# Orkis-Research/Quaternion-Convolutional-Neural-Networks-for-End-to-End-Automatic-Speech-Recognition

Hardware: AMD Instinct MI355X
Metric: quaternion-conv samples/sec (fwd+bwd+Adam of the full TIMIT QCNN, per-GPU batch 256) (higher is better)
Workload: dtype bf16; 1 GPU; cfg3_qcnn_relu_dropout_b256_bf16; per_gpu_batch=256, global_batch=256, filters=32, padding=same, activation=relu, loss=ctc, parallelism=dp1, optimizer=adam(5e-4) + l2 term folded into the update, launch=eager

## Files before the change

### include/qk.h

```cpp
#ifndef QK_H_
#define QK_H_

#include <stddef.h>
#include <stdint.h>

#ifdef __cplusplus
extern "C" {
#endif

#define QK_VERSION 103

typedef enum {
    QK_OK = 0,
    QK_ERR_INVALID_ARG = -1,
    QK_ERR_UNSUPPORTED = -2,
    QK_ERR_WORKSPACE = -3,
    QK_ERR_LAUNCH = -4
} qk_status_t;

typedef enum { QK_F32 = 0, QK_BF16 = 1, QK_F16 = 2 } qk_dtype_t;
typedef enum { QK_CH_LAST = 0, QK_CH_FIRST = 1 } qk_layout_t;
typedef enum { QK_ACT_LINEAR = 0, QK_ACT_RELU = 1 } qk_act_t;
typedef enum { QK_OP_FWD = 0, QK_OP_BWD_DATA = 1, QK_OP_BWD_WEIGHT = 2, QK_OP_BWD = 3 } qk_op_t;

typedef struct {
    int32_t rank;
    int32_t batch;
    int32_t in_spatial[3];
    int32_t out_spatial[3];
    int32_t cq;
    int32_t fq;
    int32_t kernel[3];
    int32_t stride[3];
    int32_t dilation[3];
    int32_t pad_lo[3];
    int32_t layout;
    int32_t dtype;
    int32_t activation;
    int32_t has_bias;
    int32_t conj;
    int32_t ws_has_kernel;
    int32_t kernel_order;
} qk_conv_desc_t;
#define QK_KERNEL_TAPS_MAJOR 0
#define QK_KERNEL_CHANNEL_MAJOR 1

typedef struct {
    int32_t rows;
    int32_t in_q;
    int32_t q_units;
    int32_t dtype;
    int32_t activation;
    int32_t has_bias;
    int32_t ws_has_kernel;
} qk_dense_desc_t;

int qk_version(void);
const char *qk_last_error(void);

#define QK_DBG_NO_MFMA16 1u
#define QK_DBG_NO_BAND16 2u
#define QK_DBG_NO_BAND32 4u
#define QK_DBG_WGRAD16_ONE_TAP 8u
#define QK_DBG_NO_WGRAD_BAND 32u
#define QK_DBG_NO_POINT16 64u
#define QK_DBG_CTC_TWO_SWEEPS 128u
#define QK_DBG_DETERMINISTIC 0x10000u
#define QK_DBG_WGRAD_BAND_V1 0x20000u
#define QK_DBG_NO_SMALL16 0x40000u
#define QK_DBG_NO_CONV_CHAIN 0x100000u
#define QK_DBG_NO_FUSED_PRELU 0x200000u
#define QK_DBG_NO_FUSED_DROPOUT 0x400000u
#define QK_DBG_NO_FUSED_CTC 0x800000u
#define QK_DBG_NO_FUSED_FIRST 0x1000000u
#define QK_DBG_NO_DENSE_IN_CHAIN 0x2000000u
#define QK_DBG_NO_FUSED_SOFTMAX 0x4000000u
#define QK_DBG_BAND16_8WAVES 16u
unsigned qk_set_debug_flags(unsigned flags);
void qk_set_debug_buffer(void *device_buffer, size_t bytes);
unsigned qk_get_debug_flags(void);

typedef enum { QK_PATH_NONE = 0, QK_PATH_MFMA16 = 1, QK_PATH_MFMA16_BAND = 2, QK_PATH_FP32_MFMA = 3,
               QK_PATH_MFMA16_POINT = 4, QK_PATH_MFMA16_SMALL = 5  } qk_path_t;
int qk_last_path(void);

typedef struct {
    int32_t op;
    int32_t dtype;
    int32_t path;
    int64_t rows;
    int32_t n, k;
    float ms;
} qk_prof_rec_t;
int qk_prof_enable(int on);
int qk_prof_count(void);
int qk_prof_get(int index, qk_prof_rec_t *out);

size_t qk_conv_workspace_bytes(const qk_conv_desc_t *desc, int op );
size_t qk_dense_workspace_bytes(const qk_dense_desc_t *desc, int op );

int qk_conv_fwd(const qk_conv_desc_t *desc, const void *x, const float *w, const float *bias,
                void *y, void *workspace, size_t workspace_bytes, void *stream);

int qk_conv_bwd_data(const qk_conv_desc_t *desc, const void *dy, const void *y, const float *w,
                     void *dx, void *workspace, size_t workspace_bytes, void *stream);

int qk_conv_bwd_weight(const qk_conv_desc_t *desc, const void *x, const void *dy, const void *y,
                       float *dw, float *dbias, void *workspace, size_t workspace_bytes,
                       void *stream);

int qk_conv_bwd_weight_acc(const qk_conv_desc_t *desc, const void *x, const void *dy, const void *y,
                           float *dw, float *dbias, void *workspace, size_t workspace_bytes,
                           void *stream);
int qk_dense_bwd_weight_acc(const qk_dense_desc_t *desc, const void *x, const void *dy, const void *y,
                            float *dw, float *dbias, void *workspace, size_t workspace_bytes,
                            void *stream);

int qk_conv_bwd(const qk_conv_desc_t *desc, const void *x, const void *dy, const void *y, const float *w,
                void *dx, float *dw, float *dbias, void *workspace, size_t workspace_bytes, void *stream);

#define QK_BWD_MASK_DX 1
#define QK_BWD_DY_PREMASKED 2
#define QK_BWD_ACCUMULATE 4
int qk_conv_bwd_chain(const qk_conv_desc_t *desc, const void *x, const void *dy, const void *y, const float *w,
                      void *dx, float *dw, float *dbias, int32_t flags, void *workspace, size_t workspace_bytes,
                      void *stream);
int qk_dense_bwd_chain(const qk_dense_desc_t *desc, const void *x, const void *dy, const void *y, const float *w,
                       void *dx, float *dw, float *dbias, int32_t flags, void *workspace, size_t workspace_bytes,
                       void *stream);

typedef struct {
    int32_t alpha_axis;
    int32_t alpha_len;
    const float *alpha;
    float drop_rate;
    uint32_t drop_seed;
    const uint32_t *drop_seed_dev;
} qk_postop_t;

int qk_conv_fwd_post(const qk_conv_desc_t *desc, const qk_postop_t *post, const void *x, const float *w,
                     const float *bias, void *pre, void *y, void *workspace, size_t workspace_bytes, void *stream);

int qk_conv_bwd_post(const qk_conv_desc_t *desc, const void *x, const void *dy, const float *w, void *dx, float *dw,
                     float *dbias, const qk_postop_t *post_x, const void *x_pre, float *dalpha_x, int32_t flags,
                     void *workspace, size_t workspace_bytes, void *stream);

int qk_postop_fwd(const qk_conv_desc_t *t, const qk_postop_t *post, const void *pre, void *y, void *stream);
int qk_postop_bwd(const qk_conv_desc_t *t, const qk_postop_t *post, const void *pre, const void *dy, void *dpre,
                  float *dalpha, void *stream);

size_t qk_conv_relu_pool_aux_bytes(const qk_conv_desc_t *desc, int32_t pool);
int qk_conv_relu_pool_fwd(const qk_conv_desc_t *desc, int32_t pool, const void *x, const float *w, const float *bias,
                          void *pooled, void *aux, void *stream);
int qk_conv_relu_pool_bwd(const qk_conv_desc_t *desc, int32_t pool, const void *x, const void *dpooled, const void *aux,
                          float *dw, float *dbias, int32_t flags, void *stream);

int qk_conv_prelu_pool_fwd(const qk_conv_desc_t *desc, int32_t pool, const qk_postop_t *post, const void *x, const float *w,
                           const float *bias, void *pooled, void *pre_pooled, void *aux, void *stream);
int qk_conv_prelu_pool_bwd(const qk_conv_desc_t *desc, int32_t pool, const qk_postop_t *post, const void *x, const void *dpooled,
                           const void *pre_pooled, const void *aux, float *dw, float *dbias, float *dalpha, int32_t flags,
                           void *stream);

int qk_conv_fold_taps(const qk_conv_desc_t *desc, const void *x, void *xcol, int32_t cq2, void *stream);

int qk_dense_fwd(const qk_dense_desc_t *desc, const void *x, const float *w, const float *bias,
                 void *y, void *workspace, size_t workspace_bytes, void *stream);
int qk_dense_bwd_data(const qk_dense_desc_t *desc, const void *dy, const void *y, const float *w,
                      void *dx, void *workspace, size_t workspace_bytes, void *stream);
int qk_dense_bwd_weight(const qk_dense_desc_t *desc, const void *x, const void *dy, const void *y,
                        float *dw, float *dbias, void *workspace, size_t workspace_bytes,
                        void *stream);

int qk_dense_bwd(const qk_dense_desc_t *desc, const void *x, const void *dy, const void *y, const float *w,
                 void *dx, float *dw, float *dbias, void *workspace, size_t workspace_bytes, void *stream);

typedef struct {
    int32_t batch, in_h, in_w, channels;
    int32_t win_h, win_w;
    int32_t out_h, out_w;
    int32_t dtype;
} qk_pool_desc_t;
int qk_maxpool2d_fwd(const qk_pool_desc_t *desc, const void *x, void *y, void *stream);
int qk_maxpool2d_bwd(const qk_pool_desc_t *desc, const void *x, const void *dy, void *dx, void *stream);

int qk_adam_step(float *param, const float *grad, float *m, float *v, size_t n, float lr,
                 float beta1, float beta2, float eps, int32_t step, float grad_scale,
                 void *stream);

int qk_adam_step_zero_grad(float *param, float *grad, float *m, float *v, size_t n, float lr,
                           float beta1, float beta2, float eps, int32_t step, float grad_scale,
                           void *stream);

size_t qk_ctc_workspace_bytes(int32_t batch, int32_t frames, int32_t max_label_len);
int qk_ctc_batch_cost(int32_t dtype, int32_t batch, int32_t frames, int32_t classes, const void *y_pred, const int32_t *labels,
                      int32_t max_label_len, const int32_t *input_length, const int32_t *label_length, float *cost, void *dy_pred,
                      void *workspace, size_t workspace_bytes, void *stream);

int qk_ctc_greedy_decode(int32_t dtype, int32_t batch, int32_t frames, int32_t classes, const void *y_pred, const int32_t *input_length,
                         int32_t *decoded, int32_t *decoded_len, float *log_prob, void *stream);
size_t qk_ctc_beam_workspace_bytes(int32_t batch, int32_t frames, int32_t beam_width);
int qk_ctc_beam_search_decode(int32_t dtype, int32_t batch, int32_t frames, int32_t classes, const void *y_pred, const int32_t *input_length,
                              int32_t beam_width, int32_t top_paths, int32_t merge_repeated, int32_t *decoded, int32_t *decoded_len,
                              float *log_prob, void *workspace, size_t workspace_bytes, void *stream);
int qk_ctc_beam_search_decode_lm(int32_t dtype, int32_t batch, int32_t frames, int32_t classes, const void *y_pred,
                                 const int32_t *input_length, int32_t beam_width, int32_t top_paths, int32_t merge_repeated,
                                 int32_t lm_order, const float *lm_table, float lm_weight, float insertion_bonus, int32_t lm_eos,
                                 int32_t *decoded, int32_t *decoded_len, float *log_prob, float *score,
                                 void *workspace, size_t workspace_bytes, void *stream);
int qk_edit_distance(int32_t batch, const int32_t *hyp, int32_t hyp_stride, const int32_t *hyp_len, const int32_t *ref, int32_t ref_stride,
                     const int32_t *ref_len, const int32_t *class_map, int32_t classes, int32_t *distance, int32_t *ref_len_out, void *stream);

#define QK_FBANK_MAX_FILT 128
enum { QK_WAVE_F32 = 0, QK_WAVE_I16 = 1 };
enum { QK_WINDOW_RECT = 0, QK_WINDOW_HAMMING = 1 };
enum { QK_FBANK_NORM_NONE = 0, QK_FBANK_NORM_UTTERANCE = 1 };
int32_t qk_fbank_num_frames(int64_t samples, int32_t frame_len, int32_t frame_step);
size_t qk_fbank_workspace_bytes(int32_t batch, int32_t frames, int32_t rows, int32_t normalize);
int qk_fbank_quaternion(int32_t wave_dtype, int32_t batch, int64_t max_samples, const void *wave, const int32_t *lengths, int32_t frames,
                        int32_t frame_len, int32_t frame_step, int32_t nfft, float preemph, int32_t window, int32_t nfilt,
                        const int32_t *mel_bins, int32_t append_energy, int32_t delta_n, int32_t normalize, int32_t out_dtype, void *out,
                        int32_t *frame_lengths, void *workspace, size_t workspace_bytes, void *stream);

#define QK_SPECAUG_MAX_MASKS 8
#define QK_SPECAUG_PLAN_WORDS 36
typedef struct qk_specaug_t {
    int32_t time_warp;
    int32_t freq_masks;
    int32_t freq_width;
    int32_t time_masks;
    int32_t time_width;
    float time_ratio;
    float fill;
    uint32_t seed;
} qk_specaug_t;
int qk_spec_augment(int32_t in_dtype, int32_t out_dtype, int32_t batch, int32_t planes, int32_t rows, int32_t frames,
                    const void *x, const int32_t *lengths, const qk_specaug_t *policy, const uint32_t *counter_dev ,
                    void *out, int32_t *plan , void *stream);

#define QK_SPEED_MAX_SPEEDS 8
#define QK_SPEED_MAX_DEN    32
#define QK_SPEED_MAX_TAPS   64
#define QK_SPEED_PLAN_WORDS 4
typedef struct qk_speed_perturb_t {
    int32_t n_speeds;
    int32_t num[QK_SPEED_MAX_SPEEDS];
    int32_t den[QK_SPEED_MAX_SPEEDS];
    int32_t half_width[QK_SPEED_MAX_SPEEDS];
    int32_t table_offset[QK_SPEED_MAX_SPEEDS];
    float gain_lo, gain_hi;
    uint32_t seed;
} qk_speed_perturb_t;
int64_t qk_speed_perturb_out_samples(int64_t max_samples, const qk_speed_perturb_t *policy);
int qk_speed_perturb(int32_t wave_dtype, int32_t batch, int64_t max_samples, const void *wave, const int32_t *lengths,
                     const qk_speed_perturb_t *policy, const float *tables , const uint32_t *counter_dev ,
                     int64_t out_samples, float *out, int32_t *out_lengths, int32_t *plan , void *stream);

int qk_softmax_rows_fwd(int32_t dtype, int64_t rows, int32_t cols, const float *logits, const float *bias, void *y, void *stream);
int qk_softmax_rows_bwd(int32_t dtype, int64_t rows, int32_t cols, const void *y, const void *dy, void *dlogits, float *dbias, void *stream);
int qk_dense_softmax_supported(int32_t dtype, int64_t rows, int32_t in_dim, int32_t units);
int qk_dense_softmax_fwd(int32_t dtype, int64_t rows, int32_t in_dim, int32_t units, const void *x, const float *kernel, const float *bias,
                         void *y, void *stream);
size_t qk_dense_softmax_bwd_workspace_bytes(int32_t dtype, int64_t rows, int32_t in_dim, int32_t units);
int qk_dense_softmax_bwd(int32_t dtype, int64_t rows, int32_t in_dim, int32_t units, const void *x, const float *kernel, const void *y,
                         const void *dy, void *dx, float *dkernel, float *dbias, const float *dy_scale_dev, float dy_scale,
                         void *workspace, size_t workspace_bytes, void *stream);
int qk_weighted_sum(int32_t dtype, int64_t n, const void *a, const float *w, float *out, void *stream);

int qk_conv_prep_kernels(int32_t n, const qk_conv_desc_t *const *descs, const int32_t *ops, const float *const *w,
                         void *const *workspaces, void *stream);

int qk_adam_step_l2(float *param, float *grad, float *m, float *v, const float *decay, size_t n, float lr,
                    float beta1, float beta2, float eps, int32_t step, float grad_scale, int32_t zero_grad,
                    void *stream);

int qk_adam_step_dev(float *param, float *grad, float *m, float *v, const float *decay, size_t n, float lr,
                     float beta1, float beta2, float eps, int32_t *step_dev, float grad_scale, int32_t zero_grad,
                     void *stream);

typedef struct qk_grad_guard_config_t {
    float clipnorm;
    float clipvalue;
    int32_t dynamic;
    float growth_factor;
    float backoff_factor;
    int32_t growth_interval;
    float min_scale;
    float max_scale;
} qk_grad_guard_config_t;

typedef struct qk_grad_guard_state_t {
    float scale;
    int32_t good_steps;
    int32_t skipped_steps;
    int32_t last_skipped;
    float last_norm;
    float last_coef;
    float last_unscale;
    int32_t nonfinite_count;
} qk_grad_guard_state_t;

size_t qk_grad_guard_workspace_bytes(size_t n);

int qk_grad_guard_reduce(const float *grad, const float *param, const float *decay, size_t n, float grad_scale,
                         const qk_grad_guard_config_t *config, qk_grad_guard_state_t *state, void *workspace,
                         size_t workspace_bytes, void *stream);

int qk_adam_step_guarded(float *param, float *grad, float *m, float *v, const float *decay, size_t n, float lr,
                         float beta1, float beta2, float eps, int32_t *step_dev, int32_t zero_grad,
                         const qk_grad_guard_config_t *config, const qk_grad_guard_state_t *state, void *stream);

#ifdef __cplusplus
}
#endif
#endif
```

### quaternion-convolutional-neural-networks-for-end-to-end-automatic-speech-recognition_amd/_lib.py

```python
import ctypes
import os

_HERE = os.path.dirname(os.path.realpath(__file__))
LIB_PATH = os.environ.get('QK_LIB') or os.path.join(_HERE, 'libqk_hip.so')

QK_F32, QK_BF16, QK_F16 = 0, 1, 2
QK_CH_LAST, QK_CH_FIRST = 0, 1
QK_ACT_LINEAR, QK_ACT_RELU = 0, 1
QK_OP_FWD, QK_OP_BWD_DATA, QK_OP_BWD_WEIGHT, QK_OP_BWD = 0, 1, 2, 3
QK_KERNEL_TAPS_MAJOR, QK_KERNEL_CHANNEL_MAJOR = 0, 1
QK_BWD_MASK_DX, QK_BWD_DY_PREMASKED, QK_BWD_ACCUMULATE = 1, 2, 4
QK_DBG_NO_MFMA16, QK_DBG_NO_BAND16, QK_DBG_NO_BAND32, QK_DBG_WGRAD16_ONE_TAP, QK_DBG_BAND16_8WAVES = 1, 2, 4, 8, 16
QK_DBG_NO_WGRAD_BAND = 32
QK_DBG_NO_POINT16 = 64
QK_DBG_CTC_TWO_SWEEPS = 128
QK_DBG_DETERMINISTIC = 0x10000
QK_DBG_WGRAD_BAND_V1 = 0x20000
QK_DBG_NO_SMALL16 = 0x40000
QK_DBG_NO_CONV_CHAIN, QK_DBG_NO_FUSED_PRELU, QK_DBG_NO_FUSED_DROPOUT, QK_DBG_NO_FUSED_CTC = 0x100000, 0x200000, 0x400000, 0x800000
QK_DBG_NO_FUSED_FIRST, QK_DBG_NO_DENSE_IN_CHAIN, QK_DBG_NO_FUSED_SOFTMAX = 0x1000000, 0x2000000, 0x4000000
QK_WAVE_F32, QK_WAVE_I16 = 0, 1
QK_WINDOW_RECT, QK_WINDOW_HAMMING = 0, 1
QK_FBANK_NORM_NONE, QK_FBANK_NORM_UTTERANCE = 0, 1
QK_FBANK_MAX_FILT = 128
QK_SPECAUG_MAX_MASKS, QK_SPECAUG_PLAN_WORDS = 8, 36
QK_SPEED_MAX_SPEEDS, QK_SPEED_MAX_DEN, QK_SPEED_MAX_TAPS, QK_SPEED_PLAN_WORDS = 8, 32, 64, 4
QK_ERR_INVALID_ARG, QK_ERR_UNSUPPORTED, QK_ERR_WORKSPACE, QK_ERR_LAUNCH = -1, -2, -3, -4
QK_PATH_NAMES = {0: 'none', 1: 'mfma16', 2: 'mfma16_band', 3: 'fp32_mfma', 4: 'mfma16_point', 5: 'mfma16_small'}

I32 = ctypes.c_int32


class ConvDesc(ctypes.Structure):
    _fields_ = [('rank', I32), ('batch', I32), ('in_spatial', I32 * 3), ('out_spatial', I32 * 3),
                ('cq', I32), ('fq', I32), ('kernel', I32 * 3), ('stride', I32 * 3),
                ('dilation', I32 * 3), ('pad_lo', I32 * 3), ('layout', I32), ('dtype', I32),
                ('activation', I32), ('has_bias', I32), ('conj', I32), ('ws_has_kernel', I32), ('kernel_order', I32)]


class DenseDesc(ctypes.Structure):
    _fields_ = [('rows', I32), ('in_q', I32), ('q_units', I32), ('dtype', I32),
                ('activation', I32), ('has_bias', I32), ('ws_has_kernel', I32)]


_VP, _FP, _SZ = ctypes.c_void_p, ctypes.c_void_p, ctypes.c_size_t
_CD, _DD = ctypes.POINTER(ConvDesc), ctypes.POINTER(DenseDesc)
class PoolDesc(ctypes.Structure):
    _fields_ = [('batch', ctypes.c_int32), ('in_h', ctypes.c_int32), ('in_w', ctypes.c_int32),
                ('channels', ctypes.c_int32), ('win_h', ctypes.c_int32), ('win_w', ctypes.c_int32),
                ('out_h', ctypes.c_int32), ('out_w', ctypes.c_int32), ('dtype', ctypes.c_int32)]


_PD = ctypes.POINTER(PoolDesc)


class PostOp(ctypes.Structure):
    _fields_ = [('alpha_axis', ctypes.c_int32), ('alpha_len', ctypes.c_int32), ('alpha', ctypes.c_void_p),
                ('drop_rate', ctypes.c_float), ('drop_seed', ctypes.c_uint32), ('drop_seed_dev', ctypes.c_void_p)]


_PO = ctypes.POINTER(PostOp)

class ProfRec(ctypes.Structure):
    _fields_ = [('op', I32), ('dtype', I32), ('path', I32), ('rows', ctypes.c_int64), ('n', I32), ('k', I32),
                ('ms', ctypes.c_float)]


class GradGuardConfig(ctypes.Structure):
    _fields_ = [('clipnorm', ctypes.c_float), ('clipvalue', ctypes.c_float), ('dynamic', I32),
                ('growth_factor', ctypes.c_float), ('backoff_factor', ctypes.c_float), ('growth_interval', I32),
                ('min_scale', ctypes.c_float), ('max_scale', ctypes.c_float)]


class SpecAugPolicy(ctypes.Structure):
    _fields_ = [('time_warp', I32), ('freq_masks', I32), ('freq_width', I32), ('time_masks', I32), ('time_width', I32),
                ('time_ratio', ctypes.c_float), ('fill', ctypes.c_float), ('seed', ctypes.c_uint32)]


class SpeedPerturbPolicy(ctypes.Structure):
    _fields_ = [('n_speeds', I32), ('num', I32 * 8), ('den', I32 * 8), ('half_width', I32 * 8), ('table_offset', I32 * 8),
                ('gain_lo', ctypes.c_float), ('gain_hi', ctypes.c_float), ('seed', ctypes.c_uint32)]


GRAD_GUARD_STATE = (('scale', True), ('good_steps', False), ('skipped_steps', False), ('last_skipped', False),
                    ('last_norm', True), ('last_coef', True), ('last_unscale', True), ('nonfinite_count', False))
_GC = ctypes.POINTER(GradGuardConfig)

SYMBOLS = {
    'qk_version': (ctypes.c_int, []),
    'qk_prof_enable': (ctypes.c_int, [ctypes.c_int]),
    'qk_prof_count': (ctypes.c_int, []),
    'qk_prof_get': (ctypes.c_int, [ctypes.c_int, ctypes.POINTER(ProfRec)]),
    'qk_last_error': (ctypes.c_char_p, []),
    'qk_set_debug_flags': (ctypes.c_uint, [ctypes.c_uint]),
    'qk_get_debug_flags': (ctypes.c_uint, []),
    'qk_set_debug_buffer': (None, [_VP, _SZ]),
    'qk_last_path': (ctypes.c_int, []),
    'qk_conv_workspace_bytes': (_SZ, [_CD, ctypes.c_int]),
    'qk_dense_workspace_bytes': (_SZ, [_DD, ctypes.c_int]),
    'qk_conv_fwd': (ctypes.c_int, [_CD, _VP, _FP, _FP, _VP, _VP, _SZ, _VP]),
    'qk_conv_bwd_data': (ctypes.c_int, [_CD, _VP, _VP, _FP, _VP, _VP, _SZ, _VP]),
    'qk_conv_fwd_post': (ctypes.c_int, [_CD, _PO, _VP, _FP, _FP, _VP, _VP, _VP, _SZ, _VP]),
    'qk_conv_bwd_post': (ctypes.c_int, [_CD, _VP, _VP, _FP, _VP, _FP, _FP, _PO, _VP, _FP, I32, _VP, _SZ, _VP]),
    'qk_postop_fwd': (ctypes.c_int, [_CD, _PO, _VP, _VP, _VP]),
    'qk_postop_bwd': (ctypes.c_int, [_CD, _PO, _VP, _VP, _VP, _FP, _VP]),
    'qk_conv_bwd_weight': (ctypes.c_int, [_CD, _VP, _VP, _VP, _FP, _FP, _VP, _SZ, _VP]),
    'qk_conv_bwd_chain': (ctypes.c_int, [_CD, _VP, _VP, _VP, _FP, _VP, _FP, _FP, I32, _VP, _SZ, _VP]),
    'qk_dense_bwd_chain': (ctypes.c_int, [_DD, _VP, _VP, _VP, _FP, _VP, _FP, _FP, I32, _VP, _SZ, _VP]),
    'qk_conv_bwd_weight_acc': (ctypes.c_int, [_CD, _VP, _VP, _VP, _FP, _FP, _VP, _SZ, _VP]),
    'qk_dense_bwd_weight_acc': (ctypes.c_int, [_DD, _VP, _VP, _VP, _FP, _FP, _VP, _SZ, _VP]),
    'qk_conv_bwd': (ctypes.c_int, [_CD, _VP, _VP, _VP, _FP, _VP, _FP, _FP, _VP, _SZ, _VP]),
    'qk_dense_bwd': (ctypes.c_int, [_DD, _VP, _VP, _VP, _FP, _VP, _FP, _FP, _VP, _SZ, _VP]),
    'qk_conv_fold_taps': (ctypes.c_int, [_CD, _VP, _VP, I32, _VP]),
    'qk_conv_relu_pool_aux_bytes': (_SZ, [_CD, I32]),
    'qk_conv_relu_pool_fwd': (ctypes.c_int, [_CD, I32, _VP, _FP, _FP, _VP, _VP, _VP]),
    'qk_conv_relu_pool_bwd': (ctypes.c_int, [_CD, I32, _VP, _VP, _VP, _FP, _FP, I32, _VP]),
    'qk_conv_prelu_pool_fwd': (ctypes.c_int, [_CD, I32, _PO, _VP, _FP, _FP, _VP, _VP, _VP, _VP]),
    'qk_conv_prelu_pool_bwd': (ctypes.c_int, [_CD, I32, _PO, _VP, _VP, _VP, _VP, _FP, _FP, _FP, I32, _VP]),
    'qk_dense_fwd': (ctypes.c_int, [_DD, _VP, _FP, _FP, _VP, _VP, _SZ, _VP]),
    'qk_dense_bwd_data': (ctypes.c_int, [_DD, _VP, _VP, _FP, _VP, _VP, _SZ, _VP]),
    'qk_dense_bwd_weight': (ctypes.c_int, [_DD, _VP, _VP, _VP, _FP, _FP, _VP, _SZ, _VP]),
    'qk_adam_step_zero_grad': (ctypes.c_int, [_FP, _FP, _FP, _FP, _SZ, ctypes.c_float, ctypes.c_float,
                                              ctypes.c_float, ctypes.c_float, I32, ctypes.c_float, _VP]),
    'qk_ctc_workspace_bytes': (_SZ, [I32, I32, I32]),
    'qk_ctc_batch_cost': (ctypes.c_int, [I32, I32, I32, I32, _VP, _VP, I32, _VP, _VP, _FP, _VP, _VP, _SZ, _VP]),
    'qk_conv_prep_kernels': (ctypes.c_int, [I32, ctypes.POINTER(_CD), ctypes.POINTER(I32), ctypes.POINTER(ctypes.c_void_p),
                                            ctypes.POINTER(ctypes.c_void_p), _VP]),
    'qk_adam_step_l2': (ctypes.c_int, [_FP, _FP, _FP, _FP, _FP, _SZ, ctypes.c_float, ctypes.c_float,
                                       ctypes.c_float, ctypes.c_float, I32, ctypes.c_float, I32, _VP]),
    'qk_adam_step_dev': (ctypes.c_int, [_FP, _FP, _FP, _FP, _FP, _SZ, ctypes.c_float, ctypes.c_float,
                                        ctypes.c_float, ctypes.c_float, _VP, ctypes.c_float, I32, _VP]),
    'qk_ctc_greedy_decode': (ctypes.c_int, [I32, I32, I32, I32, _VP, _VP, _VP, _VP, _FP, _VP]),
    'qk_ctc_beam_workspace_bytes': (_SZ, [I32, I32, I32]),
    'qk_ctc_beam_search_decode': (ctypes.c_int, [I32, I32, I32, I32, _VP, _VP, I32, I32, I32, _VP, _VP, _FP, _VP, _SZ, _VP]),
    'qk_ctc_beam_search_decode_lm': (ctypes.c_int, [I32, I32, I32, I32, _VP, _VP, I32, I32, I32, I32, _FP, ctypes.c_float,
                                                    ctypes.c_float, I32, _VP, _VP, _FP, _FP, _VP, _SZ, _VP]),
    'qk_edit_distance': (ctypes.c_int, [I32, _VP, I32, _VP, _VP, I32, _VP, _VP, I32, _VP, _VP, _VP]),
    'qk_fbank_num_frames': (I32, [ctypes.c_int64, I32, I32]),
    'qk_fbank_workspace_bytes': (_SZ, [I32, I32, I32, I32]),
    'qk_fbank_quaternion': (ctypes.c_int, [I32, I32, ctypes.c_int64, _VP, _VP, I32, I32, I32, I32, ctypes.c_float, I32, I32,
                                           ctypes.POINTER(I32), I32, I32, I32, I32, _VP, _VP, _VP, _SZ, _VP]),
    'qk_spec_augment': (ctypes.c_int, [I32, I32, I32, I32, I32, I32, _VP, _VP, ctypes.POINTER(SpecAugPolicy), _VP, _VP, _VP, _VP]),
    'qk_speed_perturb_out_samples': (ctypes.c_int64, [ctypes.c_int64, ctypes.POINTER(SpeedPerturbPolicy)]),
    'qk_speed_perturb': (ctypes.c_int, [I32, I32, ctypes.c_int64, _VP, _VP, ctypes.POINTER(SpeedPerturbPolicy), _VP, _VP, ctypes.c_int64,
                                        _VP, _VP, _VP, _VP]),
    'qk_softmax_rows_fwd': (ctypes.c_int, [I32, ctypes.c_int64, I32, _VP, _VP, _VP, _VP]),
    'qk_softmax_rows_bwd': (ctypes.c_int, [I32, ctypes.c_int64, I32, _VP, _VP, _VP, _VP, _VP]),
    'qk_dense_softmax_supported': (ctypes.c_int, [I32, ctypes.c_int64, I32, I32]),
    'qk_dense_softmax_fwd': (ctypes.c_int, [I32, ctypes.c_int64, I32, I32, _VP, _VP, _VP, _VP, _VP]),
    'qk_dense_softmax_bwd_workspace_bytes': (ctypes.c_size_t, [I32, ctypes.c_int64, I32, I32]),
    'qk_dense_softmax_bwd': (ctypes.c_int, [I32, ctypes.c_int64, I32, I32, _VP, _VP, _VP, _VP, _VP, _VP, _VP, _VP, ctypes.c_float, _VP, _SZ, _VP]),
    'qk_weighted_sum': (ctypes.c_int, [I32, ctypes.c_int64, _VP, _VP, _VP, _VP]),
    'qk_maxpool2d_fwd': (ctypes.c_int, [_PD, _VP, _VP, _VP]),
    'qk_maxpool2d_bwd': (ctypes.c_int, [_PD, _VP, _VP, _VP, _VP]),
    'qk_adam_step': (ctypes.c_int, [_FP, _FP, _FP, _FP, _SZ, ctypes.c_float, ctypes.c_float,
                                    ctypes.c_float, ctypes.c_float, I32, ctypes.c_float, _VP]),
    'qk_grad_guard_workspace_bytes': (_SZ, [_SZ]),
    'qk_grad_guard_reduce': (ctypes.c_int, [_FP, _FP, _FP, _SZ, ctypes.c_float, _GC, _VP, _VP, _SZ, _VP]),
    'qk_adam_step_guarded': (ctypes.c_int, [_FP, _FP, _FP, _FP, _FP, _SZ, ctypes.c_float, ctypes.c_float, ctypes.c_float,
                                            ctypes.c_float, _VP, I32, _GC, _VP, _VP]),
}

_lib = None


def lib():
    global _lib
    if _lib is None:
        if not os.path.exists(LIB_PATH):
            raise RuntimeError(
                'libqk_hip.so is not built (%s). Run `python -c "import __graft_entry__ as g; '
                'g.build()"` -- the quaternion layers have no CPU or eager fallback.' % LIB_PATH)
        handle = ctypes.CDLL(LIB_PATH)
        for name, (res, args) in SYMBOLS.items():
            fn = getattr(handle, name)
            fn.restype, fn.argtypes = res, args
        _lib = handle
    return _lib


def check(rc, what):
    if rc != 0:
        msg = lib().qk_last_error()
        raise RuntimeError('%s failed (status %d): %s' % (what, rc, msg.decode() if msg else ''))


def dbg(bit):
    return bool(lib().qk_get_debug_flags() & bit)


class debug_flags(object):

    def __init__(self, bits, ablate=0):
        self.bits = int(bits) | (int(ablate) << 8)

    def __enter__(self):
        self.prev = lib().qk_get_debug_flags()
        lib().qk_set_debug_flags(self.prev | self.bits)
        return self

    def __exit__(self, *exc):
        lib().qk_set_debug_flags(self.prev)
        return False


class profile(object):

    OPS = {QK_OP_FWD: 'fwd', QK_OP_BWD_DATA: 'bwd_data', QK_OP_BWD_WEIGHT: 'bwd_weight'}

    def __enter__(self):
        lib().qk_prof_enable(1)
        return self

    def __exit__(self, *exc):
        lib().qk_prof_enable(0)
        return False

    def records(self):
        out = []
        rec = ProfRec()
        for i in range(lib().qk_prof_count()):
            check(lib().qk_prof_get(i, ctypes.byref(rec)), 'qk_prof_get')
            out.append(dict(op=self.OPS.get(rec.op, str(rec.op)), dtype=rec.dtype, path=QK_PATH_NAMES.get(rec.path, 'none'),
                            rows=int(rec.rows), n=int(rec.n), k=int(rec.k), ms=float(rec.ms)))
        return out


def last_path():
    return QK_PATH_NAMES.get(lib().qk_last_path(), 'none')
```

### quaternion-convolutional-neural-networks-for-end-to-end-automatic-speech-recognition_amd/csrc/qk_api.hip

```cpp
#include <limits.h>
#include <math.h>
#include <stdarg.h>
#include <stdio.h>
#include <string.h>

#include "qk_common.h"

#include <atomic>
#include <mutex>
#include <vector>

namespace qk {

static thread_local char g_err[512] = "";
static thread_local int g_path = QK_PATH_NONE;
void note_path(int p) { g_path = p; }

namespace {
unsigned env_flags()
{
    unsigned f = 0;
    if (getenv("QK_NO_MFMA16")) f |= kDbgNoMfma16;
    if (getenv("QK_NO_BAND16")) f |= kDbgNoBand16;
    if (getenv("QK_NO_BAND32")) f |= kDbgNoBand32;
    if (getenv("QK_WGRAD16_ONE_TAP")) f |= kDbgWgradOneTap;
    if (getenv("QK_BAND16_8WAVES")) f |= kDbgBand8Waves;
    if (getenv("QK_NO_WGRAD_BAND")) f |= kDbgNoWgradBand;
    if (getenv("QK_NO_POINT16")) f |= kDbgNoPoint16;
    if (getenv("QK_CTC_TWO_SWEEPS")) f |= kDbgCtcTwoSweeps;
    if (getenv("QK_DETERMINISTIC")) f |= kDbgDeterministic;
    if (getenv("QK_WGRAD_BAND_V1")) f |= kDbgWgradBandV1;
    if (getenv("QK_NO_SMALL16")) f |= kDbgNoSmall16;
    if (getenv("QK_NO_CONV_CHAIN")) f |= QK_DBG_NO_CONV_CHAIN;
    if (getenv("QK_NO_FUSED_PRELU")) f |= QK_DBG_NO_FUSED_PRELU;
    if (getenv("QK_NO_FUSED_DROPOUT")) f |= QK_DBG_NO_FUSED_DROPOUT;
    if (getenv("QK_NO_FUSED_CTC")) f |= QK_DBG_NO_FUSED_CTC;
    if (getenv("QK_NO_FUSED_FIRST")) f |= QK_DBG_NO_FUSED_FIRST;
    if (getenv("QK_NO_DENSE_IN_CHAIN")) f |= QK_DBG_NO_DENSE_IN_CHAIN;
    if (getenv("QK_NO_FUSED_SOFTMAX")) f |= QK_DBG_NO_FUSED_SOFTMAX;
    if (const char *ab = getenv("QK_ABLATE")) f |= ((unsigned)atoi(ab) << kDbgAblateShift) & kDbgAblateMask;
    return f;
}
std::atomic<unsigned> &dbg_word()
{
    static std::atomic<unsigned> w{env_flags()};
    return w;
}
struct ForceCfg { bool set; int policy, bq; };
const ForceCfg &force_cfg()
{
    static const ForceCfg fc = [] {
        ForceCfg c = {false, -1, -1};
        if (const char *f = getenv("QK_FORCE_CFG")) c.set = sscanf(f, "%d,%d", &c.policy, &c.bq) == 2;
        return c;
    }();
    return fc;
}
}

unsigned debug_flags() { return dbg_word().load(std::memory_order_relaxed); }
static std::atomic<unsigned long long *> g_dbg_buf{nullptr};
static std::atomic<size_t> g_dbg_bytes{0};
unsigned long long *debug_buffer(size_t *bytes) { if (bytes) *bytes = g_dbg_bytes.load(); return g_dbg_buf.load(); }

namespace {
struct ProfRec { int op, dtype, path; long long rows; int n, k; hipEvent_t e0, e1; };
struct Prof { std::mutex mu; std::atomic<int> on{0}; std::vector<ProfRec> recs; };
Prof &prof() { static Prof p; return p; }
}
static thread_local int g_prof_nest = 0;
struct ProfScope {
    bool live = false;
    ProfRec r;
    hipStream_t stream;
    ProfScope(int op, const qk_conv_desc_t *d, hipStream_t st) : stream(st)
    {
        if (g_prof_nest++ > 0) return;
        if (!prof().on.load(std::memory_order_relaxed) || !d) return;
        r.op = op; r.dtype = d->dtype; r.path = QK_PATH_NONE;
        r.rows = (long long)d->batch * d->out_spatial[0] * d->out_spatial[1] * d->out_spatial[2];
        r.n = 4 * d->fq;
        r.k = 4 * d->cq * d->kernel[0] * d->kernel[1] * d->kernel[2];
        if (hipEventCreate(&r.e0) != hipSuccess) return;
        if (hipEventCreate(&r.e1) != hipSuccess) { (void)hipEventDestroy(r.e0); return; }
        live = hipEventRecord(r.e0, stream) == hipSuccess;
    }
    ~ProfScope()
    {
        --g_prof_nest;
        if (!live) return;
        (void)hipEventRecord(r.e1, stream);
        r.path = g_path;
        std::lock_guard<std::mutex> lk(prof().mu);
        prof().recs.push_back(r);
    }
};
bool debug_force_cfg(int *policy, int *bq)
{
    const ForceCfg &c = force_cfg();
    if (c.set) { *policy = c.policy; *bq = c.bq; }
    return c.set;
}
int device_cu_count()
{
    int dev = 0, n = 0;
    if (hipGetDevice(&dev) != hipSuccess || hipDeviceGetAttribute(&n, hipDeviceAttributeMultiprocessorCount, dev) != hipSuccess || n <= 0)
        return 256;
    return n;
}

void set_error(const char *fmt, ...)
{
    va_list ap;
    va_start(ap, fmt);
    vsnprintf(g_err, sizeof(g_err), fmt, ap);
    va_end(ap);
}

#define QK_DECL(sfx)                                                                              \
    int launch_hgemm_##sfx(const void *, const void *, const float *, const float *, void *,      \
                           const GemmGeom &, bool, hipStream_t);                                  \
    int launch_wgrad_##sfx(const void *, const void *, const void *, float *, float *,            \
                           const WgradGeom &, bool, hipStream_t);
QK_DECL(f32)
QK_DECL(bf16)
QK_DECL(f16)
#undef QK_DECL

int try_hgemm_16(int dtype, const void *in, const void *mask, const float *w_f32, const float *bias,
                 void *out, const GemmGeom &g, bool w_is_transposed, void *ws, size_t ws_bytes,
                 hipStream_t stream);

int try_wgrad_band_16(int dtype, const void *x, const void *dy, const void *ymask, float *dw, float *dbias,
                      const WgradGeom &g, hipStream_t stream);
int try_wgrad_16(int dtype, const void *x, const void *dy, const void *ymask, float *dw, float *dbias,
                 const WgradGeom &g, hipStream_t stream);

int launch_hgemm(int dtype, const void *in, const void *mask, const float *wk, const float *bias,
                 void *out, const GemmGeom &g, bool vec_ok, hipStream_t stream)
{
    switch (dtype) {
    case QK_F32: return launch_hgemm_f32(in, mask, wk, bias, out, g, vec_ok, stream);
    case QK_BF16: return launch_hgemm_bf16(in, mask, wk, bias, out, g, vec_ok, stream);
    case QK_F16: return launch_hgemm_f16(in, mask, wk, bias, out, g, vec_ok, stream);
    }
    return QK_ERR_INVALID_ARG;
}

int launch_wgrad(int dtype, const void *x, const void *dy, const void *ymask, float *dw,
                 float *dbias, WgradGeom g, bool vec_ok, hipStream_t stream)
{
    switch (dtype) {
    case QK_F32: return launch_wgrad_f32(x, dy, ymask, dw, dbias, g, vec_ok, stream);
    case QK_BF16: return launch_wgrad_bf16(x, dy, ymask, dw, dbias, g, vec_ok, stream);
    case QK_F16: return launch_wgrad_f16(x, dy, ymask, dw, dbias, g, vec_ok, stream);
    }
    return QK_ERR_INVALID_ARG;
}

namespace {

size_t elem_bytes(int dtype) { return dtype == QK_F32 ? 4 : 2; }

bool aligned(const void *p, size_t a) { return (reinterpret_cast<uintptr_t>(p) % a) == 0; }

bool vec_aligned(const void *p, int dtype) { return aligned(p, 4 * elem_bytes(dtype)); }

int validate(const qk_conv_desc_t *d, bool allow_rank0)
{
    if (!d) { set_error("descriptor is NULL"); return QK_ERR_INVALID_ARG; }
    if (d->rank < (allow_rank0 ? 0 : 1) || d->rank > 3) {
        set_error("rank %d not in [1,3]", d->rank); return QK_ERR_INVALID_ARG;
    }
    if (d->batch <= 0 || d->cq <= 0 || d->fq <= 0) {
        set_error("batch/cq/fq must be positive (got %d/%d/%d)", d->batch, d->cq, d->fq);
        return QK_ERR_INVALID_ARG;
    }
    long long si = 1, so = 1, taps = 1;
    for (int i = 0; i < 3; ++i) {
        if (d->in_spatial[i] <= 0 || d->out_spatial[i] <= 0 || d->kernel[i] <= 0 ||
            d->stride[i] <= 0 || d->dilation[i] <= 0 || d->pad_lo[i] < 0) {
            set_error("axis %d: extents/kernel/stride/dilation must be > 0 and pad_lo >= 0", i);
            return QK_ERR_INVALID_ARG;
        }
        if (i >= d->rank && (d->in_spatial[i] != 1 || d->out_spatial[i] != 1 || d->kernel[i] != 1 ||
                             d->stride[i] != 1 || d->dilation[i] != 1 || d->pad_lo[i] != 0)) {
            set_error("axis %d is beyond rank %d and must be the identity (1,1,1,1,1,0)", i, d->rank);
            return QK_ERR_INVALID_ARG;
        }
        si *= d->in_spatial[i]; so *= d->out_spatial[i]; taps *= d->kernel[i];
    }
    if (si * d->batch * 4LL * d->cq > INT_MAX || so * d->batch * 4LL * d->fq > INT_MAX ||
// ... 966 lines not shown
    g.span = (g.tile - 1) * frame_step + frame_len;
    const bool norm = normalize == QK_FBANK_NORM_UTTERANCE;
    const size_t need = fbank_workspace_bytes(batch, frames, g.F, norm);
    if (!workspace || workspace_bytes < need || !aligned(workspace, 16)) { set_error("fbank_quaternion needs %zu workspace bytes, got %zu", need, workspace_bytes); return QK_ERR_WORKSPACE; }
    return check_launch(launch_fbank(wave_dtype, wave, lengths, g, delta_n, norm, out_dtype, out, frame_lengths, workspace,
                                     (hipStream_t)stream), "qk_fbank_quaternion");
}

int qk_spec_augment(int32_t in_dtype, int32_t out_dtype, int32_t batch, int32_t planes, int32_t rows, int32_t frames,
                    const void *x, const int32_t *lengths, const qk_specaug_t *policy, const uint32_t *counter_dev,
                    void *out, int32_t *plan, void *stream)
{
    if (batch < 1 || planes < 1 || rows < 1 || frames < 1 || in_dtype < QK_F32 || in_dtype > QK_F16 || out_dtype < QK_F32 || out_dtype > QK_F16) {
        set_error("spec_augment: bad arguments (batch %d, planes %d, rows %d, frames %d, dtypes %d / %d)", batch, planes, rows, frames, in_dtype, out_dtype);
        return QK_ERR_INVALID_ARG;
    }
    if (!x || !lengths || !policy || !out) { set_error("spec_augment: NULL argument"); return QK_ERR_INVALID_ARG; }
    const qk_specaug_t &p = *policy;
    if (p.freq_masks < 0 || p.freq_masks > QK_SPECAUG_MAX_MASKS || p.time_masks < 0 || p.time_masks > QK_SPECAUG_MAX_MASKS) {
        set_error("spec_augment: freq_masks %d / time_masks %d outside 0 .. %d", p.freq_masks, p.time_masks, QK_SPECAUG_MAX_MASKS);
        return QK_ERR_INVALID_ARG;
    }
    if (p.time_warp < 0 || p.freq_width < 0 || p.time_width < 0) {
        set_error("spec_augment: time_warp %d, freq_width %d and time_width %d must be >= 0", p.time_warp, p.freq_width, p.time_width);
        return QK_ERR_INVALID_ARG;
    }
    if (!isfinite(p.time_ratio) || p.time_ratio < 0.f || p.time_ratio > 1.f || !isfinite(p.fill)) {
        set_error("spec_augment: time_ratio %g must lie in [0, 1] and fill %g be finite", (double)p.time_ratio, (double)p.fill);
        return QK_ERR_INVALID_ARG;
    }
    const long long count = (long long)batch * planes * rows * frames;
    if (count > INT_MAX) { set_error("spec_augment: tensor with >= 2^31 elements"); return QK_ERR_UNSUPPORTED; }
    const size_t in_bytes = (size_t)count * elem_bytes(in_dtype), out_bytes = (size_t)count * elem_bytes(out_dtype);
    if (!aligned(x, elem_bytes(in_dtype)) || !aligned(out, elem_bytes(out_dtype)) || (plan && !aligned(plan, 4))) {
        set_error("spec_augment: x, out and plan must be aligned to their element size"); return QK_ERR_INVALID_ARG;
    }
    const uintptr_t xa = reinterpret_cast<uintptr_t>(x), oa = reinterpret_cast<uintptr_t>(out);
    if (xa < oa + out_bytes && oa < xa + in_bytes) { set_error("spec_augment: out overlaps x (the warp reads neighbouring frames)"); return QK_ERR_INVALID_ARG; }
    return check_launch(launch_spec_augment(in_dtype, out_dtype, batch, planes, rows, frames, x, lengths, p, counter_dev, out, plan,
                                            (hipStream_t)stream), "qk_spec_augment");
}

static int speed_policy_check(const qk_speed_perturb_t *policy)
{
    if (!policy) { set_error("speed_perturb: policy is NULL"); return QK_ERR_INVALID_ARG; }
    const qk_speed_perturb_t &p = *policy;
    if (p.n_speeds < 1 || p.n_speeds > QK_SPEED_MAX_SPEEDS) {
        set_error("speed_perturb: n_speeds %d outside 1 .. %d", p.n_speeds, QK_SPEED_MAX_SPEEDS); return QK_ERR_INVALID_ARG;
    }
    if (!isfinite(p.gain_lo) || !isfinite(p.gain_hi) || p.gain_lo < 0.f || p.gain_lo > p.gain_hi) {
        set_error("speed_perturb: gains %g, %g must be finite with 0 <= gain_lo <= gain_hi", (double)p.gain_lo, (double)p.gain_hi);
        return QK_ERR_INVALID_ARG;
    }
    for (int i = 0; i < p.n_speeds; ++i) {
        const int num = p.num[i], den = p.den[i], kw = p.half_width[i];
        if (num < 1 || num > QK_SPEED_MAX_DEN || den < 1 || den > QK_SPEED_MAX_DEN || 2 * num < den || num > 2 * den) {
            set_error("speed_perturb: speed %d = %d / %d (both in 1 .. %d, ratio in [1/2, 2])", i, num, den, QK_SPEED_MAX_DEN);
            return QK_ERR_INVALID_ARG;
        }
        if (kw < 0 || (num == den) != (kw == 0)) {
            set_error("speed_perturb: speed %d = %d / %d with half_width %d (0 exactly when num == den)", i, num, den, kw);
            return QK_ERR_INVALID_ARG;
        }
        if (num != den && p.table_offset[i] < 0) { set_error("speed_perturb: table_offset[%d] = %d", i, p.table_offset[i]); return QK_ERR_INVALID_ARG; }
    }
    for (int i = 0; i < p.n_speeds; ++i)
        if (2 * (long long)p.half_width[i] + 2 > QK_SPEED_MAX_TAPS) {
            set_error("speed_perturb: speed %d has %lld taps, more than %d", i, 2 * (long long)p.half_width[i] + 2, QK_SPEED_MAX_TAPS);
            return QK_ERR_UNSUPPORTED;
        }
    return 0;
}

int64_t qk_speed_perturb_out_samples(int64_t max_samples, const qk_speed_perturb_t *policy)
{
    if (max_samples < 1) { set_error("speed_perturb_out_samples: max_samples %lld < 1", (long long)max_samples); return -1; }
    const int rc = speed_policy_check(policy);
    if (rc != 0 && rc != QK_ERR_UNSUPPORTED) return -1;
    if (max_samples > INT64_MAX / QK_SPEED_MAX_DEN) { set_error("speed_perturb_out_samples: max_samples too large"); return -1; }
    int64_t most = 0;
    for (int i = 0; i < policy->n_speeds; ++i) {
        const int64_t len = (max_samples * policy->den[i] + policy->num[i] - 1) / policy->num[i];
        if (len > most) most = len;
    }
    return most;
}

int qk_speed_perturb(int32_t wave_dtype, int32_t batch, int64_t max_samples, const void *wave, const int32_t *lengths,
                     const qk_speed_perturb_t *policy, const float *tables, const uint32_t *counter_dev, int64_t out_samples, float *out,
                     int32_t *out_lengths, int32_t *plan, void *stream)
{
    if (batch < 1 || max_samples < 1 || (wave_dtype != QK_WAVE_F32 && wave_dtype != QK_WAVE_I16)) {
        set_error("speed_perturb: bad arguments (batch %d, max_samples %lld, wave_dtype %d)", batch, (long long)max_samples, wave_dtype);
        return QK_ERR_INVALID_ARG;
    }
    if (!wave || !lengths || !out || !out_lengths) { set_error("speed_perturb: NULL argument"); return QK_ERR_INVALID_ARG; }
    const int rc = speed_policy_check(policy);
    if (rc == QK_ERR_INVALID_ARG) return rc;
    bool filters = false;
    for (int i = 0; i < policy->n_speeds; ++i) filters |= policy->num[i] != policy->den[i];
    if (filters && !tables) { set_error("speed_perturb: tables is NULL, but a speed has num != den"); return QK_ERR_INVALID_ARG; }
    const int64_t limit = (int64_t)1 << 26;
    if (max_samples < limit && out_samples < qk_speed_perturb_out_samples(max_samples, policy)) {
        set_error("speed_perturb: out_samples %lld below the %lld that max_samples %lld needs", (long long)out_samples,
                  (long long)qk_speed_perturb_out_samples(max_samples, policy), (long long)max_samples);
        return QK_ERR_INVALID_ARG;
    }
    const size_t wave_elem = wave_dtype == QK_WAVE_I16 ? 2 : 4;
    if (!aligned(wave, wave_elem) || !aligned(out, 4) || !aligned(lengths, 4) || !aligned(out_lengths, 4) || (plan && !aligned(plan, 4)) ||
        (tables && !aligned(tables, 4)) || (counter_dev && !aligned(counter_dev, 4))) {
        set_error("speed_perturb: pointers must be aligned to their element size"); return QK_ERR_INVALID_ARG;
    }
    if (rc != 0) return rc;
    if (max_samples >= limit || out_samples >= limit) {
        set_error("speed_perturb: max_samples %lld / out_samples %lld must be below 2^26", (long long)max_samples, (long long)out_samples);
        return QK_ERR_UNSUPPORTED;
    }
    const uintptr_t wa = reinterpret_cast<uintptr_t>(wave), oa = reinterpret_cast<uintptr_t>(out);
    const size_t wave_bytes = (size_t)batch * (size_t)max_samples * wave_elem, out_bytes = (size_t)batch * (size_t)out_samples * 4;
    if (wa < oa + out_bytes && oa < wa + wave_bytes) { set_error("speed_perturb: out overlaps wave"); return QK_ERR_INVALID_ARG; }
    return check_launch(launch_speed_perturb(wave_dtype, batch, (int)max_samples, wave, lengths, *policy, tables, counter_dev, (int)out_samples,
                                             out, out_lengths, plan, (hipStream_t)stream), "qk_speed_perturb");
}

int qk_softmax_rows_fwd(int32_t dtype, int64_t rows, int32_t cols, const float *logits, const float *bias, void *y, void *stream)
{
    if (!logits || !y || rows < 0 || cols < 1 || cols > 64 || dtype < QK_F32 || dtype > QK_F16) { set_error("qk_softmax_rows_fwd: bad argument (1 <= cols <= 64)"); return QK_ERR_INVALID_ARG; }
    if (rows == 0) return QK_OK;
    return check_launch(launch_softmax_rows(dtype, false, logits, bias, y, nullptr, rows, cols, (hipStream_t)stream), "qk_softmax_rows_fwd");
}

int qk_softmax_rows_bwd(int32_t dtype, int64_t rows, int32_t cols, const void *y, const void *dy, void *dlogits, float *dbias, void *stream)
{
    if (!y || !dy || !dlogits || rows < 0 || cols < 1 || cols > 64 || dtype < QK_F32 || dtype > QK_F16) { set_error("qk_softmax_rows_bwd: bad argument (1 <= cols <= 64)"); return QK_ERR_INVALID_ARG; }
    if (rows == 0) return QK_OK;
    return check_launch(launch_softmax_rows(dtype, true, y, dy, dlogits, dbias, rows, cols, (hipStream_t)stream), "qk_softmax_rows_bwd");
}

int qk_dense_softmax_supported(int32_t dtype, int64_t rows, int32_t in_dim, int32_t units)
{
    return dense_softmax_supported(dtype, rows, in_dim, units) ? 1 : 0;
}

int qk_dense_softmax_fwd(int32_t dtype, int64_t rows, int32_t in_dim, int32_t units, const void *x, const float *kernel, const float *bias,
                         void *y, void *stream)
{
    if (!x || !kernel || !y || rows < 0) { set_error("qk_dense_softmax_fwd: NULL buffer or negative row count"); return QK_ERR_INVALID_ARG; }
    if (!dense_softmax_supported(dtype, rows, in_dim, units)) { set_error("qk_dense_softmax_fwd: in_dim %d / units %d / dtype %d outside the kernel (in_dim 64, 128, 256; even units <= 64; 16-bit)", in_dim, units, dtype); return QK_ERR_UNSUPPORTED; }
    if (!aligned(x, 16) || !aligned(y, 4) || !aligned(kernel, 4)) { set_error("qk_dense_softmax_fwd: x must be 16-byte aligned, y 4-byte"); return QK_ERR_INVALID_ARG; }
    if (rows == 0) return QK_OK;
    return check_launch(launch_dense_softmax_fwd(dtype, rows, in_dim, units, x, kernel, bias, y, (hipStream_t)stream), "qk_dense_softmax_fwd");
}

size_t qk_dense_softmax_bwd_workspace_bytes(int32_t dtype, int64_t rows, int32_t in_dim, int32_t units)
{
    return dense_softmax_bwd_workspace_bytes(dtype, rows, in_dim, units);
}

int qk_dense_softmax_bwd(int32_t dtype, int64_t rows, int32_t in_dim, int32_t units, const void *x, const float *kernel, const void *y,
                         const void *dy, void *dx, float *dkernel, float *dbias, const float *dy_scale_dev, float dy_scale,
                         void *workspace, size_t workspace_bytes, void *stream)
{
    if (!x || !kernel || !y || !dy || !dx || rows < 0) { set_error("qk_dense_softmax_bwd: NULL buffer or negative row count"); return QK_ERR_INVALID_ARG; }
    if (!dense_softmax_supported(dtype, rows, in_dim, units)) { set_error("qk_dense_softmax_bwd: in_dim %d / units %d / dtype %d outside the kernel (in_dim 64, 128, 256; even units <= 64; 16-bit)", in_dim, units, dtype); return QK_ERR_UNSUPPORTED; }
    if (!aligned(x, 16) || !aligned(dx, 16) || !aligned(y, 4) || !aligned(dy, 4)) { set_error("qk_dense_softmax_bwd: x / dx must be 16-byte aligned, y / dy 4-byte"); return QK_ERR_INVALID_ARG; }
    if (rows == 0) return QK_OK;
    if (dkernel || dbias) {
        const size_t need = dense_softmax_bwd_workspace_bytes(dtype, rows, in_dim, units);
        if (!workspace || workspace_bytes < need || !aligned(workspace, 16)) { set_error("qk_dense_softmax_bwd needs %zu workspace bytes (16-byte aligned), got %zu", need, workspace_bytes); return QK_ERR_WORKSPACE; }
    }
    return check_launch(launch_dense_softmax_bwd(dtype, rows, in_dim, units, x, kernel, y, dy, dx, dkernel, dbias, dy_scale_dev, dy_scale, static_cast<float *>(workspace), (hipStream_t)stream), "qk_dense_softmax_bwd");
}

int qk_weighted_sum(int32_t dtype, int64_t n, const void *a, const float *w, float *out, void *stream)
{
    if (!a || !w || !out || n < 0 || dtype < QK_F32 || dtype > QK_F16) { set_error("qk_weighted_sum: bad argument"); return QK_ERR_INVALID_ARG; }
    if (n == 0) return QK_OK;
    return check_launch(launch_weighted_sum(dtype, a, w, out, n, (hipStream_t)stream), "qk_weighted_sum");
}

int qk_conv_prep_kernels(int32_t n, const qk_conv_desc_t *const *descs, const int32_t *ops, const float *const *w,
                         void *const *workspaces, void *stream)
{
    if (n < 0 || (n > 0 && (!descs || !ops || !w || !workspaces))) { set_error("qk_conv_prep_kernels: NULL argument"); return QK_ERR_INVALID_ARG; }
    for (int dt = QK_BF16; dt <= QK_F16; ++dt) {
        PrepJobs jobs;
        int m = 0;
        for (int i = 0; i <= n; ++i) {
            if (i < n) {
                const qk_conv_desc_t *d = descs[i];
                if (!d || !w[i] || !workspaces[i]) { set_error("qk_conv_prep_kernels: job %d has a NULL member", i); return QK_ERR_INVALID_ARG; }
                if (d->dtype != dt) continue;
                if (ops[i] != QK_OP_FWD && ops[i] != QK_OP_BWD_DATA && ops[i] != QK_OP_BWD) { set_error("qk_conv_prep_kernels: job %d: bad op %d", i, ops[i]); return QK_ERR_INVALID_ARG; }
                if (!aligned(workspaces[i], 16)) { set_error("qk_conv_prep_kernels: job %d: workspace not 16-byte aligned", i); return QK_ERR_INVALID_ARG; }
                if (d->cq % 16 || d->fq % 16) continue;
                const bool bwd = ops[i] != QK_OP_FWD;
                PrepJob &j = jobs.j[m++];
                j.w = w[i]; j.wq = workspaces[i]; j.taps = taps_of(d); j.cq = d->cq; j.fq = d->fq;
                j.transposed = bwd ? 1 : 0;
                j.small = 0; j.kin = 0; j.n_ot = 0;
                j.ch_major = d->kernel_order == QK_KERNEL_CHANNEL_MAJOR;
                j.neg_ijk = bwd ? (d->conj ? 1 : 0) : (d->conj ? 0 : 1);
                {
                    GemmGeom sg, sbg;
                    Small16 sm;
                    prep_geom(d, bwd, &sg);
                    if (d->layout == QK_CH_LAST && !j.ch_major && small16_shape(sg, &sbg, &sm)) {
                        PrepJob &k = jobs.j[m++];
                        k = j;
                        k.wq = static_cast<char *>(workspaces[i]) + (size_t)j.taps * pad32(d->cq) * 4 * pad32(d->fq) * 2 + 256;
                        k.small = 1; k.kin = sm.kin; k.n_ot = sm.n_ot;
                    }
                }
            }
            if (m >= 31 || (i == n && m > 0)) {
                if (int rc = launch_prep_w16_batch(dt, jobs, m, (hipStream_t)stream)) return check_launch(rc, "qk_conv_prep_kernels");
                m = 0;
            }
        }
    }
    for (int i = 0; i < n; ++i)
        if (descs[i]->dtype != QK_BF16 && descs[i]->dtype != QK_F16) { set_error("qk_conv_prep_kernels: job %d is not a 16-bit descriptor", i); return QK_ERR_INVALID_ARG; }
    return QK_OK;
}

int qk_adam_step(float *param, const float *grad, float *m, float *v, size_t n, float lr, float beta1,
                 float beta2, float eps, int32_t step, float grad_scale, void *stream)
{
    if (!param || !grad || !m || !v) { set_error("adam: NULL buffer"); return QK_ERR_INVALID_ARG; }
    if (step < 1) { set_error("adam: step must be >= 1"); return QK_ERR_INVALID_ARG; }
    return check_launch(launch_adam(param, const_cast<float *>(grad), m, v, nullptr, n, lr, beta1, beta2, eps, step, grad_scale, false, (hipStream_t)stream), "qk_adam_step");
}

int qk_adam_step_zero_grad(float *param, float *grad, float *m, float *v, size_t n, float lr, float beta1,
                           float beta2, float eps, int32_t step, float grad_scale, void *stream)
{
    if (!param || !grad || !m || !v) { set_error("adam: NULL buffer"); return QK_ERR_INVALID_ARG; }
    if (step < 1) { set_error("adam: step must be >= 1"); return QK_ERR_INVALID_ARG; }
    return check_launch(launch_adam(param, grad, m, v, nullptr, n, lr, beta1, beta2, eps, step, grad_scale, true, (hipStream_t)stream), "qk_adam_step_zero_grad");
}

int qk_adam_step_l2(float *param, float *grad, float *m, float *v, const float *decay, size_t n, float lr, float beta1,
                    float beta2, float eps, int32_t step, float grad_scale, int32_t zero_grad, void *stream)
{
    if (!param || !grad || !m || !v) { set_error("adam: NULL buffer"); return QK_ERR_INVALID_ARG; }
    if (step < 1) { set_error("adam: step must be >= 1"); return QK_ERR_INVALID_ARG; }
    return check_launch(launch_adam(param, grad, m, v, decay, n, lr, beta1, beta2, eps, step, grad_scale, zero_grad != 0, (hipStream_t)stream), "qk_adam_step_l2");
}

int qk_adam_step_dev(float *param, float *grad, float *m, float *v, const float *decay, size_t n, float lr, float beta1,
                     float beta2, float eps, int32_t *step_dev, float grad_scale, int32_t zero_grad, void *stream)
{
    if (!param || !grad || !m || !v || !step_dev) { set_error("adam: NULL buffer"); return QK_ERR_INVALID_ARG; }
    return check_launch(launch_adam(param, grad, m, v, decay, n, lr, beta1, beta2, eps, 1, grad_scale, zero_grad != 0, (hipStream_t)stream, step_dev), "qk_adam_step_dev");
}

static bool guard_config_ok(const qk_grad_guard_config_t *c, const char *what)
{
    if (!c) { set_error("%s: NULL config", what); return false; }
    if (!(c->clipnorm >= 0.f) || !(c->clipvalue >= 0.f)) { set_error("%s: clipnorm / clipvalue must be >= 0", what); return false; }
    if (c->dynamic && !(c->backoff_factor > 0.f && c->backoff_factor < 1.f && c->growth_factor > 1.f && c->growth_interval >= 1
                        && c->min_scale > 0.f && c->min_scale <= c->max_scale)) {
        set_error("%s: dynamic scaling needs 0 < backoff_factor < 1 < growth_factor, growth_interval >= 1, 0 < min_scale <= max_scale", what);
        return false;
    }
    return true;
}

size_t qk_grad_guard_workspace_bytes(size_t n) { return grad_guard_workspace_bytes(n); }

int qk_grad_guard_reduce(const float *grad, const float *param, const float *decay, size_t n, float grad_scale,
                         const qk_grad_guard_config_t *config, qk_grad_guard_state_t *state, void *workspace,
                         size_t workspace_bytes, void *stream)
{
    if (!grad || !state || !workspace) { set_error("qk_grad_guard_reduce: NULL grad, state or workspace"); return QK_ERR_INVALID_ARG; }
    if (n == 0) { set_error("qk_grad_guard_reduce: n must be > 0"); return QK_ERR_INVALID_ARG; }
    if ((param == nullptr) != (decay == nullptr)) { set_error("qk_grad_guard_reduce: param and decay go together"); return QK_ERR_INVALID_ARG; }
    if (!guard_config_ok(config, "qk_grad_guard_reduce")) return QK_ERR_INVALID_ARG;
    if (!aligned(grad, 4) || !aligned(state, 4) || (param && (!aligned(param, 4) || !aligned(decay, 4))) || !aligned(workspace, 16)) {
        set_error("qk_grad_guard_reduce: buffers need 4-byte alignment, the workspace 16-byte alignment");
        return QK_ERR_INVALID_ARG;
    }
    if (workspace_bytes < grad_guard_workspace_bytes(n)) {
        set_error("qk_grad_guard_reduce: workspace of %zu bytes, %zu needed", workspace_bytes, grad_guard_workspace_bytes(n));
        return QK_ERR_INVALID_ARG;
    }
    return check_launch(launch_grad_guard_reduce(grad, param, decay, n, grad_scale, *config, state, workspace, (hipStream_t)stream),
                        "qk_grad_guard_reduce");
}

int qk_adam_step_guarded(float *param, float *grad, float *m, float *v, const float *decay, size_t n, float lr, float beta1,
                         float beta2, float eps, int32_t *step_dev, int32_t zero_grad, const qk_grad_guard_config_t *config,
                         const qk_grad_guard_state_t *state, void *stream)
{
    if (!param || !grad || !m || !v || !step_dev || !state) { set_error("qk_adam_step_guarded: NULL buffer, step counter or state"); return QK_ERR_INVALID_ARG; }
    if (n == 0) { set_error("qk_adam_step_guarded: n must be > 0"); return QK_ERR_INVALID_ARG; }
    if (!guard_config_ok(config, "qk_adam_step_guarded")) return QK_ERR_INVALID_ARG;
    return check_launch(launch_adam_guarded(param, grad, m, v, decay, n, lr, beta1, beta2, eps, step_dev, zero_grad != 0, config->clipvalue,
                                            state, (hipStream_t)stream), "qk_adam_step_guarded");
}

}
```

### quaternion-convolutional-neural-networks-for-end-to-end-automatic-speech-recognition_amd/csrc/qk_common.h

```cpp
#pragma once

#include <hip/hip_runtime.h>
#include <stdint.h>
#include <stdio.h>
#include <stdlib.h>

#include "../../include/qk.h"

namespace qk {

constexpr unsigned kSignConv = 0x5390u;
constexpr unsigned kSignConj = 0x284Eu;

struct PostOp {
    int kind;
    int alpha_sel;
    int alpha_len;
    const float *alpha;
    float drop_scale;
    unsigned drop_thr;
    unsigned drop_seed;
    const unsigned *seed_dev;
};

// ... 131 lines not shown
    *mul = (unsigned)(((1ull << (31 + s)) + d - 1) / d);
    *sh = s;
}
__host__ __device__ __forceinline__ int fast_div(int n, unsigned mul, unsigned sh)
{
    return (int)(((unsigned long long)(unsigned)n * mul) >> (31 + sh));
}

struct bf16 { uint16_t x; };
typedef _Float16 f16;

__device__ __forceinline__ float to_f32(float v) { return v; }
__device__ __forceinline__ float to_f32(bf16 v) { return __uint_as_float(((uint32_t)v.x) << 16); }
__device__ __forceinline__ float to_f32(f16 v) { return (float)v; }

template <typename T> __device__ __forceinline__ T from_f32(float v);
template <> __device__ __forceinline__ float from_f32<float>(float v) { return v; }
template <> __device__ __forceinline__ bf16 from_f32<bf16>(float v)
{
    uint32_t u = __float_as_uint(v);
    bf16 r;
    if ((u & 0x7fffffffu) > 0x7f800000u) { r.x = (uint16_t)((u >> 16) | 0x40u); return r; }
    u += 0x7fffu + ((u >> 16) & 1u);
    r.x = (uint16_t)(u >> 16);
    return r;
}
template <> __device__ __forceinline__ f16 from_f32<f16>(float v) { return (f16)v; }

__device__ __forceinline__ void load4(const float *p, float (&o)[4])
{
    const float4 v = *reinterpret_cast<const float4 *>(p);
    o[0] = v.x; o[1] = v.y; o[2] = v.z; o[3] = v.w;
}
__device__ __forceinline__ void load4(const bf16 *p, float (&o)[4])
{
    const uint2 v = *reinterpret_cast<const uint2 *>(p);
    o[0] = __uint_as_float(v.x << 16); o[1] = __uint_as_float(v.x & 0xffff0000u);
    o[2] = __uint_as_float(v.y << 16); o[3] = __uint_as_float(v.y & 0xffff0000u);
}
__device__ __forceinline__ void load4(const f16 *p, float (&o)[4])
{
    typedef f16 h4 __attribute__((ext_vector_type(4)));
    const h4 v = *reinterpret_cast<const h4 *>(p);
    o[0] = (float)v[0]; o[1] = (float)v[1]; o[2] = (float)v[2]; o[3] = (float)v[3];
}

template <typename T>
__device__ __forceinline__ void prep_small16_write(const float *w, T *wq, long long idx, int Cq, int F, int transposed, int neg_ijk,
                                                   int kin, int q32, int fb_n)
{
    const int kso = q32 ? kin : (kin + 1) / 2;
    long long r = idx;
    const int e = (int)(r % 8); r /= 8;
    const int lane = (int)(r % 64); r /= 64;
    const int fb = (int)(r % fb_n); r /= fb_n;
    const int p = (int)(r % 4); r /= 4;
    const int kk = (int)r;
    const int k = (lane >> 4) * 8 + e;
    const int ot = kk / kso, ki = kk - ot * kso;
    const int tap_in = q32 ? ki : 2 * ki + (k >> 4);
    const int q = q32 ? k : (k & 15);
    const int j = fb * 16 + (lane & 15);
    float v = 0.f;
    if (tap_in < kin) {
        const int tap = ot * kin + tap_in;
        const int c = transposed ? j : q, f = transposed ? q : j;
        v = w[((long long)(tap * Cq + c) * 4 + p) * F + f];
        if (neg_ijk && p) v = -v;
    }
    wq[idx] = from_f32<T>(v);
}

typedef float floatx16 __attribute__((ext_vector_type(16)));
typedef float floatx4 __attribute__((ext_vector_type(4)));

__device__ __forceinline__ int mfma32_row(int r, int lane) { return (r & 3) + 8 * (r >> 2) + 4 * (lane >> 5); }

int launch_hgemm(int dtype, const void *in, const void *mask, const float *wk, const float *bias,
                 void *out, const GemmGeom &g, bool vec_ok, hipStream_t stream);
int launch_wgrad(int dtype, const void *x, const void *dy, const void *ymask, float *dw,
                 float *dbias, WgradGeom g, bool vec_ok, hipStream_t stream);
int launch_fold_taps(int dtype, const void *x, void *xcol, const GemmGeom &g, int cq2, hipStream_t stream);
int launch_mask_gt0(int dtype, void *data, const void *mask, size_t n, hipStream_t stream);
struct PrepJob { const float *w; void *wq; int taps, cq, fq, transposed, neg_ijk;
                 int small, kin, n_ot, ch_major; };
struct PrepJobs { PrepJob j[32]; };
int launch_prep_w16_batch(int dtype, const PrepJobs &jobs, int n, hipStream_t stream);
struct Small16 { int q32, fb, kin, kso, n_ot, nkk; unsigned w_bytes; };
inline bool small16_shape(const GemmGeom &g_in, GemmGeom *bg, Small16 *s)
{
    if (!((g_in.Q == 16 || g_in.Q == 32) && g_in.J == 16)) return false;
    GemmGeom g = g_in;
    g.Qp = pad32(g.Q); g.Jp = pad32(g.J);
    if (!band_geom(g, 2, bg)) return false;
    s->q32 = g.Q == 32; s->fb = g.J / 16; s->kin = bg->ks[2]; s->n_ot = bg->ks[0] * bg->ks[1];
    s->kso = s->q32 ? s->kin : (s->kin + 1) / 2;
    s->nkk = s->n_ot * s->kso;
    s->w_bytes = (unsigned)(s->nkk * 4 * s->fb * 1024);
    return s->n_ot <= 3;
}
inline size_t small16_region_bytes(const Small16 &s) { return ((size_t)s.w_bytes + 255) / 256 * 256 + 256; }
int launch_prep_small16(int dtype, const float *w, void *wq, int Cq, int F, int transposed, int neg_ijk, const Small16 &s, hipStream_t stream);
int launch_hconv16_small(int dtype, const void *in, const void *wq, const float *bias, void *out, const GemmGeom &bg, const Small16 &s, hipStream_t stream);

size_t ctc_workspace_bytes(int B, int T, int Lmax);
int launch_ctc(int dtype, int B, int T, int C, const void *pred, const int *labels, int Lmax, const int *in_len, const int *lab_len,
               float *cost, void *dpred, float *ws, hipStream_t stream);
size_t ctc_beam_workspace_bytes(int B, int T, int W);
int launch_ctc_greedy(int dtype, int B, int T, int C, const void *pred, const int *in_len, int *decoded, int *dlen, float *logp,
                      hipStream_t stream);
int launch_ctc_beam(int dtype, int B, int T, int C, const void *pred, const int *in_len, int W, int top, int merge, int *decoded,
                    int *dlen, float *logp, int *hist, hipStream_t stream);
int ctc_beam_lm_supported(int C, int W, int order);
int launch_ctc_beam_lm(int dtype, int B, int T, int C, const void *pred, const int *in_len, int W, int top, int merge, int order,
                       const float *table, float alpha, float beta, int eos, int *decoded, int *dlen, float *logp, float *score, int *hist,
                       hipStream_t stream);
int launch_edit_distance(int B, const int *hyp, int hs, const int *hl, const int *ref, int rs, const int *rl, const int *cmap,
                         int classes, int *out, int *rlen_out, hipStream_t stream);
struct FbankGeom {
    int B, n_max, T;
    int L, S, nfft;
    int nfilt, F;
    int tile, span;
    int window;
    float preemph;
    int bins[QK_FBANK_MAX_FILT + 2];
};
int fbank_tile(int L, int S);
size_t fbank_workspace_bytes(int B, int T, int F, bool norm);
int launch_fbank(int wave_dtype, const void *wave, const int *lengths, const FbankGeom &g, int N, bool norm, int out_dtype, void *out,
                 int *frame_lengths, void *ws, hipStream_t stream);
int launch_spec_augment(int in_dtype, int out_dtype, int B, int P, int R, int T, const void *x, const int *lengths,
                        const qk_specaug_t &pol, const unsigned *counter, void *out, int *plan, hipStream_t stream);
int launch_speed_perturb(int wave_dtype, int B, int n_max, const void *wave, const int *lengths, const qk_speed_perturb_t &pol,
                         const float *tables, const unsigned *counter, int n_out, float *out, int *out_lengths, int *plan,
                         hipStream_t stream);
int launch_relayout16(const void *src, void *dst, int n, int A, int B, hipStream_t stream);
struct PoolGeom { int batch, ih, iw, C, wh, ww, oh, ow; };
int launch_maxpool(int dtype, bool backward, const void *x, const void *dy, void *out, const PoolGeom &g, hipStream_t stream);
size_t conv1_pool_argbits_bytes(int N, int H, int W, int F);
int launch_conv1_pool(int dtype, bool backward, const void *x, const float *w, const float *bias, const void *io, void *argbits,
                      float *dw, float *dbias, int N, int H, int W, int F, int has_bias, hipStream_t stream,
                      const float *alpha = nullptr, int alpha_len = 0, const void *pre = nullptr, float *dalpha = nullptr,
                      int x_planes = 0);
int launch_postop(int dtype, bool backward, const void *pre, const void *dy, void *out, float *dalpha, const PostOp &p,
                  long long rows, int channels, int key_div, int key_mod, hipStream_t stream);
int launch_softmax_rows(int dtype, bool backward, const void *a, const void *b, void *out, float *dbias, long long rows, int cols,
                        hipStream_t stream);
int launch_weighted_sum(int dtype, const void *a, const float *w, float *out, long long n, hipStream_t stream);
bool dense_softmax_supported(int dtype, long long rows, int K, int U);
int launch_dense_softmax_fwd(int dtype, long long rows, int K, int U, const void *x, const float *w, const float *bias, void *y, hipStream_t stream);
size_t dense_softmax_bwd_workspace_bytes(int dtype, long long rows, int K, int U);
int launch_dense_softmax_bwd(int dtype, long long rows, int K, int U, const void *x, const float *w, const void *y, const void *dy, void *dx,
                             float *dw, float *dbias, const float *dy_scale_dev, float dy_scale, float *ws, hipStream_t stream);
int launch_adam(float *p, float *g, float *m, float *v, const float *decay, size_t n, float lr, float b1,
                float b2, float eps, int step, float gscale, bool zero_grad, hipStream_t stream, int *step_dev = nullptr);
size_t grad_guard_workspace_bytes(size_t n);
int launch_grad_guard_reduce(const float *grad, const float *param, const float *decay, size_t n, float grad_scale,
                             const qk_grad_guard_config_t &cfg, qk_grad_guard_state_t *state, void *ws, hipStream_t stream);
int launch_adam_guarded(float *p, float *g, float *m, float *v, const float *decay, size_t n, float lr, float b1, float b2, float eps,
                        int *step_dev, bool zero_grad, float clipvalue, const qk_grad_guard_state_t *state, hipStream_t stream);

void set_error(const char *fmt, ...);
void note_path(int qk_path);

enum : unsigned {
    kDbgNoMfma16 = QK_DBG_NO_MFMA16, kDbgNoBand16 = QK_DBG_NO_BAND16, kDbgNoBand32 = QK_DBG_NO_BAND32,
    kDbgWgradOneTap = QK_DBG_WGRAD16_ONE_TAP, kDbgBand8Waves = QK_DBG_BAND16_8WAVES, kDbgNoWgradBand = QK_DBG_NO_WGRAD_BAND,
    kDbgNoPoint16 = QK_DBG_NO_POINT16, kDbgCtcTwoSweeps = QK_DBG_CTC_TWO_SWEEPS, kDbgDeterministic = QK_DBG_DETERMINISTIC, kDbgWgradBandV1 = QK_DBG_WGRAD_BAND_V1, kDbgNoSmall16 = QK_DBG_NO_SMALL16, kDbgAblateShift = 8, kDbgAblateMask = 0xffu << 8
};
unsigned debug_flags();
unsigned long long *debug_buffer(size_t *bytes);
inline int debug_ablate() { return (int)((debug_flags() & kDbgAblateMask) >> kDbgAblateShift); }
bool debug_force_cfg(int *policy, int *bq);
int device_cu_count();

}
```

### quaternion-convolutional-neural-networks-for-end-to-end-automatic-speech-recognition_amd/csrc/qk_out_layer.hip

```cpp
#include "qk_common.h"

namespace qk {
namespace {

typedef __bf16 o_bf16x8 __attribute__((ext_vector_type(8)));
typedef _Float16 o_f16x8 __attribute__((ext_vector_type(8)));
typedef short o_v4s __attribute__((ext_vector_type(4)));
typedef short o_v8s __attribute__((ext_vector_type(8)));
typedef __attribute__((address_space(3))) o_v4s o_lds_v4s;

__device__ __forceinline__ floatx4 mfma_o(bf16, const uint4 &a, const uint4 &b, const floatx4 &c)
{
    return __builtin_amdgcn_mfma_f32_16x16x32_bf16(__builtin_bit_cast(o_bf16x8, a), __builtin_bit_cast(o_bf16x8, b), c, 0, 0, 0);
}
__device__ __forceinline__ floatx4 mfma_o(f16, const uint4 &a, const uint4 &b, const floatx4 &c)
{
    return __builtin_amdgcn_mfma_f32_16x16x32_f16(__builtin_bit_cast(o_f16x8, a), __builtin_bit_cast(o_f16x8, b), c, 0, 0, 0);
}
__device__ __forceinline__ unsigned pack2o(bf16, float a, float b) { return (unsigned)from_f32<bf16>(a).x | ((unsigned)from_f32<bf16>(b).x << 16); }
__device__ __forceinline__ unsigned pack2o(f16, float a, float b)
{
    const f16 x = (f16)a, y = (f16)b;
    return (unsigned)__builtin_bit_cast(unsigned short, x) | ((unsigned)__builtin_bit_cast(unsigned short, y) << 16);
}
__device__ __forceinline__ float lo16(bf16, unsigned v) { return __uint_as_float(v << 16); }
__device__ __forceinline__ float hi16(bf16, unsigned v) { return __uint_as_float(v & 0xffff0000u); }
__device__ __forceinline__ float lo16(f16, unsigned v) { return (float)__builtin_bit_cast(f16, (unsigned short)(v & 0xffffu)); }
__device__ __forceinline__ float hi16(f16, unsigned v) { return (float)__builtin_bit_cast(f16, (unsigned short)(v >> 16)); }

typedef unsigned int o_u32x4 __attribute__((ext_vector_type(4)));
__device__ __forceinline__ __amdgpu_buffer_rsrc_t rsrc_o(const void *p, unsigned long long bytes)
{
    return __builtin_amdgcn_make_buffer_rsrc(const_cast<void *>(p), 0, (int)(bytes > 0xffffffffull ? 0xffffffffu : (unsigned)bytes), 0x00020000);
}
__device__ __forceinline__ uint4 ld16_o(__amdgpu_buffer_rsrc_t r, unsigned voff)
{
    const o_u32x4 v = __builtin_amdgcn_raw_buffer_load_b128(r, (int)voff, 0, 0);
    return make_uint4(v.x, v.y, v.z, v.w);
}
constexpr unsigned kOob = 0xF0000000u;

template <typename T, int KS>
__global__ void __launch_bounds__(256) __attribute__((amdgpu_waves_per_eu(2, 2)))
k_dense_softmax_fwd(const T *__restrict__ x, const float *__restrict__ w, const float *__restrict__ bias, T *__restrict__ y,
                    const long long rows, const int U)
{
    constexpr int K = KS * 32;
    constexpr int WP = K + 8;
    __shared__ __attribute__((aligned(16))) T wt[64 * WP];
    const int tid = threadIdx.x, lane = tid & 63, wave = tid >> 6;
    const int l16 = lane & 15, g = lane >> 4;
    const __amdgpu_buffer_rsrc_t rx = rsrc_o(x, (unsigned long long)rows * K * sizeof(T));
    const long long n_tiles = (rows + 15) / 16;
    const long long stride = (long long)gridDim.x * 4;
    long long tile = (long long)blockIdx.x * 4 + wave;
    uint4 xf[KS], xn[KS];
    auto fetch = [&](long long tl, uint4 (&dst)[KS]) {
        const long long row = tl * 16 + l16;
        const unsigned off = (tl < n_tiles && row < rows) ? (unsigned)((row * K + 8 * g) * (long long)sizeof(T)) : kOob;
#pragma unroll
        for (int s = 0; s < KS; ++s) dst[s] = ld16_o(rx, off == kOob ? kOob : off + 64u * s);
    };
    fetch(tile, xf);
    {
        const int c = tid & 63, kq = tid >> 6;
        constexpr int KPT = K / 4;
        const float *wc = w + c;
#pragma unroll
        for (int k0 = 0; k0 < KPT; k0 += 16) {
            float v[16];
#pragma unroll
            for (int q = 0; q < 16; ++q) v[q] = c < U ? wc[(long long)(kq * KPT + k0 + q) * U] : 0.f;
#pragma unroll
            for (int q = 0; q < 16; q += 2) *reinterpret_cast<unsigned *>(wt + c * WP + kq * KPT + k0 + q) = pack2o(T(), v[q], v[q + 1]);
        }
    }
    __syncthreads();
    uint4 wf[4][KS];
#pragma unroll
    for (int t = 0; t < 4; ++t)
#pragma unroll
        for (int s = 0; s < KS; ++s) wf[t][s] = *reinterpret_cast<const uint4 *>(wt + (16 * t + l16) * WP + 32 * s + 8 * g);
    float b0[4][4];
#pragma unroll
    for (int t = 0; t < 4; ++t)
#pragma unroll
        for (int r = 0; r < 4; ++r) {
            const int c = 16 * t + 4 * g + r;
            b0[t][r] = c < U ? (bias ? bias[c] : 0.f) : -1e30f;
        }
    for (; tile < n_tiles; tile += stride) {
        fetch(tile + stride, xn);
        floatx4 acc[4];
#pragma unroll
        for (int t = 0; t < 4; ++t)
#pragma unroll
            for (int r = 0; r < 4; ++r) acc[t][r] = b0[t][r];
#pragma unroll
        for (int s = 0; s < KS; ++s)
#pragma unroll
            for (int t = 0; t < 4; ++t) acc[t] = mfma_o(T(), wf[t][s], xf[s], acc[t]);
        float m = -1e30f;
#pragma unroll
        for (int t = 0; t < 4; ++t)
#pragma unroll
            for (int r = 0; r < 4; ++r) m = fmaxf(m, acc[t][r]);
        m = fmaxf(m, __shfl_xor(m, 16));
        m = fmaxf(m, __shfl_xor(m, 32));
        float sum = 0.f;
#pragma unroll
        for (int t = 0; t < 4; ++t)
#pragma unroll
            for (int r = 0; r < 4; ++r) { acc[t][r] = __expf(acc[t][r] - m); sum += acc[t][r]; }
        sum += __shfl_xor(sum, 16);
        sum += __shfl_xor(sum, 32);
        const float inv = 1.f / sum;
        const long long row = tile * 16 + l16;
        if (row < rows) {
            T *yr = y + row * U;
#pragma unroll
            for (int t = 0; t < 4; ++t) {
                const int c = 16 * t + 4 * g;
                if ((U & 1) == 0) {
                    if (c + 1 < U) *reinterpret_cast<unsigned *>(yr + c) = pack2o(T(), acc[t][0] * inv, acc[t][1] * inv);
                    if (c + 3 < U) *reinterpret_cast<unsigned *>(yr + c + 2) = pack2o(T(), acc[t][2] * inv, acc[t][3] * inv);
                } else {
#pragma unroll
                    for (int r = 0; r < 4; ++r)
                        if (c + r < U) yr[c + r] = from_f32<T>(acc[t][r] * inv);
                }
            }
        }
#pragma unroll
        for (int s = 0; s < KS; ++s) xf[s] = xn[s];
    }
}

template <typename T, int NW>
__global__ void __launch_bounds__(NW * 64)
k_dense_softmax_bwd(const T *__restrict__ x, const float *__restrict__ w, const T *__restrict__ y, const T *__restrict__ dy,
                    T *__restrict__ dx, float *__restrict__ part, const long long rows, const int U,
                    const float *__restrict__ dy_scale_dev, const float dy_scale)
{
    constexpr int K = NW * 64, NTHR = NW * 64;
    constexpr int XP = K * 2 + 32;
    constexpr int DP = 160;
    static_assert(((XP / 4) % 16) == 8, "x tile pitch: 8 dwords (mod 16) keeps 8 consecutive rows on 8 different 8-bank groups");
    constexpr int RPT = (32 * 8) / NTHR;
    constexpr int XU = (32 * K * 2 / 16) / NTHR;
    __shared__ __attribute__((aligned(16))) char xs[32 * XP];
    __shared__ __attribute__((aligned(16))) char ds[32 * DP];
    __shared__ float dbs[NTHR / 8][64];
    const int tid = threadIdx.x, lane = tid & 63, wave = __builtin_amdgcn_readfirstlane(tid >> 6);
    const int l16 = lane & 15, g = lane >> 4;

    uint4 wf[2][2][2];
#pragma unroll
    for (int u = 0; u < 2; ++u)
#pragma unroll
        for (int e = 0; e < 2; ++e)
#pragma unroll
            for (int s = 0; s < 2; ++s) {
                const int col = 64 * wave + 32 * u + 8 * (l16 >> 2) + 4 * e + (l16 & 3);
                const float *wr = w + (long long)col * U + 32 * s + 8 * g;
                float v[8];
#pragma unroll
                for (int q = 0; q < 8; ++q) v[q] = (32 * s + 8 * g + q < U) ? wr[q] : 0.f;
                wf[u][e][s] = make_uint4(pack2o(T(), v[0], v[1]), pack2o(T(), v[2], v[3]), pack2o(T(), v[4], v[5]), pack2o(T(), v[6], v[7]));
            }
    floatx4 gw[4][4];
#pragma unroll
    for (int t = 0; t < 4; ++t)
#pragma unroll
        for (int u = 0; u < 4; ++u)
#pragma unroll
            for (int r = 0; r < 4; ++r) gw[t][u][r] = 0.f;
    float dbp[8];
#pragma unroll
    for (int q = 0; q < 8; ++q) dbp[q] = 0.f;

    const __amdgpu_buffer_rsrc_t rx = rsrc_o(x, (unsigned long long)rows * K * sizeof(T));
    const float sc = (dy_scale_dev ? *dy_scale_dev : 1.f) * dy_scale;
    const int l8 = tid & 7;
    const int np = (U + 1) / 2;
    const long long n_blocks = (rows + 31) / 32;
    uint4 xr[XU];
    unsigned yv[RPT][4], gv[RPT][4];
    auto fetch = [&](long long blk) {
#pragma unroll
        for (int k = 0; k < XU; ++k) {
            const int unit = tid + k * NTHR;
            const long long row = blk * 32 + unit / (K / 8);
            xr[k] = ld16_o(rx, (blk < n_blocks && row < rows) ? (unsigned)(row * K * 2 + (unit % (K / 8)) * 16) : kOob);
        }
#pragma unroll
        for (int rr = 0; rr < RPT; ++rr) {
            const long long row = blk * 32 + (tid >> 3) + rr * (NTHR / 8);
            const bool ok = blk < n_blocks && row < rows;
#pragma unroll
            for (int q = 0; q < 4; ++q) {
                const int p = l8 + 8 * q;
                const bool okp = ok && p < np;
                yv[rr][q] = okp ? *reinterpret_cast<const unsigned *>(y + row * U + 2 * p) : 0u;
                gv[rr][q] = okp ? *reinterpret_cast<const unsigned *>(dy + row * U + 2 * p) : 0u;
            }
        }
    };
    long long blk = blockIdx.x;
    if (blk < n_blocks) fetch(blk);
    for (; blk < n_blocks; blk += gridDim.x) {
#pragma unroll
        for (int rr = 0; rr < RPT; ++rr) {
            float dot = 0.f;
#pragma unroll
            for (int q = 0; q < 4; ++q)
                dot += lo16(T(), yv[rr][q]) * lo16(T(), gv[rr][q]) + hi16(T(), yv[rr][q]) * hi16(T(), gv[rr][q]);
            dot += __shfl_xor(dot, 1);
            dot += __shfl_xor(dot, 2);
            dot += __shfl_xor(dot, 4);
            const int lrow = (tid >> 3) + rr * (NTHR / 8);
#pragma unroll
            for (int q = 0; q < 4; ++q) {
                const int p = l8 + 8 * q;
                const unsigned d2 = pack2o(T(), sc * lo16(T(), yv[rr][q]) * (lo16(T(), gv[rr][q]) - dot), sc * hi16(T(), yv[rr][q]) * (hi16(T(), gv[rr][q]) - dot));
                *reinterpret_cast<unsigned *>(ds + lrow * DP + 4 * p) = p < np ? d2 : 0u;
                dbp[2 * q] += lo16(T(), d2);
                dbp[2 * q + 1] += hi16(T(), d2);
            }
        }
#pragma unroll
        for (int k = 0; k < XU; ++k) {
            const int unit = tid + k * NTHR;
            *reinterpret_cast<uint4 *>(xs + (unit / (K / 8)) * XP + (unit % (K / 8)) * 16) = xr[k];
        }
        __syncthreads();
        fetch(blk + gridDim.x);
        {
            floatx4 acc[2][2][2];
#pragma unroll
            for (int rt = 0; rt < 2; ++rt) {
                uint4 dl[2];
#pragma unroll
                for (int s = 0; s < 2; ++s) dl[s] = *reinterpret_cast<const uint4 *>(ds + (16 * rt + l16) * DP + 64 * s + 16 * g);
#pragma unroll
                for (int u = 0; u < 2; ++u)
#pragma unroll
                    for (int e = 0; e < 2; ++e) {
                        floatx4 a = {0.f, 0.f, 0.f, 0.f};
                        a = mfma_o(T(), wf[u][e][0], dl[0], a);
                        a = mfma_o(T(), wf[u][e][1], dl[1], a);
                        acc[rt][u][e] = a;
                    }
            }
#pragma unroll
            for (int rt = 0; rt < 2; ++rt) {
                const long long row = blk * 32 + 16 * rt + l16;
                if (row < rows) {
#pragma unroll
                    for (int u = 0; u < 2; ++u) {
                        const floatx4 a0 = acc[rt][u][0], a1 = acc[rt][u][1];
                        const uint4 v = make_uint4(pack2o(T(), a0[0], a0[1]), pack2o(T(), a0[2], a0[3]), pack2o(T(), a1[0], a1[1]), pack2o(T(), a1[2], a1[3]));
                        *reinterpret_cast<uint4 *>(dx + row * K + 64 * wave + 32 * u + 8 * g) = v;
                    }
                }
            }
        }
        {
            const int tr_row = 4 * g + (l16 >> 2), tr_col = 4 * (l16 & 3);
            uint4 af[4], bf[4];
#pragma unroll
            for (int t = 0; t < 4; ++t) {
                const char *p = ds + tr_row * DP + (16 * t + tr_col) * 2;
                const o_v4s lo = __builtin_amdgcn_ds_read_tr16_b64_v4i16((o_lds_v4s *)(p));
                const o_v4s hi = __builtin_amdgcn_ds_read_tr16_b64_v4i16((o_lds_v4s *)(p + 16 * DP));
                af[t] = __builtin_bit_cast(uint4, __builtin_shufflevector(lo, hi, 0, 1, 2, 3, 4, 5, 6, 7));
            }
#pragma unroll
            for (int u = 0; u < 4; ++u) {
                const char *p = xs + tr_row * XP + (64 * wave + 16 * u + tr_col) * 2;
                const o_v4s lo = __builtin_amdgcn_ds_read_tr16_b64_v4i16((o_lds_v4s *)(p));
                const o_v4s hi = __builtin_amdgcn_ds_read_tr16_b64_v4i16((o_lds_v4s *)(p + 16 * XP));
                bf[u] = __builtin_bit_cast(uint4, __builtin_shufflevector(lo, hi, 0, 1, 2, 3, 4, 5, 6, 7));
            }
#pragma unroll
            for (int t = 0; t < 4; ++t)
#pragma unroll
                for (int u = 0; u < 4; ++u) gw[t][u] = mfma_o(T(), af[t], bf[u], gw[t][u]);
        }
        __syncthreads();
    }
    if (part) {
        float *slab = part + (long long)blockIdx.x * (NW * 16 * 256 + 64);
#pragma unroll
        for (int t = 0; t < 4; ++t)
#pragma unroll
            for (int u = 0; u < 4; ++u)
                *reinterpret_cast<floatx4 *>(slab + ((wave * 16 + t * 4 + u) * 64 + lane) * 4) = gw[t][u];
#pragma unroll
        for (int q = 0; q < 4; ++q) {
            const int p = l8 + 8 * q;
            dbs[tid >> 3][2 * p] = dbp[2 * q];
            dbs[tid >> 3][2 * p + 1] = dbp[2 * q + 1];
        }
        __syncthreads();
        if (tid < 64) {
            float sum = 0.f;
            for (int r = 0; r < NTHR / 8; ++r) sum += dbs[r][tid];
            slab[NW * 16 * 256 + tid] = sum;
        }
    }
}

template <int NW>
__global__ void __launch_bounds__(1024)
k_dense_softmax_reduce(const float *__restrict__ part, const int n_slabs, float *__restrict__ dw, float *__restrict__ dbias, const int U)
{
    __shared__ floatx4 red[64][16];
    constexpr int SLAB = NW * 16 * 256 + 64;
    const int q = threadIdx.x & 15, grp = threadIdx.x >> 4;
    floatx4 sum = {0.f, 0.f, 0.f, 0.f};
    if ((int)blockIdx.x == NW * 64) {
        for (int sl = grp; sl < n_slabs; sl += 64) sum += *reinterpret_cast<const floatx4 *>(part + (long long)sl * SLAB + NW * 16 * 256 + 4 * q);
    } else {
        const float *p = part + ((long long)blockIdx.x * 16 + q) * 4;
#pragma unroll 8
        for (int sl = grp; sl < n_slabs; sl += 64) sum += *reinterpret_cast<const floatx4 *>(p + (long long)sl * SLAB);
    }
    red[grp][q] = sum;
    __syncthreads();
    if (grp < 8) {
        floatx4 v = red[grp][q];
#pragma unroll
        for (int k = 1; k < 8; ++k) v += red[grp + 8 * k][q];
        red[grp][q] = v;
    }
    __syncthreads();
    if (grp != 0) return;
    floatx4 v = red[0][q];
#pragma unroll
    for (int k = 1; k < 8; ++k) v += red[k][q];
    if ((int)blockIdx.x == NW * 64) {
        if (dbias)
#pragma unroll
            for (int r = 0; r < 4; ++r)
                if (4 * q + r < U) dbias[4 * q + r] += v[r];
        return;
    }
    if (!dw) return;
    const int f = blockIdx.x * 16 + q;
    const int reg = f >> 6, lane = f & 63;
    const int wave = reg >> 4, t = (reg >> 2) & 3, u = reg & 3, l16 = lane & 15, g = lane >> 4;
    const int xc = 64 * wave + 16 * u + l16;
#pragma unroll
    for (int r = 0; r < 4; ++r) {
        const int c = 16 * t + 4 * g + r;
        if (c < U) dw[(long long)xc * U + c] += v[r];
    }
}

}

bool dense_softmax_supported(int dtype, long long rows, int K, int U)
{
    return (dtype == QK_BF16 || dtype == QK_F16) && rows >= 0 && (K == 64 || K == 128 || K == 256) && U >= 2 && U <= 64 && (U % 2) == 0 &&
           rows * (long long)K * 2 < 0xF0000000ll;
}

int launch_dense_softmax_fwd(int dtype, long long rows, int K, int U, const void *x, const float *w, const float *bias, void *y, hipStream_t stream)
{
    if (!dense_softmax_supported(dtype, rows, K, U)) return QK_ERR_UNSUPPORTED;
    const long long n_tiles = (rows + 15) / 16;
    long long blocks = (long long)device_cu_count() * 2;
    if (blocks > (n_tiles + 3) / 4) blocks = (n_tiles + 3) / 4;
    if (blocks < 1) blocks = 1;
#define QK_GO(TT, KS) hipLaunchKernelGGL((k_dense_softmax_fwd<TT, KS>), dim3((unsigned)blocks), dim3(256), 0, stream, (const TT *)x, w, bias, (TT *)y, rows, U)
    if (dtype == QK_BF16) { if (K == 256) QK_GO(bf16, 8); else if (K == 128) QK_GO(bf16, 4); else QK_GO(bf16, 2); }
    else { if (K == 256) QK_GO(f16, 8); else if (K == 128) QK_GO(f16, 4); else QK_GO(f16, 2); }
#undef QK_GO
    return hipGetLastError() == hipSuccess ? 0 : QK_ERR_LAUNCH;
}

static int dense_softmax_bwd_grid(long long rows, int K)
{
    const long long n_blocks = (rows + 31) / 32;
    long long blocks = (long long)device_cu_count() * (K == 256 ? 1 : K == 128 ? 2 : 4);
    if (blocks > n_blocks) blocks = n_blocks;
    return (int)(blocks < 1 ? 1 : blocks);
}

size_t dense_softmax_bwd_workspace_bytes(int dtype, long long rows, int K, int U)
{
    if (!dense_softmax_supported(dtype, rows, K, U)) return 0;
    return (size_t)dense_softmax_bwd_grid(rows, K) * ((size_t)(K / 64) * 16 * 256 + 64) * sizeof(float);
}

int launch_dense_softmax_bwd(int dtype, long long rows, int K, int U, const void *x, const float *w, const void *y, const void *dy, void *dx,
                             float *dw, float *dbias, const float *dy_scale_dev, float dy_scale, float *ws, hipStream_t stream)
{
    if (!dense_softmax_supported(dtype, rows, K, U)) return QK_ERR_UNSUPPORTED;
    const int blocks = dense_softmax_bwd_grid(rows, K);
    float *part = (dw || dbias) ? ws : nullptr;
#define QK_GO(TT, NW) do { hipLaunchKernelGGL((k_dense_softmax_bwd<TT, NW>), dim3((unsigned)blocks), dim3(NW * 64), 0, stream, (const TT *)x, w, (const TT *)y, (const TT *)dy, (TT *)dx, part, rows, U, dy_scale_dev, dy_scale); \
        if (part) hipLaunchKernelGGL((k_dense_softmax_reduce<NW>), dim3(NW * 64 + 1), dim3(1024), 0, stream, part, blocks, dw, dbias, U); } while (0)
    if (dtype == QK_BF16) { if (K == 256) QK_GO(bf16, 4); else if (K == 128) QK_GO(bf16, 2); else QK_GO(bf16, 1); }
    else { if (K == 256) QK_GO(f16, 4); else if (K == 128) QK_GO(f16, 2); else QK_GO(f16, 1); }
#undef QK_GO
    return hipGetLastError() == hipSuccess ? 0 : QK_ERR_LAUNCH;
}

}
```

### quaternion-convolutional-neural-networks-for-end-to-end-automatic-speech-recognition_amd/functional.py

```python
import ctypes
import math

import numpy as np
import torch

from . import _lib as L
from ._shape import conv_output_length, normalize_tuple, tf_pads

_DTYPES = {torch.float32: L.QK_F32, torch.bfloat16: L.QK_BF16, torch.float16: L.QK_F16}
_PREP_CACHE_ON = not __import__('os').environ.get('QK_NO_PREP_CACHE')
_PREP_PARAMS = __import__('weakref').WeakValueDictionary()
_CAST_PARAMS = __import__('weakref').WeakValueDictionary()
_PREP_WARNED = False


def invalidate_cached_kernels(params=None):
    if params is None:
        params = list(_PREP_PARAMS.values()) + list(_CAST_PARAMS.values())
    n = 0
    for p in params:
        hit = False
        for key in ('_qk_prep', '_qk_cast16', '_qk_cast'):
            if p.__dict__.pop(key, None) is not None:
                hit = True
# ... 91 lines not shown
        self._ws_bytes = {}

    def _prep_job(self, op):
        d = self.desc
        if isinstance(d, L.DenseDesc):
            c = L.ConvDesc()
            c.rank, c.batch, c.cq, c.fq, c.dtype, c.conj, c.layout = 0, d.rows, d.in_q, d.q_units, d.dtype, 1, L.QK_CH_LAST
            for i in range(3):
                c.in_spatial[i] = c.out_spatial[i] = c.kernel[i] = c.stride[i] = c.dilation[i] = 1
        else:
            c = L.ConvDesc.from_buffer_copy(d)
        return c, (L.QK_OP_FWD if op == L.QK_OP_FWD else L.QK_OP_BWD_DATA)

    def _kernel_only_bytes(self, op):
        d = self.desc
        if d.dtype == L.QK_F32 or getattr(d, 'layout', L.QK_CH_LAST) != L.QK_CH_LAST:
            return 0
        cq, fq = (d.in_q, d.q_units) if isinstance(d, L.DenseDesc) else (d.cq, d.fq)
        if cq % 16 or fq % 16:
            return 0
        kop = L.QK_OP_FWD if op == L.QK_OP_FWD else L.QK_OP_BWD_DATA
        n = self._ws_bytes.get(('k', kop))
        if n is None:
            n = self._ws_bytes[('k', kop)] = int(getattr(L.lib(), self.ws_fn)(ctypes.byref(self.desc), kop))
        return n

    def _prep_key(self, op):
        d = self.desc
        key = ('f' if op == L.QK_OP_FWD else 't', int(d.conj) if hasattr(d, 'conj') else 1, int(d.dtype))
        if getattr(d, 'kernel_order', L.QK_KERNEL_TAPS_MAJOR) != L.QK_KERNEL_TAPS_MAJOR:
            key += (int(d.kernel_order), tuple(d.kernel), int(d.cq), int(d.fq))
        return key

    def _ws(self, op, like, wparam=None):
        n = self._ws_bytes.get(op)
        if n is None:
            n = self._ws_bytes[op] = int(getattr(L.lib(), self.ws_fn)(ctypes.byref(self.desc), op))
        self.desc.ws_has_kernel = 0
        if n == 0:
            return None, 0
        if (wparam is not None and not self.static_buffers and n == self._kernel_only_bytes(op) and wparam.is_leaf
                and wparam.requires_grad and _PREP_CACHE_ON):
            key = self._prep_key(op)
            cache = wparam.__dict__.setdefault('_qk_prep', {})
            base = getattr(wparam, '_qk_flat_base', None)
            ver = (wparam._version, -1 if base is None else base._version)
            hit = cache.get(key)
            if hit is not None and hit[0] == ver and hit[1] == wparam.data_ptr() and hit[2].numel() == n \
                    and hit[2].device == like.device:
                self.desc.ws_has_kernel = 1
                return hit[2], n
            buf = torch.empty(n, dtype=torch.uint8, device=like.device)
            cache[key] = [ver, wparam.data_ptr(), buf, self._prep_job(op)]
            _PREP_PARAMS[id(wparam)] = wparam
            return buf, n
        if self.static_buffers:
            buf = self._ws_cache.get(op)
            if buf is None:
                buf = self._ws_cache[op] = torch.empty(n, dtype=torch.uint8, device=like.device)
            return buf, n
        return torch.empty(n, dtype=torch.uint8, device=like.device), n

    def fwd(self, x, w, bias, out=None, wparam=None):
        y = out if out is not None else torch.empty(self.y_shape, dtype=x.dtype, device=x.device)
        ws, n = self._ws(L.QK_OP_FWD, x, wparam)
        with _on_device(x.device):
            rc = getattr(L.lib(), self.names[0])(ctypes.byref(self.desc), _ptr(x), _ptr(w), _ptr(bias),
                                                 _ptr(y), _ptr(ws), n, _stream(x))
        L.check(rc, self.names[0])
        return y

    def bwd_data(self, dy, y, w, out=None, wparam=None):
        dx = out if out is not None else torch.empty(self.x_shape, dtype=dy.dtype, device=dy.device)
        ws, n = self._ws(L.QK_OP_BWD_DATA, dy, wparam)
        with _on_device(dy.device):
            rc = getattr(L.lib(), self.names[1])(ctypes.byref(self.desc), _ptr(dy), _ptr(y), _ptr(w),
                                                 _ptr(dx), _ptr(ws), n, _stream(dy))
        L.check(rc, self.names[1])
        return dx

    def bwd_weight(self, x, dy, y, has_bias, out=None, masked_dy_out=None, accumulate=False):
        if out is not None:
            dw, db = out
        else:
            dw = torch.empty(self.w_shape, dtype=torch.float32, device=x.device)
            db = torch.empty((self.w_shape[-1],), dtype=torch.float32, device=x.device) if has_bias else None
        ws, n = self._ws(L.QK_OP_BWD_WEIGHT, x)
        if masked_dy_out is not None:
            ws, n = masked_dy_out, masked_dy_out.numel() * masked_dy_out.element_size()
        with _on_device(x.device):
            name = self.names[2] + ('_acc' if accumulate else '')
            if accumulate and out is None:
                raise ValueError('accumulate=True needs the buffers to add into (out=)')
            rc = getattr(L.lib(), name)(ctypes.byref(self.desc), _ptr(x), _ptr(dy), _ptr(y),
                                        _ptr(dw), _ptr(db), _ptr(ws), n, _stream(x))
        L.check(rc, name)
        return dw, db


    def fwd_post(self, x, w, bias, post, wparam=None):
        pre = torch.empty(self.y_shape, dtype=x.dtype, device=x.device) if post.alpha is not None else None
        y = torch.empty(self.y_shape, dtype=x.dtype, device=x.device)
        ws, n = self._ws(L.QK_OP_FWD, x, wparam)
        with _on_device(x.device):
            rc = L.lib().qk_conv_fwd_post(ctypes.byref(self.desc), ctypes.byref(post.struct), _ptr(x), _ptr(w), _ptr(bias),
                                          _ptr(pre), _ptr(y), _ptr(ws), n, _stream(x))
        L.check(rc, 'qk_conv_fwd_post')
        return pre, y

    def bwd_post(self, x, dy, w, has_bias, post_x, x_pre, dalpha_x, direct=None, wparam=None):
        dx = torch.empty(self.x_shape, dtype=dy.dtype, device=dy.device)
        if direct is not None:
            dw, db = direct
        else:
            dw = torch.empty(self.w_shape, dtype=torch.float32, device=x.device)
            db = torch.empty((self.w_shape[-1],), dtype=torch.float32, device=x.device) if has_bias else None
        ws, n = self._ws(L.QK_OP_BWD, x, wparam)
        with _on_device(x.device):
            rc = L.lib().qk_conv_bwd_post(ctypes.byref(self.desc), _ptr(x), _ptr(dy), _ptr(w), _ptr(dx), _ptr(dw), _ptr(db),
                                          ctypes.byref(post_x.struct), _ptr(x_pre), _ptr(dalpha_x),
                                          L.QK_BWD_ACCUMULATE if direct is not None else 0, _ptr(ws), n, _stream(x))
        L.check(rc, 'qk_conv_bwd_post')
        return (dx, None, None) if direct is not None else (dx, dw, db)

    def bwd(self, x, dy, y, w, has_bias, out=None, flags=0, wparam=None):
        if out is not None:
            dx, dw, db = out
        else:
            dx = torch.empty(self.x_shape, dtype=dy.dtype, device=dy.device)
            dw = torch.empty(self.w_shape, dtype=torch.float32, device=x.device)
            db = torch.empty((self.w_shape[-1],), dtype=torch.float32, device=x.device) if has_bias else None
        ws, n = self._ws(L.QK_OP_BWD, x, wparam)
        name = self.names[1].replace('_bwd_data', '_bwd')
        with _on_device(x.device):
            if flags:
                name += '_chain'
                rc = getattr(L.lib(), name)(ctypes.byref(self.desc), _ptr(x), _ptr(dy), _ptr(y), _ptr(w), _ptr(dx),
                                            _ptr(dw), _ptr(db), int(flags), _ptr(ws), n, _stream(x))
            else:
                rc = getattr(L.lib(), name)(ctypes.byref(self.desc), _ptr(x), _ptr(dy), _ptr(y), _ptr(w), _ptr(dx),
                                            _ptr(dw), _ptr(db), _ptr(ws), n, _stream(x))
        L.check(rc, name)
        return dx, dw, db


class PostOp(object):

    def __init__(self, alpha, alpha_axis=-1, rate=0.0, seed=0, seed_dev=None):
        if alpha is not None and (alpha.dtype != torch.float32 or not alpha.is_cuda):
            raise TypeError('PReLU slopes must be float32 device tensors')
        if seed_dev is not None and (seed_dev.dtype != torch.int32 or not seed_dev.is_cuda or seed_dev.numel() != 1):
            raise TypeError('seed_dev must be a one-element int32 device tensor (the training step counter of adam_step)')
        self.seed_dev = seed_dev
        if not 0.0 <= float(rate) < 1.0:
            raise ValueError('dropout rate must be in [0, 1), got %r' % (rate,))
        self.alpha, self.alpha_axis, self.rate, self.seed = alpha, int(alpha_axis), float(rate), int(seed) & 0xffffffff
        self.applied_rate = min(255, int(self.rate * 256.0 + 0.5)) / 256.0
        self.flat = alpha.detach().reshape(-1).contiguous() if alpha is not None else None
        self.struct = L.PostOp(self.alpha_axis if alpha is not None else -1, self.flat.numel() if alpha is not None else 0,
                               self.flat.data_ptr() if alpha is not None else None, self.rate, self.seed,
                               seed_dev.data_ptr() if seed_dev is not None else None)


def _tensor_desc(t):
    d = L.ConvDesc()
    d.rank, d.batch, d.fq, d.dtype = t.dim() - 2, t.shape[0], t.shape[-1] // 4, _DTYPES[t.dtype]
    for i in range(3):
        d.out_spatial[i] = t.shape[1 + i] if i < t.dim() - 2 else 1
    return d


def postop_fwd(pre, post):
    y = torch.empty_like(pre)
    d = _tensor_desc(pre)
    with _on_device(pre.device):
        rc = L.lib().qk_postop_fwd(ctypes.byref(d), ctypes.byref(post.struct), _ptr(pre), _ptr(y), _stream(pre))
    L.check(rc, 'qk_postop_fwd')
    return y


def postop_bwd(pre, dy, post, dalpha):
    dpre = torch.empty_like(pre)
    d = _tensor_desc(pre)
    with _on_device(pre.device):
        rc = L.lib().qk_postop_bwd(ctypes.byref(d), ctypes.byref(post.struct), _ptr(pre), _ptr(dy), _ptr(dpre), _ptr(dalpha),
                                   _stream(pre))
    L.check(rc, 'qk_postop_bwd')
    return dpre


class _PostOpFn(torch.autograd.Function):
    @staticmethod
    def forward(ctx, pre, alpha, post):
        ctx.post = post
        y = postop_fwd(pre, post)
        ctx.save_for_backward(pre if post.alpha is not None else y)
        return y

    @staticmethod
    def backward(ctx, dy):
        pre, = ctx.saved_tensors
        post = ctx.post
        if post.alpha is None:
            return postop_bwd(pre, dy.contiguous(), post, None), None, None
        dalpha = torch.zeros(post.flat.numel(), dtype=torch.float32, device=pre.device)
        dpre = postop_bwd(pre, dy.contiguous(), post, dalpha)
        return dpre, dalpha.reshape(post.alpha.shape), None


def prelu_dropout(x, alpha, alpha_axis=-1, rate=0.0, seed=0):
    _require_device(x, 'prelu_dropout')
    xc = x.contiguous()
    if xc.shape[-1] % (4 if xc.dtype == torch.float32 else 8) or xc.dim() < 2 or xc.dim() > 5:
        raise ValueError('prelu_dropout: unsupported shape %s' % (tuple(x.shape),))
    return _PostOpFn.apply(xc, alpha, PostOp(alpha, alpha_axis, rate, seed))


def relu_dropout(x, rate=0.0, seed=0):
    return prelu_dropout(x, None, -1, rate, seed)


def _direct_grad(w, b, want_w, want_b):
    if not (want_w and getattr(w, '_qk_direct_grad', False) and w.grad is not None and w.grad.is_contiguous()
            and w.grad.dtype == torch.float32):
        return None
    if b is None:
        return w.grad, None
    if not (want_b and getattr(b, '_qk_direct_grad', False) and b.grad is not None and b.grad.is_contiguous()
            and b.grad.dtype == torch.float32):
        return None
    return w.grad, b.grad


def _grad_ready(*params):
    for p in params:
        cb = getattr(p, '_qk_grad_ready', None) if p is not None else None
        if cb is not None:
            cb(p)


class _HamiltonFn(torch.autograd.Function):
    @staticmethod
    def forward(ctx, x, w, bias, call):
        y = call.fwd(x, w, bias, wparam=w)
        ctx.call = call
        ctx.has_bias = bias is not None
        ctx.params = (w, bias)
        ctx.save_for_backward(x, w, y if call.relu else None)
        return y

    @staticmethod
    def backward(ctx, dy):
        x, w, y = ctx.saved_tensors
        call = ctx.call
        dy = dy.contiguous()
        dx = dw = db = None
        want_w = ctx.needs_input_grad[1] or (ctx.has_bias and ctx.needs_input_grad[2])
        direct = _direct_grad(ctx.params[0], ctx.params[1], ctx.needs_input_grad[1], ctx.has_bias and ctx.needs_input_grad[2])
        if ctx.needs_input_grad[0] and want_w:
            if direct is not None:
                dx = torch.empty(call.x_shape, dtype=dy.dtype, device=dy.device)
                call.bwd(x, dy, y, w, ctx.has_bias, out=(dx,) + direct, flags=L.QK_BWD_ACCUMULATE, wparam=ctx.params[0])
            else:
                dx, dw, db = call.bwd(x, dy, y, w, ctx.has_bias, wparam=ctx.params[0])
        elif ctx.needs_input_grad[0]:
            dx = call.bwd_data(dy, y, w, wparam=ctx.params[0])
        elif want_w:
            if direct is not None:
                call.bwd_weight(x, dy, y, ctx.has_bias, out=direct, accumulate=True)
            else:
                dw, db = call.bwd_weight(x, dy, y, ctx.has_bias)
        if direct is not None and want_w:
            _grad_ready(*ctx.params)
        return dx, dw, db, None


def _act_code(activation):
    if activation in (None, 'linear'):
        return L.QK_ACT_LINEAR
    if activation == 'relu':
        return L.QK_ACT_RELU
    raise ValueError('fused activation must be None/"linear"/"relu", got %r' % (activation,))


def _check_weights(w, bias, n_out):
    if w.dtype != torch.float32 or (bias is not None and bias.dtype != torch.float32):
        raise TypeError('kernel / bias must be float32 (Keras floatx); activations may be 16-bit')
    if bias is not None and tuple(bias.shape) != (n_out,):
        raise ValueError('bias must have shape (%d,), got %s' % (n_out, tuple(bias.shape)))


def conv_call(x_shape, w_shape, dtype, rank, strides=1, padding='valid', layout='channels_last',
              dilation_rate=1, activation=None, use_bias=True, conj=False, kernel_order=0):
    st = normalize_tuple(strides, rank, 'strides')
    dl = normalize_tuple(dilation_rate, rank, 'dilation_rate')
    if len(x_shape) != rank + 2 or len(w_shape) != rank + 2:
        raise ValueError('rank %d conv needs %d-D input and kernel' % (rank, rank + 2))
    if layout == 'channels_first':
        ci, sp = x_shape[1], tuple(x_shape[2:])
    else:
        ci, sp = x_shape[-1], tuple(x_shape[1:-1])
    cq, fq = w_shape[-2], w_shape[-1] // 4
    if ci != 4 * cq or w_shape[-1] != 4 * fq:
        raise ValueError('input channels %d / kernel shape %s are not quaternion-consistent'
                         % (ci, tuple(w_shape)))
    d = L.ConvDesc()
# ... 270 lines not shown

    @staticmethod
    def backward(ctx, dout):
        x, aux = ctx.saved_tensors
        dout = dout.contiguous()
        direct = _direct_grad(ctx.params[0], ctx.params[1], ctx.needs_input_grad[1], ctx.has_bias and ctx.needs_input_grad[2])
        if direct is not None:
            dw, db = direct
        else:
            dw = torch.empty(ctx.w_shape, dtype=torch.float32, device=x.device)
            db = torch.empty((ctx.w_shape[-1],), dtype=torch.float32, device=x.device) if ctx.has_bias else None
        with _on_device(x.device):
            rc = L.lib().qk_conv_relu_pool_bwd(ctypes.byref(ctx.call.desc), ctx.pool, _ptr(x), _ptr(dout), _ptr(aux), _ptr(dw), _ptr(db),
                                               L.QK_BWD_ACCUMULATE if direct is not None else 0, _stream(x))
        L.check(rc, 'qk_conv_relu_pool_bwd')
        if direct is not None:
            _grad_ready(*ctx.params)
            return None, None, None, None, None
        return None, dw, db, None, None


def _first_layer_call(x, kernel, activation, use_bias, x_layout):
    if x_layout == 'channels_first':
        n, c, h, w = x.shape
        call = conv_call((n, h, w, c), tuple(kernel.shape), x.dtype, 2, 1, 'same', 'channels_last', 1, activation, use_bias, False)
        call.desc.layout = L.QK_CH_FIRST
        return call
    return conv_call(tuple(x.shape), tuple(kernel.shape), x.dtype, 2, 1, 'same', 'channels_last', 1, activation, use_bias, False)


def conv_relu_pool_supported(x, kernel, pool, x_layout='channels_last'):
    ch_axis, h_axis = (1, 2) if x_layout == 'channels_first' else (-1, 1)
    if not (x.is_cuda and x.dtype in (torch.bfloat16, torch.float16) and x.dim() == 4 and x.shape[ch_axis] == 4 and not x.requires_grad
            and kernel.dim() == 4 and tuple(kernel.shape[:3]) == (3, 5, 1) and kernel.shape[-1] % 4 == 0 and x.shape[0] > 0):
        return False
    if tf_pads(x.shape[h_axis], pool, pool, 1, 'same')[0] != 0:
        return False
    try:
        call = _first_layer_call(x, kernel, 'relu', True, x_layout)
    except ValueError:
        return False
    return int(L.lib().qk_conv_relu_pool_aux_bytes(ctypes.byref(call.desc), pool)) > 0


def conv_relu_pool(x, kernel, bias=None, pool=3, x_layout='channels_last'):
    _require_device(x, 'conv_relu_pool')
    _check_weights(kernel, bias, kernel.shape[-1])
    xc = x.contiguous()
    call = _first_layer_call(xc, kernel, 'relu', bias is not None, x_layout)
    if not L.lib().qk_conv_relu_pool_aux_bytes(ctypes.byref(call.desc), pool):
        raise RuntimeError('conv_relu_pool: geometry outside the fused first-layer kernel')
    return _ConvReluPoolFn.apply(xc, kernel.contiguous(), bias, call, pool)


class _ConvPreluPoolFn(torch.autograd.Function):

    @staticmethod
    def forward(ctx, x, w, bias, alpha, call, pool, post):
        n, h, wd = call.desc.batch, call.desc.in_spatial[0], call.desc.in_spatial[1]
        ctx.params = (w, bias)
        out = torch.empty((n, -(-h // pool), wd, w.shape[-1]), dtype=x.dtype, device=x.device)
        nb = int(L.lib().qk_conv_relu_pool_aux_bytes(ctypes.byref(call.desc), pool))
        keep = any(ctx.needs_input_grad[1:4])
        aux = torch.empty(nb, dtype=torch.uint8, device=x.device) if keep else None
        pre = torch.empty_like(out) if keep else None
        with _on_device(x.device):
            rc = L.lib().qk_conv_prelu_pool_fwd(ctypes.byref(call.desc), pool, ctypes.byref(post.struct), _ptr(x), _ptr(w), _ptr(bias),
                                                _ptr(out), _ptr(pre), _ptr(aux), _stream(x))
        L.check(rc, 'qk_conv_prelu_pool_fwd')
        ctx.call, ctx.pool, ctx.post, ctx.has_bias = call, pool, post, bias is not None
        ctx.w_shape = tuple(w.shape)
        ctx.save_for_backward(x, aux, pre)
        return out

    @staticmethod
    def backward(ctx, dout):
        x, aux, pre = ctx.saved_tensors
        dout = dout.contiguous()
        post = ctx.post
        direct = _direct_grad(ctx.params[0], ctx.params[1], ctx.needs_input_grad[1], ctx.has_bias and ctx.needs_input_grad[2])
        if direct is not None:
            dw, db = direct
        else:
            dw = torch.empty(ctx.w_shape, dtype=torch.float32, device=x.device)
            db = torch.empty((ctx.w_shape[-1],), dtype=torch.float32, device=x.device) if ctx.has_bias else None
        da = torch.zeros(post.flat.numel(), dtype=torch.float32, device=x.device)
        with _on_device(x.device):
            rc = L.lib().qk_conv_prelu_pool_bwd(ctypes.byref(ctx.call.desc), ctx.pool, ctypes.byref(post.struct), _ptr(x), _ptr(dout),
                                                _ptr(pre), _ptr(aux), _ptr(dw), _ptr(db), _ptr(da),
                                                L.QK_BWD_ACCUMULATE if direct is not None else 0, _stream(x))
        L.check(rc, 'qk_conv_prelu_pool_bwd')
        if direct is not None:
            _grad_ready(*ctx.params)
            return None, None, None, da.reshape(post.alpha.shape), None, None, None
        return None, dw, db, da.reshape(post.alpha.shape), None, None, None


def conv_prelu_pool_supported(x, kernel, alpha, alpha_axis, pool, x_layout='channels_last'):
    n = alpha.numel()
    h = x.shape[2] if x_layout == 'channels_first' else x.shape[1]
    return (conv_relu_pool_supported(x, kernel, pool, x_layout) and alpha.is_cuda and alpha.dtype == torch.float32 and
            ((alpha_axis == -1 and n == 1) or (alpha_axis == 0 and n == h and n <= 64)))


def conv_prelu_pool(x, kernel, bias, alpha, alpha_axis=0, pool=3, x_layout='channels_last'):
    _require_device(x, 'conv_prelu_pool')
    _check_weights(kernel, bias, kernel.shape[-1])
    xc = x.contiguous()
    call = _first_layer_call(xc, kernel, None, bias is not None, x_layout)
    post = PostOp(alpha, alpha_axis, 0.0, 0)
    return _ConvPreluPoolFn.apply(xc, kernel.contiguous(), bias, alpha, call, pool, post)


chain_tap = None


class _ConvChainFn(torch.autograd.Function):

    @staticmethod
    def forward(ctx, x, calls, posts, *params):
        n = len(calls)
        ws, bs, alphas = params[:n], params[n:2 * n], params[2 * n:]
        acts, pres = [x], []
        for call, w, b, post in zip(calls, ws, bs, posts):
            if post is None:
                acts.append(call.fwd(acts[-1], w, b, wparam=w))
                pres.append(None)
            else:
                pre, y = call.fwd_post(acts[-1], w, b, post, wparam=w)
                acts.append(y)
                pres.append(pre)
        if chain_tap is not None:
            chain_tap(list(acts))
        ctx.calls, ctx.posts = calls, posts
        ctx.param_refs = (ws, bs)
        ctx.has_bias = [b is not None for b in bs]
        ctx.n_pre = [p is not None for p in pres]
        ctx.save_for_backward(*acts, *ws, *[p for p in pres if p is not None])
        return acts[-1]

    @staticmethod
    def backward(ctx, dy):
        calls, posts = ctx.calls, ctx.posts
        n = len(calls)
        saved = ctx.saved_tensors
        acts, ws = saved[:n + 1], saved[n + 1:2 * n + 1]
        it = iter(saved[2 * n + 1:])
        pres = [next(it) if has else None for has in ctx.n_pre]
        g = dy.contiguous()
        dws, dbs, das = [None] * n, [None] * n, [None] * n
        for i, post in enumerate(posts):
            if post is not None and post.alpha is not None:
                das[i] = torch.zeros(post.flat.numel(), dtype=torch.float32, device=g.device)
        if posts[n - 1] is not None:
            last = posts[n - 1]
            g = postop_bwd(pres[n - 1] if last.alpha is not None else acts[n], g, last, das[n - 1])
        for i in range(n - 1, -1, -1):
            pw, pb = ctx.param_refs[0][i], ctx.param_refs[1][i]
            direct = _direct_grad(pw, pb, ctx.needs_input_grad[3 + i], ctx.has_bias[i] and ctx.needs_input_grad[3 + n + i])
            if i > 0 and posts[i - 1] is not None:
                g, dws[i], dbs[i] = calls[i].bwd_post(acts[i], g, ws[i], ctx.has_bias[i], posts[i - 1], pres[i - 1], das[i - 1],
                                                      direct=direct, wparam=pw)
                if direct is not None:
                    _grad_ready(pw, pb)
                continue
            if i == 0 and not ctx.needs_input_grad[0]:
                if direct is not None:
                    calls[0].bwd_weight(acts[0], g, acts[1], ctx.has_bias[0], out=direct, accumulate=True)
                    _grad_ready(pw, pb)
                else:
                    dws[0], dbs[0] = calls[0].bwd_weight(acts[0], g, acts[1], ctx.has_bias[0])
                g = None
                continue
            flags = 0
            if i > 0 and calls[i - 1].relu:
                flags |= L.QK_BWD_MASK_DX
            if i < n - 1 and calls[i].relu:
                flags |= L.QK_BWD_DY_PREMASKED
            if direct is not None:
                dx = torch.empty(calls[i].x_shape, dtype=g.dtype, device=g.device)
                calls[i].bwd(acts[i], g, acts[i + 1], ws[i], ctx.has_bias[i], out=(dx,) + direct, flags=flags | L.QK_BWD_ACCUMULATE,
                             wparam=pw)
                _grad_ready(pw, pb)
                g = dx
            else:
                g, dws[i], dbs[i] = calls[i].bwd(acts[i], g, acts[i + 1], ws[i], ctx.has_bias[i], flags=flags, wparam=pw)
        das = [None if d is None else d.reshape(p.alpha.shape) for d, p in zip(das, posts)]
        dws = [None if d is None else d.reshape(w.shape) for d, w in zip(dws, ctx.param_refs[0])]
        return (g, None, None) + tuple(dws) + tuple(dbs) + tuple(das)


def quaternion_conv_chain(x, layers):
    _require_device(x, 'quaternion_conv_chain')
    xp = x.contiguous()
    calls, ws, bs, posts, alphas = [], [], [], [], []
    shape = tuple(xp.shape)
    for kernel, bias, kw in layers:
        order = 0
        if kernel.dim() == 2 and kw.get('dense_kernel_size') is not None:
            ksz = tuple(int(v) for v in kw['dense_kernel_size'])
            rank = len(ksz)
            taps = int(math.prod(ksz))
            if kernel.shape[0] % taps:
                raise ValueError('dense kernel rows %d are not a multiple of the %d taps' % (kernel.shape[0], taps))
            kw = dict(kw, conj=True, strides=1, padding='valid', dilation_rate=1)
            w_shape = ksz + (kernel.shape[0] // taps, kernel.shape[1])
            order = L.QK_KERNEL_CHANNEL_MAJOR
        elif kernel.dim() == 2:
            rank = len(shape) - 2
            kw = dict(kw, conj=True, strides=1, padding='valid', dilation_rate=1)
            w_shape = (1,) * rank + tuple(kernel.shape)
        else:
            rank = kernel.dim() - 2
            w_shape = tuple(kernel.shape)
        _check_weights(kernel, bias, kernel.shape[-1])
        po = kw.get('post')
        if po is not None and kw.get('activation') not in (None, 'linear'):
            raise ValueError('a layer with a post-op must be linear (the post-op is its activation)')
        call = conv_call(shape, w_shape, xp.dtype, rank, kw.get('strides', 1), kw.get('padding', 'valid'),
                         'channels_last', kw.get('dilation_rate', 1), kw.get('activation'), bias is not None,
                         bool(kw.get('conj', False)), order)
        calls.append(call)
        ws.append(kernel.contiguous())
        bs.append(bias)
        posts.append(None if po is None else PostOp(po['alpha'], po.get('alpha_axis', -1), po.get('rate', 0.0), po.get('seed', 0), po.get('seed_dev')))
        alphas.append(None if po is None else po['alpha'])
        shape = tuple(call.y_shape)
    return _ConvChainFn.apply(xp, tuple(calls), tuple(posts), *ws, *bs, *alphas)


def softmax_rows_fwd(logits, bias, out_dtype):
    _require_device(logits, 'softmax_rows_fwd')
    if logits.dtype != torch.float32 or logits.dim() != 2 or not logits.is_contiguous() or logits.shape[1] > 64:
        raise ValueError('softmax_rows_fwd: contiguous fp32 (rows, cols <= 64) logits')
    y = torch.empty(logits.shape, dtype=out_dtype, device=logits.device)
    with _on_device(logits.device):
        rc = L.lib().qk_softmax_rows_fwd(_DTYPES[out_dtype], logits.shape[0], logits.shape[1], _ptr(logits), _ptr(bias), _ptr(y), _stream(logits))
    L.check(rc, 'qk_softmax_rows_fwd')
    return y


def softmax_rows_bwd(y, dy, dbias=None):
    _require_device(y, 'softmax_rows_bwd')
    if dy.dtype != y.dtype or dy.shape != y.shape or dy.device != y.device or y.dim() != 2:
        raise ValueError('softmax_rows_bwd: dy must match y (2-D, same shape, dtype and device); got %s %s vs %s %s'
                         % (tuple(dy.shape), dy.dtype, tuple(y.shape), y.dtype))
    if dbias is not None and (dbias.dtype != torch.float32 or dbias.numel() != y.shape[1] or dbias.device != y.device or not dbias.is_contiguous()):
        raise ValueError('softmax_rows_bwd: dbias must be a contiguous fp32 device tensor with one entry per column')
    y, dy = y.contiguous(), dy.contiguous()
    dl = torch.empty_like(y)
    with _on_device(y.device):
        rc = L.lib().qk_softmax_rows_bwd(_DTYPES[y.dtype], y.shape[0], y.shape[1], _ptr(y), _ptr(dy), _ptr(dl), _ptr(dbias), _stream(y))
    L.check(rc, 'qk_softmax_rows_bwd')
    return dl


def dense_softmax_supported(x, units):
    return (x.is_cuda and x.dim() == 2 and x.dtype in (torch.bfloat16, torch.float16) and x.is_contiguous()
            and bool(L.lib().qk_dense_softmax_supported(_DTYPES[x.dtype], x.shape[0], x.shape[1], int(units))))


def dense_softmax_fwd(x, kernel, bias):
    _require_device(x, 'dense_softmax_fwd')
    if kernel.dtype != torch.float32 or not kernel.is_contiguous() or kernel.dim() != 2 or kernel.shape[0] != x.shape[1] or kernel.device != x.device:
        raise ValueError('dense_softmax_fwd: kernel must be a contiguous fp32 (in_dim, units) device tensor')
    if bias is not None and (bias.dtype != torch.float32 or bias.numel() != kernel.shape[1] or not bias.is_contiguous() or bias.device != x.device):
        raise ValueError('dense_softmax_fwd: bias must be a contiguous fp32 device tensor with one entry per unit')
    x = x.contiguous()
    y = torch.empty((x.shape[0], kernel.shape[1]), dtype=x.dtype, device=x.device)
    with _on_device(x.device):
        rc = L.lib().qk_dense_softmax_fwd(_DTYPES[x.dtype], x.shape[0], x.shape[1], kernel.shape[1], _ptr(x), _ptr(kernel), _ptr(bias), _ptr(y), _stream(x))
    L.check(rc, 'qk_dense_softmax_fwd')
    return y


def dense_softmax_bwd(x, kernel, y, dy, dkernel, dbias, dy_scale_dev=None, dy_scale=1.0):
    if dy_scale_dev is not None and (dy_scale_dev.dtype != torch.float32 or dy_scale_dev.numel() != 1 or dy_scale_dev.device != x.device):
        raise ValueError('dense_softmax_bwd: dy_scale_dev must be a one-element fp32 tensor on the device of x')
    _require_device(x, 'dense_softmax_bwd')
    if dy.dtype != y.dtype or dy.shape != y.shape or y.dtype != x.dtype or y.device != x.device or dy.device != x.device:
        raise ValueError('dense_softmax_bwd: y / dy must match each other and x in dtype and device')
    for name, t, n in (('dkernel', dkernel, kernel.numel()), ('dbias', dbias, kernel.shape[1])):
        if t is not None and (t.dtype != torch.float32 or t.numel() != n or not t.is_contiguous() or t.device != x.device):
            raise ValueError('dense_softmax_bwd: %s must be a contiguous fp32 device tensor of %d elements' % (name, n))
    x, y, dy = x.contiguous(), y.contiguous(), dy.contiguous()
    dx = torch.empty_like(x)
    with _on_device(x.device):
        ws, n = None, 0
        if dkernel is not None or dbias is not None:
            n = int(L.lib().qk_dense_softmax_bwd_workspace_bytes(_DTYPES[x.dtype], x.shape[0], x.shape[1], kernel.shape[1]))
            ws = torch.empty(n, dtype=torch.uint8, device=x.device)
        rc = L.lib().qk_dense_softmax_bwd(_DTYPES[x.dtype], x.shape[0], x.shape[1], kernel.shape[1], _ptr(x), _ptr(kernel), _ptr(y), _ptr(dy),
                                          _ptr(dx), _ptr(dkernel), _ptr(dbias), _ptr(dy_scale_dev), float(dy_scale), _ptr(ws), n, _stream(x))
    L.check(rc, 'qk_dense_softmax_bwd')
    return dx


class _WeightedSumFn(torch.autograd.Function):

    @staticmethod
    def forward(ctx, a, w):
        out = torch.zeros((), dtype=torch.float32, device=a.device)
        with _on_device(a.device):
            rc = L.lib().qk_weighted_sum(_DTYPES[a.dtype], a.numel(), _ptr(a), _ptr(w), _ptr(out), _stream(a))
        L.check(rc, 'qk_weighted_sum')
        cache = w.__dict__.setdefault('_qk_cast', {})
        _CAST_PARAMS[id(w)] = w
        hit = cache.get(a.dtype)
        ver = (w._version, w.data_ptr())
        if hit is None or hit[0] != ver:
            hit = cache[a.dtype] = (ver, w.to(a.dtype))
        ctx.wt = hit[1]
        ctx.a_shape = a.shape
        return out

    @staticmethod
    def backward(ctx, g):
        return (ctx.wt * g.to(ctx.wt.dtype)).reshape(ctx.a_shape), None


def weighted_sum(a, w):
    _require_device(a, 'weighted_sum')
    if w.dtype != torch.float32 or w.numel() != a.numel() or w.requires_grad:
        raise ValueError('weighted_sum: w must be a constant fp32 tensor with as many elements as a')
    return _WeightedSumFn.apply(a.contiguous(), w.contiguous())


class _CtcFn(torch.autograd.Function):

    @staticmethod
    def forward(ctx, y_pred, labels, input_length, label_length, loss_scale=1.0):
        b, t, c = y_pred.shape
        lab = labels.to(device=y_pred.device, dtype=torch.int32).contiguous()
        il = input_length.reshape(-1).to(device=y_pred.device, dtype=torch.int32).contiguous()
        ll = label_length.reshape(-1).to(device=y_pred.device, dtype=torch.int32).contiguous()
        lmax = lab.shape[1] if lab.dim() == 2 else 0
        cost = torch.empty(b, dtype=torch.float32, device=y_pred.device)
        want = ctx.needs_input_grad[0]
        dpred = torch.empty_like(y_pred) if want else None
        n = int(L.lib().qk_ctc_workspace_bytes(b, t, lmax))
        ws = torch.empty(n, dtype=torch.uint8, device=y_pred.device)
        with _on_device(y_pred.device):
            rc = L.lib().qk_ctc_batch_cost(_DTYPES[y_pred.dtype], b, t, c, _ptr(y_pred), _ptr(lab), lmax, _ptr(il), _ptr(ll), _ptr(cost),
                                           _ptr(dpred), _ptr(ws), n, _stream(y_pred))
        L.check(rc, 'qk_ctc_batch_cost')
        ctx.save_for_backward(dpred)
        ctx.loss_scale = loss_scale if isinstance(loss_scale, torch.Tensor) else float(loss_scale)
        return cost.reshape(b, 1)

    @staticmethod
    def backward(ctx, dcost):
        dpred, = ctx.saved_tensors
        if isinstance(ctx.loss_scale, torch.Tensor) or ctx.loss_scale != 1.0:
            return (dpred.float() * (dcost.reshape(-1, 1, 1).float() * ctx.loss_scale)).to(dpred.dtype), None, None, None, None
        return dpred * dcost.reshape(-1, 1, 1).to(dpred.dtype), None, None, None, None


def ctc_cost_and_grad(y_pred, labels, input_length, label_length):
    _require_device(y_pred, 'ctc_cost_and_grad')
    y_pred = y_pred.contiguous()
    b, t, c = y_pred.shape
    lab = labels.to(device=y_pred.device, dtype=torch.int32).contiguous()
    il = input_length.reshape(-1).to(device=y_pred.device, dtype=torch.int32).contiguous()
    ll = label_length.reshape(-1).to(device=y_pred.device, dtype=torch.int32).contiguous()
    lmax = lab.shape[1] if lab.dim() == 2 else 0
    cost = torch.empty(b, dtype=torch.float32, device=y_pred.device)
    dpred = torch.empty_like(y_pred)
    n = int(L.lib().qk_ctc_workspace_bytes(b, t, lmax))
    ws = torch.empty(n, dtype=torch.uint8, device=y_pred.device)
    with _on_device(y_pred.device):
        rc = L.lib().qk_ctc_batch_cost(_DTYPES[y_pred.dtype], b, t, c, _ptr(y_pred), _ptr(lab), lmax, _ptr(il), _ptr(ll), _ptr(cost),
                                       _ptr(dpred), _ptr(ws), n, _stream(y_pred))
    L.check(rc, 'qk_ctc_batch_cost')
    return cost, dpred


def ctc_shape_supported(frames, classes, max_label_len):
    return classes <= 256 and max_label_len <= 127 and (frames + 8 * max_label_len + 4 + 2 * classes + 4) * 4 <= 64 * 1024


def ctc_supported(y_pred, labels):
    return (y_pred.is_cuda and y_pred.dtype in _DTYPES and y_pred.dim() == 3 and y_pred.shape[0] > 0 and labels.dim() == 2
            and ctc_shape_supported(y_pred.shape[1], y_pred.shape[2], labels.shape[1]))


def loss_scale_arg(loss_scale, device=None):
    if isinstance(loss_scale, torch.Tensor):
        if (loss_scale.dtype != torch.float32 or loss_scale.numel() != 1 or not loss_scale.is_cuda
                or (device is not None and loss_scale.device != device)):
            raise TypeError('a tensor loss_scale must be a one-element float32 tensor on the device of the data')
        return loss_scale.detach()
    if not (loss_scale > 0 and math.isfinite(loss_scale)):
        raise ValueError('loss_scale must be a positive finite number')
    return float(loss_scale)


def ctc_batch_cost(y_pred, labels, input_length, label_length, loss_scale=1.0):
    _require_device(y_pred, 'ctc_batch_cost')
    return _CtcFn.apply(y_pred.contiguous(), labels, input_length, label_length, loss_scale_arg(loss_scale, y_pred.device))


CTC_MAX_BEAM, CTC_MAX_CLASSES, EDIT_MAX_REF = 128, 256, 1024


def _decode_args(y_pred, input_length, what):
    _require_device(y_pred, what)
    if y_pred.dim() != 3 or min(y_pred.shape) < 1:
        raise ValueError('%s: y_pred must be a non-empty (B, T, C) tensor, got shape %s' % (what, tuple(y_pred.shape)))
    b, t, c = y_pred.shape
    if c < 2 or c > CTC_MAX_CLASSES:
        raise ValueError('%s: %d classes; the decoders take 2 <= classes <= %d' % (what, c, CTC_MAX_CLASSES))
    il = input_length
    if not torch.is_tensor(il):
        il = torch.as_tensor(il)
    if il.numel() != b or (il.dim() == 2 and il.shape[1] != 1) or il.dim() > 2:
        raise ValueError('%s: input_length must have shape (B,) or (B, 1), got %s' % (what, tuple(il.shape)))
    if il.is_cuda and il.device != y_pred.device:
        raise ValueError('%s: input_length is on %s, y_pred on %s' % (what, il.device, y_pred.device))
    il = il.reshape(-1).to(device=y_pred.device, dtype=torch.int32).contiguous()
    return y_pred.contiguous(), il


def ctc_greedy_decode(y_pred, input_length):
    y, il = _decode_args(y_pred, input_length, 'ctc_greedy_decode')
    b, t, c = y.shape
    dec = torch.empty((b, t), dtype=torch.int32, device=y.device)
    dlen = torch.empty(b, dtype=torch.int32, device=y.device)
    lp = torch.empty(b, dtype=torch.float32, device=y.device)
    with _on_device(y.device):
        rc = L.lib().qk_ctc_greedy_decode(_DTYPES[y.dtype], b, t, c, _ptr(y), _ptr(il), _ptr(dec), _ptr(dlen), _ptr(lp), _stream(y))
    L.check(rc, 'qk_ctc_greedy_decode')
    return dec, dlen, lp


def ctc_beam_search_decode(y_pred, input_length, beam_width=100, top_paths=1, merge_repeated=True):
    beam_width, top_paths = int(beam_width), int(top_paths)
    if not 1 <= beam_width <= CTC_MAX_BEAM:
        raise ValueError('ctc_beam_search_decode: beam_width %d outside 1 .. %d' % (beam_width, CTC_MAX_BEAM))
    if not 1 <= top_paths <= beam_width:
        raise ValueError('ctc_beam_search_decode: top_paths %d outside 1 .. beam_width (%d)' % (top_paths, beam_width))
    y, il = _decode_args(y_pred, input_length, 'ctc_beam_search_decode')
    b, t, c = y.shape
    dec = torch.empty((top_paths, b, t), dtype=torch.int32, device=y.device)
    dlen = torch.empty((top_paths, b), dtype=torch.int32, device=y.device)
    lp = torch.empty((b, top_paths), dtype=torch.float32, device=y.device)
    n = int(L.lib().qk_ctc_beam_workspace_bytes(b, t, beam_width))
# ... 314 lines not shown
```

### quaternion-convolutional-neural-networks-for-end-to-end-automatic-speech-recognition_amd/layers.py

```python

import numpy as np
import torch
import torch.nn.functional as F

from . import _lib as L
from . import functional as Fq
from ._shape import normalize_tuple, tf_pads
from .keras_like import Layer, activations, initializers, regularizers


class Flatten(Layer):
    def call(self, inputs):
        return inputs.reshape(inputs.shape[0], -1)

    def compute_output_shape(self, input_shape):
        return (input_shape[0], int(np.prod(input_shape[1:])))


class Dropout(Layer):
    def __init__(self, rate, **kwargs):
        super(Dropout, self).__init__(**kwargs)
        self.rate = rate

    def call(self, inputs):
        return F.dropout(inputs, self.rate, self.training)


class _TallDenseFn(torch.autograd.Function):

    SPLITS = 32

    @staticmethod
    def forward(ctx, x, w, b):
        w16 = w.to(x.dtype)
        ctx.save_for_backward(x, w16)
        ctx.has_bias = b is not None
        out = x @ w16
        return out + b.to(x.dtype) if b is not None else out

    @staticmethod
    def backward(ctx, dy):
        x, w16 = ctx.saved_tensors
        dy = dy.contiguous()
        dx = dy @ w16.t() if ctx.needs_input_grad[0] else None
        dw = db = None
        if ctx.needs_input_grad[1]:
            s = _TallDenseFn.SPLITS
            dw = torch.bmm(x.view(s, -1, x.shape[1]).transpose(1, 2), dy.view(s, -1, dy.shape[1]), out_dtype=torch.float32).sum(0)
        if ctx.has_bias and ctx.needs_input_grad[2]:
            db = dy.float().sum(0)
        return dx, dw, db


def _cast_cached(w, dtype):
    base = getattr(w, '_qk_flat_base', None)
    ver = (w._version, -1 if base is None else base._version, w.data_ptr())
    hit = w.__dict__.get('_qk_cast16')
    if hit is None or hit[0] != ver or hit[1].dtype != dtype:
        hit = (ver, w.detach().to(dtype))
        w.__dict__['_qk_cast16'] = hit
        Fq._CAST_PARAMS[id(w)] = w
    return hit[1]


class _DenseSoftmaxFn(torch.autograd.Function):

    @staticmethod
    def forward(ctx, x, w, b):
        ctx.fused = Fq.dense_softmax_supported(x, w.shape[1]) and w.is_contiguous() and (b is None or b.is_contiguous())
        ctx.params = (w, b)
        if ctx.fused:
            y = Fq.dense_softmax_fwd(x, w.detach(), b.detach() if b is not None else None)
            ctx.save_for_backward(x, w, y)
            return y
        w16 = _cast_cached(w, x.dtype)
        logits = torch.mm(x, w16, out_dtype=torch.float32)
        y = Fq.softmax_rows_fwd(logits, b, x.dtype)
        ctx.save_for_backward(x, w16, y)
        return y

    @staticmethod
    def backward(ctx, dy):
        x, wk, y = ctx.saved_tensors
        w, b = ctx.params
        want_w = ctx.needs_input_grad[1]
        want_b = b is not None and ctx.needs_input_grad[2]
        if ctx.fused:
            direct = Fq._direct_grad(w, b, want_w, want_b) if want_w and (b is None or want_b) else None
            if direct is not None:
                dw, db = direct
            else:
                dw = torch.zeros(w.shape, dtype=torch.float32, device=y.device) if want_w else None
                db = torch.zeros(b.shape, dtype=torch.float32, device=y.device) if want_b else None
            dx = Fq.dense_softmax_bwd(x, wk.detach(), y, dy, dw, db)
            if direct is not None:
                Fq._grad_ready(w, b)
                dw = db = None
            return (dx if ctx.needs_input_grad[0] else None), dw, db
        w16 = wk
        direct_b = want_b and getattr(b, '_qk_direct_grad', False) and b.grad is not None and b.grad.dtype == torch.float32
        db = None
        if want_b:
            db = b.grad if direct_b else torch.zeros(b.shape, dtype=torch.float32, device=y.device)
        dl = Fq.softmax_rows_bwd(y, dy.contiguous(), db)
        dx = dl @ w16.t() if ctx.needs_input_grad[0] else None
        dw = None
        if want_w:
            s = _TallDenseFn.SPLITS
            dw = torch.bmm(x.view(s, -1, x.shape[1]).transpose(1, 2), dl.view(s, -1, dl.shape[1]), out_dtype=torch.float32).sum(0)
        if direct_b:
            Fq._grad_ready(b)
            db = None
        return dx, dw, db


class _DenseSoftmaxCtcMeanFn(torch.autograd.Function):

    @staticmethod
    def forward(ctx, x, w, b, labels, input_length, label_length, batch, loss_scale):
        y = Fq.dense_softmax_fwd(x, w.detach(), b.detach() if b is not None else None)
        cost, dpred = Fq.ctc_cost_and_grad(y.view(batch, -1, y.shape[1]), labels, input_length, label_length)
        ctx.save_for_backward(x, w, y, dpred)
        if isinstance(loss_scale, torch.Tensor):
            ctx.params, ctx.scale, ctx.scale_dev = (w, b), 1.0 / batch, loss_scale
        else:
            ctx.params, ctx.scale, ctx.scale_dev = (w, b), float(loss_scale) / batch, None
        return cost.mean()

    @staticmethod
    def backward(ctx, g):
        x, wk, y, dpred = ctx.saved_tensors
        w, b = ctx.params
        want_w, want_b = ctx.needs_input_grad[1], b is not None and ctx.needs_input_grad[2]
        direct = Fq._direct_grad(w, b, want_w, want_b) if want_w and (b is None or want_b) else None
        if direct is not None:
            dw, db = direct
        else:
            dw = torch.zeros(w.shape, dtype=torch.float32, device=y.device) if want_w else None
            db = torch.zeros(b.shape, dtype=torch.float32, device=y.device) if want_b else None
        g = g.detach().reshape(1).float()
        if ctx.scale_dev is not None:
            g = g * ctx.scale_dev.reshape(1)
        dx = Fq.dense_softmax_bwd(x, wk.detach(), y, dpred.view(y.shape), dw, db, dy_scale_dev=g, dy_scale=ctx.scale)
        if direct is not None:
            Fq._grad_ready(w, b)
            dw = db = None
        return (dx if ctx.needs_input_grad[0] else None), dw, db, None, None, None, None, None


def dense_softmax_ctc_mean(features, dense, labels, input_length, label_length, loss_scale=1.0):
    loss_scale = Fq.loss_scale_arg(loss_scale, features.device if features.is_cuda else None)
    if (not features.is_cuda or features.dim() != 3 or not dense.built or dense.kernel.dtype != torch.float32
            or activations.serialize(dense.activation) != 'softmax' or L.dbg(L.QK_DBG_NO_FUSED_SOFTMAX | L.QK_DBG_NO_FUSED_CTC)):
        return None
    b, t, k = features.shape
    x2 = features.reshape(b * t, k)
    if not (b > 0 and x2.is_contiguous() and Fq.dense_softmax_supported(x2, dense.units) and dense.kernel.is_contiguous()
            and (dense.bias is None or dense.bias.is_contiguous())):
        return None
    if not (labels.dim() == 2 and Fq.ctc_shape_supported(t, dense.units, labels.shape[1])):
        return None
    return _DenseSoftmaxCtcMeanFn.apply(x2, dense.kernel, dense.bias, labels, input_length, label_length, b, loss_scale)


class Dense(Layer):

    def __init__(self, units, activation=None, use_bias=True, kernel_initializer='glorot_uniform',
                 bias_initializer='zeros', kernel_regularizer=None, bias_regularizer=None, **kwargs):
        super(Dense, self).__init__(**kwargs)
        self.units, self.use_bias = units, use_bias
        self.activation = activations.get(activation)
        self.kernel_initializer = initializers.get(kernel_initializer)
        self.bias_initializer = initializers.get(bias_initializer)
        self.kernel_regularizer = regularizers.get(kernel_regularizer)
        self.bias_regularizer = regularizers.get(bias_regularizer)

    def build(self, input_shape):
        self.add_weight('kernel', (input_shape[-1], self.units), initializer=self.kernel_initializer,
                        regularizer=self.kernel_regularizer)
        if self.use_bias:
            self.add_weight('bias', (self.units,), initializer=self.bias_initializer,
                            regularizer=self.bias_regularizer)
        else:
            self.bias = None
        self.built = True

    def call(self, inputs):
        rows = inputs.numel() // max(inputs.shape[-1], 1)
        tall = (inputs.is_cuda and inputs.dtype in (torch.bfloat16, torch.float16) and self.kernel.dtype == torch.float32
                and rows >= 8192 and rows % _TallDenseFn.SPLITS == 0 and inputs.is_contiguous())
        if (inputs.is_cuda and inputs.dtype in (torch.bfloat16, torch.float16) and self.kernel.dtype == torch.float32 and rows > 0
                and inputs.is_contiguous() and activations.serialize(self.activation) == 'softmax' and self.units <= 64
                and not L.dbg(L.QK_DBG_NO_FUSED_SOFTMAX)):
            x2 = inputs.reshape(rows, inputs.shape[-1])
            if tall or Fq.dense_softmax_supported(x2, self.units):
                y = _DenseSoftmaxFn.apply(x2, self.kernel, self.bias)
                return y.reshape(tuple(inputs.shape[:-1]) + (self.units,))
        if tall:
            out = _TallDenseFn.apply(inputs.reshape(rows, inputs.shape[-1]), self.kernel, self.bias)
            return self.activation(out.reshape(tuple(inputs.shape[:-1]) + (self.units,)))
        out = inputs @ self.kernel.to(inputs.dtype)
        if self.bias is not None:
            out = out + self.bias.to(inputs.dtype)
        return self.activation(out)

    def compute_output_shape(self, input_shape):
        return tuple(input_shape[:-1]) + (self.units,)


def _pool_nd(x, pool, strides, padding, axes, mode):
    rank = len(axes)
    if x.dim() == 4 and rank <= 2:
        win, step = [1, 1, 1], [1, 1, 1]
        for ax, pl, st in zip(axes, pool, strides):
            win[ax - 1], step[ax - 1] = pl, st
        if win[0] == 1 and step[0] == 1:
            lo_hi = [tf_pads(x.shape[d], win[d - 1], step[d - 1], 1, padding) for d in (2, 3)]
            if all(lo == 0 for lo, _ in lo_hi):
                ceil = any(hi > 0 for _, hi in lo_hi)
                if mode == 'max':
                    xl = x.permute(0, 2, 3, 1)
                    if xl.is_contiguous() and Fq.maxpool2d_supported(xl, win[1:], step[1:]):
                        out = [-(-x.shape[d] // step[d - 1]) if ceil else (x.shape[d] - win[d - 1]) // step[d - 1] + 1
                               for d in (2, 3)]
                        return Fq.maxpool2d_channels_last(xl, win[1:], out).permute(0, 3, 1, 2)
                    return F.max_pool2d(x, tuple(win[1:]), tuple(step[1:]), ceil_mode=ceil)
                return F.avg_pool2d(x, tuple(win[1:]), tuple(step[1:]), ceil_mode=ceil, count_include_pad=False)
    perm = [0] + [i for i in range(1, x.dim()) if i not in axes] + list(axes)
    xp = x.permute(perm)
    lead = xp.shape[:x.dim() - rank]
    xp = xp.reshape((-1, 1) + tuple(xp.shape[-rank:]))
    pads = []
    for ax in reversed(range(rank)):
        lo, hi = tf_pads(xp.shape[2 + ax], pool[ax], strides[ax], 1, padding)
        pads += [lo, hi]
    fn = {1: (F.max_pool1d, F.avg_pool1d), 2: (F.max_pool2d, F.avg_pool2d), 3: (F.max_pool3d, F.avg_pool3d)}[rank]
    if mode == 'max':
        if any(pads):
            xp = F.pad(xp, pads, value=float('-inf'))
        y = fn[0](xp, pool, strides)
    else:
        k = float(np.prod(pool))
        if any(pads):
            ones = F.pad(torch.ones_like(xp), pads)
            y = fn[1](F.pad(xp, pads), pool, strides) / fn[1](ones, pool, strides)
        else:
            y = fn[1](xp, pool, strides)
        del k
    y = y.reshape(tuple(lead) + tuple(y.shape[-rank:]))
    inv = [0] * x.dim()
    for i, p in enumerate(perm):
        inv[p] = i
    return y.permute(inv)


class _Pooling(Layer):
    rank, mode = 1, 'max'

    def __init__(self, pool_size=2, strides=None, padding='valid', data_format=None, **kwargs):
        super(_Pooling, self).__init__(**kwargs)
        self.pool_size = normalize_tuple(pool_size, self.rank, 'pool_size')
        self.strides = normalize_tuple(self.pool_size if strides is None else strides, self.rank, 'strides')
        self.padding = padding
        self.data_format = 'channels_last' if data_format is None else data_format

    def call(self, inputs):
        first = 2 if self.data_format == 'channels_first' else 1
        axes = tuple(range(first, first + self.rank))
        return _pool_nd(inputs, self.pool_size, self.strides, self.padding, axes, self.mode)


class AveragePooling1D(_Pooling):
    rank, mode = 1, 'avg'


class MaxPooling1D(_Pooling):
    rank, mode = 1, 'max'


class MaxPooling2D(_Pooling):
    rank, mode = 2, 'max'


class AveragePooling2D(_Pooling):
    rank, mode = 2, 'avg'


class PReLU(Layer):

    def __init__(self, alpha_initializer='zeros', alpha_regularizer=None, alpha_constraint=None,
                 shared_axes=None, **kwargs):
        super(PReLU, self).__init__(**kwargs)
        if shared_axes is None:
            self.shared_axes = None
        elif not isinstance(shared_axes, (list, tuple)):
            self.shared_axes = [shared_axes]
        else:
            self.shared_axes = list(shared_axes)
        self.alpha_initializer = initializers.get(alpha_initializer)
        self.alpha_regularizer = regularizers.get(alpha_regularizer)
        self.alpha_constraint = alpha_constraint

    def build(self, input_shape):
        shape = [1 if d is None else d for d in input_shape[1:]]
        for i in self.shared_axes or []:
            shape[i - 1] = 1
        self.add_weight('alpha', tuple(shape), initializer=self.alpha_initializer,
                        regularizer=self.alpha_regularizer, constraint=self.alpha_constraint)
        self.built = True

    def call(self, inputs):
        a = self.alpha.to(inputs.dtype)
        return torch.relu(inputs) - a * torch.relu(-inputs)

    def get_config(self):
# ... 91 lines not shown
```

### quaternion-convolutional-neural-networks-for-end-to-end-automatic-speech-recognition_amd/models/interspeech_model.py

```python

import collections

import torch

from .. import _lib as L
from .. import functional as Fq
from ..complexnn import QuaternionConv2D, QuaternionDense
from ..keras_like import Layer, activations, regularizers
from ..layers import (Dense, Dropout, MaxPooling2D, PReLU, TimeDistributed, ctc_batch_cost, ctc_decode, dense_softmax_ctc_mean,
                      label_error_rate)

EvalResult = collections.namedtuple('EvalResult', 'loss errors symbols per decoded log_prob')


class TimitQCNN(torch.nn.Module):
    def __init__(self, num_layers=10, start_filter=32, act='relu', aact='none', dropout=0.0, l2=0.0,
                 quat_init='quaternion', internal_layout='channels_last', fuse_head=True, chain_convs=True):
        super(TimitQCNN, self).__init__()
        n, sf = num_layers, start_filter
        if aact != 'none':
            act = 'linear'
        reg = regularizers.l2(l2) if l2 else None
        conv_args = dict(activation=act, data_format='channels_first', padding='same', bias_initializer='zeros',
                         kernel_regularizer=reg, kernel_initializer=quat_init, use_bias=True,
                         internal_layout=internal_layout)
        dense_args = dict(activation=act, kernel_regularizer=reg, kernel_initializer='random_uniform',
                          bias_initializer='zeros', use_bias=True)
        self.aact, self.rate, self.act = aact, dropout, act
        self.fuse_head = fuse_head
        self.chain_convs = (chain_convs and internal_layout == 'channels_last'
                            and not L.dbg(L.QK_DBG_NO_CONV_CHAIN))
        self.conv = QuaternionConv2D(sf, (3, 5), name='conv', **conv_args)
        self.pool = MaxPooling2D(pool_size=(1, 3), padding='same')
        widths = [sf] * (n // 2) + [2 * sf] * (n // 2)
        self.convs = torch.nn.ModuleList([QuaternionConv2D(w, (3, 5), name='conv%d' % i, **conv_args)
                                          for i, w in enumerate(widths)])
        self.dense = torch.nn.ModuleList([TimeDistributed(QuaternionDense(256, **dense_args)) for _ in range(3)])
        n_act = 1 + len(widths) + 3
        self.prelu = torch.nn.ModuleList([PReLU(shared_axes=[1, 0]) for _ in range(n_act)]) if aact == 'prelu' else None
        self.drop = Dropout(dropout)
        self._drop_base = 0
        self.drop_step_dev = None
        self.pred = TimeDistributed(Dense(62, activation='softmax', kernel_regularizer=reg, use_bias=True,
                                          bias_initializer='zeros', kernel_initializer='random_uniform'))

    def _act(self, x, i):
        return self.prelu[i](x) if self.prelu is not None else x

    def _new_drop_base(self):
        base = int(torch.randint(0, 2 ** 31 - 1, (1,)).item()) if (self.training and self.rate > 0) else 0
        rank = 0
        if torch.distributed.is_available() and torch.distributed.is_initialized():
            rank = torch.distributed.get_rank()
        self._drop_base = (base ^ (rank * 0x9E3779B1)) & 0xffffffff

    def _post(self, k, out_shape, device, dropout=True):
        rate = self.rate if (dropout and self.training) else 0.0
        seed = (self._drop_base + 7919 * (k + 1)) & 0xffffffff
        if self.prelu is None:
            return dict(alpha=None, alpha_axis=-1, rate=rate, seed=seed, seed_dev=self.drop_step_dev if rate > 0 else None)
        pl = self.prelu[k]
        pl.ensure_built(out_shape, device)
        axis = 0 if pl.alpha.numel() > 1 else -1
        return dict(alpha=pl.alpha, alpha_axis=axis, rate=rate, seed=seed, seed_dev=self.drop_step_dev if rate > 0 else None)

    def _link(self, layer, kernel, k, out_shape, device, fused, dropout=True, **geometry):
        if fused:
            return kernel, layer.bias, dict(geometry, activation=None, post=self._post(k, out_shape, device, dropout))
        return kernel, layer.bias, dict(geometry, activation=activations.serialize(layer.activation))

    def _head_kernel(self, shape, device, dtype, in_chain):
        d0 = self.dense[0].layer
        b, c, f, t = shape
        d0.ensure_built((None, c * f), device)
        if (in_chain and dtype in (torch.bfloat16, torch.float16) and device.type == 'cuda' and (c // 4) % 32 == 0
                and (d0.r.shape[-1] // 4) % 32 == 0 and d0.r.is_contiguous()):
            return d0.r, dict(conj=True, dense_kernel_size=(f, 1))
        w = d0.r.view(c // 4, f, d0.r.shape[-1]).permute(1, 0, 2).unsqueeze(1).contiguous()
        return w, dict(strides=1, padding='valid', dilation_rate=1, conj=True)

    def forward(self, x):
        return self.pred(self.features(x))

    def features(self, x):
        dev, relu_form = x.device, self.prelu is None
        fusable = self.chain_convs and x.is_cuda and x.dtype in (torch.bfloat16, torch.float16, torch.float32)
        if relu_form:
            fused = fusable and self.act == 'relu' and self.training and self.rate > 0 and not L.dbg(L.QK_DBG_NO_FUSED_DROPOUT)
        else:
            fused = fusable and not L.dbg(L.QK_DBG_NO_FUSED_PRELU)
        if fused:
            self._new_drop_base()

        c, pl = self.conv, self.pool
        c.ensure_built(x.shape, dev)
        xl, lay = (x, 'channels_first') if x.is_contiguous() else (x.movedim(1, -1), 'channels_last')
        one_kernel = ((relu_form or fused) and x.is_cuda and x.dim() == 4 and c.padding == 'same' and c.strides == (1, 1)
                      and c.dilation_rate == (1, 1) and c.internal_layout == 'channels_last' and pl.pool_size == (1, 3)
                      and pl.strides == (1, 3) and pl.padding == 'same' and pl.data_format == 'channels_last'
                      and not L.dbg(L.QK_DBG_NO_FUSED_FIRST))
        if relu_form:
            if one_kernel and activations.serialize(c.activation) == 'relu' and Fq.conv_relu_pool_supported(xl, c.kernel, 3, lay):
                o = Fq.conv_relu_pool(xl, c.kernel, c.bias, 3, lay).movedim(-1, 1)
            else:
                o = pl(c(x))
        elif fused:
            po = self._post(0, c.compute_output_shape(tuple(x.shape)), dev, dropout=False)
            if one_kernel and Fq.conv_prelu_pool_supported(xl, c.kernel, po['alpha'], po['alpha_axis'], 3, lay):
                o = Fq.conv_prelu_pool(xl, c.kernel, c.bias, po['alpha'], po['alpha_axis'], 3, lay).movedim(-1, 1)
            else:
                o = pl(Fq.quaternion_conv(x, c.kernel, c.bias, strides=c.strides, padding=c.padding, data_format='channels_first',
                                          dilation_rate=c.dilation_rate, activation=None, post=po))
        else:
            o = pl(self.prelu[0](c(x)))

        chain = fused or (self.chain_convs and x.is_cuda and relu_form and not (self.training and self.rate > 0)
                          and len(self.convs) > 1
                          and all(activations.serialize(cv.activation) in ('linear', 'relu') for cv in self.convs))
        shape, links, k = tuple(o.shape), [], 1
        for cv in self.convs:
            if chain:
                cv.ensure_built(shape, dev)
                shape = cv.compute_output_shape(shape)
                links.append(self._link(cv, cv.kernel, k, shape, dev, fused, strides=cv.strides, padding=cv.padding,
                                        dilation_rate=cv.dilation_rate))
            else:
                o = self.drop(self._act(cv(o), k))
            k += 1

        d0, first = self.dense[0].layer, 0
        if fused or (chain and self.fuse_head and activations.serialize(d0.activation) in ('linear', 'relu')):
            kernel, geometry = self._head_kernel(shape, dev, o.dtype, in_chain=True)
            width = d0.r.shape[-1]
            links.append(self._link(d0, kernel, k, (shape[0], shape[3], width), dev, fused, **geometry))
            k, first = k + 1, 1
            if fused and relu_form and not L.dbg(L.QK_DBG_NO_DENSE_IN_CHAIN):
                for i in (1, 2):
                    dn = self.dense[i].layer
                    dn.ensure_built((None, width), dev)
                    width = dn.r.shape[-1]
                    links.append(self._link(dn, dn.r, k, (shape[0], shape[3], width), dev, fused, dropout=(i < 2)))
                    k, first = k + 1, first + 1
        if chain:
            y = Fq.quaternion_conv_chain(o.movedim(1, -1), links)
            o = y.reshape(y.shape[0], y.shape[2], y.shape[3]) if first else y.movedim(-1, 1)
        if first == 0 and self.fuse_head and o.is_cuda:
            b, t = o.shape[0], o.shape[3]
            kernel, _ = self._head_kernel(tuple(o.shape), dev, o.dtype, in_chain=False)
            name = activations.serialize(d0.activation)
            act = name if name in ('linear', 'relu') else 'linear'
            y = Fq.quaternion_conv(o, kernel, d0.bias, 1, 'valid', 'channels_first', 1, act, conj=True)
            if act != name:
                y = d0.activation(y)
            o = self.drop(self._act(y.reshape(b, d0.r.shape[-1], t).permute(0, 2, 1), k))
            k, first = k + 1, 1
        elif first == 0:
            o = o.permute(0, 3, 1, 2)
            o = o.reshape(o.shape[0], o.shape[1], o.shape[2] * o.shape[3])

        for i in range(first, len(self.dense)):
            if fused:
                dn, (b, t, w) = self.dense[i].layer, o.shape
                dn.ensure_built((None, w), dev)
                po = self._post(k, (b, t, dn.r.shape[-1]), dev, dropout=(i < 2))
                relu = relu_form and po['rate'] == 0.0
                o = Fq.quaternion_dense(o.reshape(b * t, w), dn.r, dn.bias, activation='relu' if relu else None).reshape(b, t, -1)
                if not relu:
                    o = Fq.prelu_dropout(o, po['alpha'], po['alpha_axis'], po['rate'], po['seed'])
            else:
                o = self._act(self.dense[i](o), k)
                if i < 2:
                    o = self.drop(o)
            k += 1
        return o

    def ctc_loss(self, x, labels, input_length, label_length, loss_scale=1.0):
        return ctc_batch_cost(self(x), labels, input_length, label_length, loss_scale=loss_scale)

    def ctc_mean_loss(self, x, labels, input_length, label_length, loss_scale=1.0):
        if not (x.is_cuda and x.dtype in (torch.bfloat16, torch.float16)):
            return self.ctc_loss(x, labels, input_length, label_length, loss_scale=loss_scale).mean()
        feats = self.features(x)
        dense = self.pred.layer
        dense.ensure_built((None, feats.shape[-1]), x.device)
        loss = dense_softmax_ctc_mean(feats, dense, labels, input_length, label_length, loss_scale)
        if loss is None:
            loss = ctc_batch_cost(self.pred(feats), labels, input_length, label_length, loss_scale=loss_scale).mean()
        return loss

    def _inference(self, fn):
        was = self.training
        self.train(False)
        try:
            with torch.no_grad():
                return fn()
        finally:
            self.train(was)

    def decode(self, x, input_length=None, greedy=True, beam_width=100, top_paths=1, merge_repeated=True, lm=None, lm_weight=0.5,
               insertion_bonus=0.0):
        if lm is not None and greedy:
            raise ValueError('decode: a language model needs the beam search (greedy=False)')
        def run():
            y = self(x)
            il = input_length if input_length is not None else torch.full((y.shape[0],), y.shape[1], dtype=torch.int32, device=y.device)
            return ctc_decode(y, il, greedy=greedy, beam_width=beam_width, top_paths=top_paths, merge_repeated=merge_repeated, lm=lm,
                              lm_weight=lm_weight, insertion_bonus=insertion_bonus)
        return self._inference(run)

    def transcribe(self, wave, lengths=None, greedy=True, beam_width=100, top_paths=1, lm=None, lm_weight=0.5, insertion_bonus=0.0,
                   **fbank_kw):
        if lm is not None and greedy:
            raise ValueError('transcribe: a language model needs the beam search (greedy=False)')
        from ..features import quaternion_fbank
        fbank_kw.setdefault('dtype', next(self.parameters()).dtype)
        x, frame_lengths = quaternion_fbank(wave, lengths, **fbank_kw)
        return self.decode(x, frame_lengths, greedy=greedy, beam_width=beam_width, top_paths=top_paths, lm=lm, lm_weight=lm_weight,
                           insertion_bonus=insertion_bonus)

    def evaluate(self, x, labels, input_length, label_length, greedy=True, beam_width=100, class_map=None, lm=None, lm_weight=0.5,
                 insertion_bonus=0.0):
        if lm is not None and greedy:
            raise ValueError('evaluate: a language model needs the beam search (greedy=False)')

        def run():
            y = self(x)
            loss = ctc_batch_cost(y, labels, input_length, label_length).mean()
            decoded, log_prob = ctc_decode(y, input_length, greedy=greedy, beam_width=beam_width, top_paths=1, lm=lm,
                                           lm_weight=lm_weight, insertion_bonus=insertion_bonus)
            errors, symbols, per = label_error_rate(decoded[0], None, labels, label_length, class_map)
            return EvalResult(loss, errors, symbols, per, decoded[0], log_prob)
        return self._inference(run)

    def regularization_loss(self):
        terms = [t for m in self.modules() if isinstance(m, Layer) for t in m.regularization_losses()]
        if not terms:
            return next(self.parameters()).new_zeros(())
        return torch.stack([t.float() for t in terms]).sum()

    def training_loss(self, x, labels, input_length, label_length, loss_scale=1.0):
        reg = self.regularization_loss()
        if isinstance(loss_scale, torch.Tensor):
            loss_scale = Fq.loss_scale_arg(loss_scale, x.device)
        if isinstance(loss_scale, torch.Tensor) or loss_scale != 1.0:
            from ..layers import _GradScale
            reg = _GradScale.apply(reg, loss_scale)
        return self.ctc_mean_loss(x, labels, input_length, label_length, loss_scale=loss_scale) + reg


class _RealConv2D(Layer):

    def __init__(self, filters, kernel_size, activation=None, kernel_regularizer=None, **kwargs):
        super(_RealConv2D, self).__init__(**kwargs)
        from ..keras_like import activations, initializers
        self.filters, self.kernel_size = filters, tuple(kernel_size)
        self.activation = activations.get(activation)
        self.kernel_regularizer = regularizers.get(kernel_regularizer)
        self._init = initializers.get('random_uniform')
        self._zeros = initializers.get('zeros')

    def build(self, input_shape):
        self.add_weight('kernel', self.kernel_size + (input_shape[1], self.filters), initializer=self._init,
                        regularizer=self.kernel_regularizer)
        self.add_weight('bias', (self.filters,), initializer=self._zeros)
        self.built = True

    def call(self, inputs):
        w = self.kernel.permute(3, 2, 0, 1).to(inputs.dtype)
        y = torch.nn.functional.conv2d(inputs, w, self.bias.to(inputs.dtype), padding=(self.kernel_size[0] // 2, self.kernel_size[1] // 2))
        return self.activation(y)

    def compute_output_shape(self, input_shape):
        return (input_shape[0], self.filters) + tuple(input_shape[2:])


class TimitRealCNN(torch.nn.Module):

    def __init__(self, num_layers=10, start_filter=32, act='relu', aact='none', dropout=0.0, l2=0.0):
        super(TimitRealCNN, self).__init__()
        n, sf = num_layers, start_filter
        if aact != 'none':
            act = 'linear'
        reg = regularizers.l2(l2) if l2 else None
        self.conv = _RealConv2D(sf, (3, 5), activation=act, kernel_regularizer=reg)
        self.pool = MaxPooling2D(pool_size=(1, 3), padding='same')
        widths = [sf] * (n // 2) + [2 * sf] * (n // 2)
        self.convs = torch.nn.ModuleList([_RealConv2D(w, (3, 5), activation=act, kernel_regularizer=reg) for w in widths])
        dense_args = dict(activation=act, kernel_regularizer=reg, kernel_initializer='random_uniform', bias_initializer='zeros', use_bias=True)
        self.dense = torch.nn.ModuleList([TimeDistributed(Dense(1024, **dense_args)) for _ in range(3)])
        self.prelu = torch.nn.ModuleList([PReLU(shared_axes=[1, 0]) for _ in range(1 + len(widths) + 3)]) if aact == 'prelu' else None
        self.drop = Dropout(dropout)
        self.pred = TimeDistributed(Dense(62, activation='softmax', kernel_regularizer=reg, use_bias=True,
                                          bias_initializer='zeros', kernel_initializer='random_uniform'))

    def _act(self, x, i):
        return self.prelu[i](x) if self.prelu is not None else x

    def forward(self, x):
        o = self.pool(self._act(self.conv(x), 0))
        k = 1
        for c in self.convs:
            o = self.drop(self._act(c(o), k))
            k += 1
        o = o.permute(0, 3, 1, 2)
        o = o.reshape(o.shape[0], o.shape[1], o.shape[2] * o.shape[3])
        for i, dl in enumerate(self.dense):
            o = self._act(dl(o), k)
            k += 1
            if i < 2:
                o = self.drop(o)
        return self.pred(o)

    def ctc_mean_loss(self, x, labels, input_length, label_length, loss_scale=1.0):
        return self.ctc_loss(x, labels, input_length, label_length, loss_scale=loss_scale).mean()

    ctc_loss = TimitQCNN.ctc_loss
    regularization_loss = TimitQCNN.regularization_loss
    training_loss = TimitQCNN.training_loss


def getTimitModel2D(d):
    kind = getattr(d, 'model', 'quaternion')
    if kind == 'real':
        m = TimitRealCNN(d.num_layers, d.start_filter, d.act, d.aact, d.dropout, getattr(d, 'l2', 0.0))
        return m, (lambda x: m(x))
    if kind != 'quaternion':
        raise ValueError("d.model must be 'quaternion' or 'real', got %r" % (kind,))
    m = TimitQCNN(d.num_layers, d.start_filter, d.act, d.aact, d.dropout, getattr(d, 'l2', 0.0),
                  getattr(d, 'quat_init', 'quaternion'))
    return m, (lambda x: m(x))
```

Before: 14800 samples/s.

## Fuse last two quaternion dense layers and softmax head into one tail kernel

Adds a single HIP kernel that runs dense2 (relu and dropout), dense3 (relu) and the softmax output dense in one pass with MFMA, keeping weights in LDS and activations in registers. The training loss path routes the chain output into this kernel plus CTC through a new autograd function. The softmax backward now applies the relu mask on its input, so the backward through dense3 and dense2 reuses the existing conv bwd_post calls. This cuts separate launches and global round-trips between the tail layers. In exchange it adds a narrow shape-specific path (64 quaternion channels, 16-bit dtypes) and more code to keep correct.

Result: no change. 14850 samples/s (median of 6 runs) (+0.3%).

```diff
diff --git a/include/qk.h b/include/qk.h
--- a/include/qk.h
+++ b/include/qk.h
@@ -75,13 +75,15 @@
 #define QK_DBG_NO_FUSED_FIRST 0x1000000u
 #define QK_DBG_NO_DENSE_IN_CHAIN 0x2000000u
 #define QK_DBG_NO_FUSED_SOFTMAX 0x4000000u
+#define QK_DBG_NO_DENSE_TAIL 0x8000000u
 #define QK_DBG_BAND16_8WAVES 16u
 unsigned qk_set_debug_flags(unsigned flags);
 void qk_set_debug_buffer(void *device_buffer, size_t bytes);
 unsigned qk_get_debug_flags(void);
 
 typedef enum { QK_PATH_NONE = 0, QK_PATH_MFMA16 = 1, QK_PATH_MFMA16_BAND = 2, QK_PATH_FP32_MFMA = 3,
-               QK_PATH_MFMA16_POINT = 4, QK_PATH_MFMA16_SMALL = 5  } qk_path_t;
+               QK_PATH_MFMA16_POINT = 4, QK_PATH_MFMA16_SMALL = 5 ,
+               QK_PATH_DENSE_TAIL = 6  } qk_path_t;
 int qk_last_path(void);
 
 typedef struct {
@@ -264,6 +266,13 @@
 int qk_dense_softmax_bwd(int32_t dtype, int64_t rows, int32_t in_dim, int32_t units, const void *x, const float *kernel, const void *y,
                          const void *dy, void *dx, float *dkernel, float *dbias, const float *dy_scale_dev, float dy_scale,
                          void *workspace, size_t workspace_bytes, void *stream);
+int qk_dense_softmax_bwd_relu(int32_t dtype, int64_t rows, int32_t in_dim, int32_t units, const void *x, const float *kernel, const void *y,
+                              const void *dy, void *dx, float *dkernel, float *dbias, const float *dy_scale_dev, float dy_scale,
+                              int32_t relu_x, void *workspace, size_t workspace_bytes, void *stream);
+int qk_dense_tail_supported(int32_t dtype, int64_t rows, int32_t in_q, int32_t q_units2, int32_t q_units3, int32_t units);
+int qk_dense_tail_fwd(int32_t dtype, int64_t rows, int32_t in_q, int32_t q_units2, int32_t q_units3, int32_t units, const void *h1,
+                      const float *w2, const float *b2, const float *w3, const float *b3, const float *kernel, const float *bias,
+                      const qk_postop_t *post2, void *y2, void *y3, void *y, void *stream);
 int qk_weighted_sum(int32_t dtype, int64_t n, const void *a, const float *w, float *out, void *stream);
 
 int qk_conv_prep_kernels(int32_t n, const qk_conv_desc_t *const *descs, const int32_t *ops, const float *const *w,
diff --git a/quaternion-convolutional-neural-networks-for-end-to-end-automatic-speech-recognition_amd/_lib.py b/quaternion-convolutional-neural-networks-for-end-to-end-automatic-speech-recognition_amd/_lib.py
--- a/quaternion-convolutional-neural-networks-for-end-to-end-automatic-speech-recognition_amd/_lib.py
+++ b/quaternion-convolutional-neural-networks-for-end-to-end-automatic-speech-recognition_amd/_lib.py
@@ -19,6 +19,7 @@
 QK_DBG_NO_SMALL16 = 0x40000
 QK_DBG_NO_CONV_CHAIN, QK_DBG_NO_FUSED_PRELU, QK_DBG_NO_FUSED_DROPOUT, QK_DBG_NO_FUSED_CTC = 0x100000, 0x200000, 0x400000, 0x800000
 QK_DBG_NO_FUSED_FIRST, QK_DBG_NO_DENSE_IN_CHAIN, QK_DBG_NO_FUSED_SOFTMAX = 0x1000000, 0x2000000, 0x4000000
+QK_DBG_NO_DENSE_TAIL = 0x8000000
 QK_WAVE_F32, QK_WAVE_I16 = 0, 1
 QK_WINDOW_RECT, QK_WINDOW_HAMMING = 0, 1
 QK_FBANK_NORM_NONE, QK_FBANK_NORM_UTTERANCE = 0, 1
@@ -26,7 +27,8 @@
 QK_SPECAUG_MAX_MASKS, QK_SPECAUG_PLAN_WORDS = 8, 36
 QK_SPEED_MAX_SPEEDS, QK_SPEED_MAX_DEN, QK_SPEED_MAX_TAPS, QK_SPEED_PLAN_WORDS = 8, 32, 64, 4
 QK_ERR_INVALID_ARG, QK_ERR_UNSUPPORTED, QK_ERR_WORKSPACE, QK_ERR_LAUNCH = -1, -2, -3, -4
-QK_PATH_NAMES = {0: 'none', 1: 'mfma16', 2: 'mfma16_band', 3: 'fp32_mfma', 4: 'mfma16_point', 5: 'mfma16_small'}
+QK_PATH_NAMES = {0: 'none', 1: 'mfma16', 2: 'mfma16_band', 3: 'fp32_mfma', 4: 'mfma16_point', 5: 'mfma16_small',
+                 6: 'dense_tail'}
 
 I32 = ctypes.c_int32
 
@@ -148,8 +150,11 @@
     'qk_softmax_rows_bwd': (ctypes.c_int, [I32, ctypes.c_int64, I32, _VP, _VP, _VP, _VP, _VP]),
     'qk_dense_softmax_supported': (ctypes.c_int, [I32, ctypes.c_int64, I32, I32]),
     'qk_dense_softmax_fwd': (ctypes.c_int, [I32, ctypes.c_int64, I32, I32, _VP, _VP, _VP, _VP, _VP]),
+    'qk_dense_tail_supported': (ctypes.c_int, [I32, ctypes.c_int64, I32, I32, I32, I32]),
+    'qk_dense_tail_fwd': (ctypes.c_int, [I32, ctypes.c_int64, I32, I32, I32, I32, _VP, _FP, _FP, _FP, _FP, _FP, _FP, _PO, _VP, _VP, _VP, _VP]),
     'qk_dense_softmax_bwd_workspace_bytes': (ctypes.c_size_t, [I32, ctypes.c_int64, I32, I32]),
     'qk_dense_softmax_bwd': (ctypes.c_int, [I32, ctypes.c_int64, I32, I32, _VP, _VP, _VP, _VP, _VP, _VP, _VP, _VP, ctypes.c_float, _VP, _SZ, _VP]),
+    'qk_dense_softmax_bwd_relu': (ctypes.c_int, [I32, ctypes.c_int64, I32, I32, _VP, _VP, _VP, _VP, _VP, _VP, _VP, _VP, ctypes.c_float, I32, _VP, _SZ, _VP]),
     'qk_weighted_sum': (ctypes.c_int, [I32, ctypes.c_int64, _VP, _VP, _VP, _VP]),
     'qk_maxpool2d_fwd': (ctypes.c_int, [_PD, _VP, _VP, _VP]),
     'qk_maxpool2d_bwd': (ctypes.c_int, [_PD, _VP, _VP, _VP, _VP]),
diff --git a/quaternion-convolutional-neural-networks-for-end-to-end-automatic-speech-recognition_amd/csrc/qk_api.hip b/quaternion-convolutional-neural-networks-for-end-to-end-automatic-speech-recognition_amd/csrc/qk_api.hip
--- a/quaternion-convolutional-neural-networks-for-end-to-end-automatic-speech-recognition_amd/csrc/qk_api.hip
+++ b/quaternion-convolutional-neural-networks-for-end-to-end-automatic-speech-recognition_amd/csrc/qk_api.hip
@@ -38,6 +38,7 @@
     if (getenv("QK_NO_FUSED_FIRST")) f |= QK_DBG_NO_FUSED_FIRST;
     if (getenv("QK_NO_DENSE_IN_CHAIN")) f |= QK_DBG_NO_DENSE_IN_CHAIN;
     if (getenv("QK_NO_FUSED_SOFTMAX")) f |= QK_DBG_NO_FUSED_SOFTMAX;
+    if (getenv("QK_NO_DENSE_TAIL")) f |= QK_DBG_NO_DENSE_TAIL;
     if (const char *ab = getenv("QK_ABLATE")) f |= ((unsigned)atoi(ab) << kDbgAblateShift) & kDbgAblateMask;
     return f;
 }
@@ -1310,6 +1311,34 @@
     return check_launch(launch_dense_softmax_fwd(dtype, rows, in_dim, units, x, kernel, bias, y, (hipStream_t)stream), "qk_dense_softmax_fwd");
 }
 
+int qk_dense_tail_supported(int32_t dtype, int64_t rows, int32_t in_q, int32_t q_units2, int32_t q_units3, int32_t units)
+{
+    return dense_tail_supported(dtype, rows, in_q, q_units2, q_units3, units) ? 1 : 0;
+}
+
+int qk_dense_tail_fwd(int32_t dtype, int64_t rows, int32_t in_q, int32_t q_units2, int32_t q_units3, int32_t units, const void *h1,
+                      const float *w2, const float *b2, const float *w3, const float *b3, const float *kernel, const float *bias,
+                      const qk_postop_t *post2, void *y2, void *y3, void *y, void *stream)
+{
+    if (!h1 || !w2 || !w3 || !kernel || !y2 || !y3 || !y || rows < 0) { set_error("qk_dense_tail_fwd: NULL buffer or negative row count"); return QK_ERR_INVALID_ARG; }
+    if (!dense_tail_supported(dtype, rows, in_q, q_units2, q_units3, units)) { set_error("qk_dense_tail_fwd: in_q %d / q_units %d, %d / units %d / dtype %d outside the kernel (64 quaternion channels throughout; even units <= 64; 16-bit)", in_q, q_units2, q_units3, units, dtype); return QK_ERR_UNSUPPORTED; }
+    if (post2 && post2->alpha) { set_error("qk_dense_tail_fwd: the relu form of the post-op only (alpha == NULL)"); return QK_ERR_UNSUPPORTED; }
+    if (!aligned(h1, 16) || !aligned(y2, 16) || !aligned(y3, 16) || !aligned(y, 4)) { set_error("qk_dense_tail_fwd: h1 / y2 / y3 must be 16-byte aligned, y 4-byte"); return QK_ERR_INVALID_ARG; }
+    PostOp po;
+    const int32_t sp[3] = {1, 1, 1};
+    if (int rc = to_postop(post2, 0, sp, &po)) return rc;
+    po.kind = 2;
+    po.drop_scale = po.drop_thr ? po.drop_scale : 1.f;
+    if (rows == 0) return QK_OK;
+    qk_conv_desc_t d;
+    memset(&d, 0, sizeof(d));
+    d.batch = (int32_t)(rows > 0x7fffffff ? 0x7fffffff : rows); d.cq = in_q; d.fq = q_units3; d.dtype = dtype;
+    for (int i = 0; i < 3; ++i) d.out_spatial[i] = d.kernel[i] = 1;
+    ProfScope prof_scope(QK_OP_FWD, &d, (hipStream_t)stream);
+    note_path(QK_PATH_DENSE_TAIL);
+    return check_launch(launch_dense_tail_fwd(dtype, rows, units, h1, w2, b2, w3, b3, kernel, bias, y2, y3, y, po, (hipStream_t)stream), "qk_dense_tail_fwd");
+}
+
 size_t qk_dense_softmax_bwd_workspace_bytes(int32_t dtype, int64_t rows, int32_t in_dim, int32_t units)
 {
     return dense_softmax_bwd_workspace_bytes(dtype, rows, in_dim, units);
@@ -1318,6 +1347,14 @@
 int qk_dense_softmax_bwd(int32_t dtype, int64_t rows, int32_t in_dim, int32_t units, const void *x, const float *kernel, const void *y,
                          const void *dy, void *dx, float *dkernel, float *dbias, const float *dy_scale_dev, float dy_scale,
                          void *workspace, size_t workspace_bytes, void *stream)
+{
+    return qk_dense_softmax_bwd_relu(dtype, rows, in_dim, units, x, kernel, y, dy, dx, dkernel, dbias, dy_scale_dev, dy_scale, 0, workspace,
+                                     workspace_bytes, stream);
+}
+
+int qk_dense_softmax_bwd_relu(int32_t dtype, int64_t rows, int32_t in_dim, int32_t units, const void *x, const float *kernel, const void *y,
+                              const void *dy, void *dx, float *dkernel, float *dbias, const float *dy_scale_dev, float dy_scale,
+                              int32_t relu_x, void *workspace, size_t workspace_bytes, void *stream)
 {
     if (!x || !kernel || !y || !dy || !dx || rows < 0) { set_error("qk_dense_softmax_bwd: NULL buffer or negative row count"); return QK_ERR_INVALID_ARG; }
     if (!dense_softmax_supported(dtype, rows, in_dim, units)) { set_error("qk_dense_softmax_bwd: in_dim %d / units %d / dtype %d outside the kernel (in_dim 64, 128, 256; even units <= 64; 16-bit)", in_dim, units, dtype); return QK_ERR_UNSUPPORTED; }
@@ -1327,7 +1364,7 @@
         const size_t need = dense_softmax_bwd_workspace_bytes(dtype, rows, in_dim, units);
         if (!workspace || workspace_bytes < need || !aligned(workspace, 16)) { set_error("qk_dense_softmax_bwd needs %zu workspace bytes (16-byte aligned), got %zu", need, workspace_bytes); return QK_ERR_WORKSPACE; }
     }
-    return check_launch(launch_dense_softmax_bwd(dtype, rows, in_dim, units, x, kernel, y, dy, dx, dkernel, dbias, dy_scale_dev, dy_scale, static_cast<float *>(workspace), (hipStream_t)stream), "qk_dense_softmax_bwd");
+    return check_launch(launch_dense_softmax_bwd(dtype, rows, in_dim, units, x, kernel, y, dy, dx, dkernel, dbias, dy_scale_dev, dy_scale, static_cast<float *>(workspace), (hipStream_t)stream, relu_x ? 1 : 0), "qk_dense_softmax_bwd");
 }
 
 int qk_weighted_sum(int32_t dtype, int64_t n, const void *a, const float *w, float *out, void *stream)
diff --git a/quaternion-convolutional-neural-networks-for-end-to-end-automatic-speech-recognition_amd/csrc/qk_common.h b/quaternion-convolutional-neural-networks-for-end-to-end-automatic-speech-recognition_amd/csrc/qk_common.h
--- a/quaternion-convolutional-neural-networks-for-end-to-end-automatic-speech-recognition_amd/csrc/qk_common.h
+++ b/quaternion-convolutional-neural-networks-for-end-to-end-automatic-speech-recognition_amd/csrc/qk_common.h
@@ -307,7 +307,10 @@
 int launch_dense_softmax_fwd(int dtype, long long rows, int K, int U, const void *x, const float *w, const float *bias, void *y, hipStream_t stream);
 size_t dense_softmax_bwd_workspace_bytes(int dtype, long long rows, int K, int U);
 int launch_dense_softmax_bwd(int dtype, long long rows, int K, int U, const void *x, const float *w, const void *y, const void *dy, void *dx,
-                             float *dw, float *dbias, const float *dy_scale_dev, float dy_scale, float *ws, hipStream_t stream);
+                             float *dw, float *dbias, const float *dy_scale_dev, float dy_scale, float *ws, hipStream_t stream, int relu_x = 0);
+bool dense_tail_supported(int dtype, long long rows, int in_q, int q_units2, int q_units3, int U);
+int launch_dense_tail_fwd(int dtype, long long rows, int U, const void *h1, const float *w2, const float *b2, const float *w3, const float *b3,
+                          const float *wo, const float *bo, void *y2, void *y3, void *p, const PostOp &post2, hipStream_t stream);
 int launch_adam(float *p, float *g, float *m, float *v, const float *decay, size_t n, float lr, float b1,
                 float b2, float eps, int step, float gscale, bool zero_grad, hipStream_t stream, int *step_dev = nullptr);
 size_t grad_guard_workspace_bytes(size_t n);
diff --git a/quaternion-convolutional-neural-networks-for-end-to-end-automatic-speech-recognition_amd/csrc/qk_dense_tail.hip b/quaternion-convolutional-neural-networks-for-end-to-end-automatic-speech-recognition_amd/csrc/qk_dense_tail.hip
--- /dev/null
+++ b/quaternion-convolutional-neural-networks-for-end-to-end-automatic-speech-recognition_amd/csrc/qk_dense_tail.hip
@@ -0,0 +1,224 @@
+#include "qk_common.h"
+#include "qk_postop.h"
+
+namespace qk {
+namespace {
+
+typedef __bf16 t_bf16x8 __attribute__((ext_vector_type(8)));
+typedef _Float16 t_f16x8 __attribute__((ext_vector_type(8)));
+
+__device__ __forceinline__ floatx4 mfma_t(bf16, const uint4 &a, const uint4 &b, const floatx4 &c)
+{
+    return __builtin_amdgcn_mfma_f32_16x16x32_bf16(__builtin_bit_cast(t_bf16x8, a), __builtin_bit_cast(t_bf16x8, b), c, 0, 0, 0);
+}
+__device__ __forceinline__ floatx4 mfma_t(f16, const uint4 &a, const uint4 &b, const floatx4 &c)
+{
+    return __builtin_amdgcn_mfma_f32_16x16x32_f16(__builtin_bit_cast(t_f16x8, a), __builtin_bit_cast(t_f16x8, b), c, 0, 0, 0);
+}
+
+typedef unsigned int t_u32x4 __attribute__((ext_vector_type(4)));
+__device__ __forceinline__ __amdgpu_buffer_rsrc_t rsrc_t(const void *p, unsigned long long bytes)
+{
+    return __builtin_amdgcn_make_buffer_rsrc(const_cast<void *>(p), 0, (int)(bytes > 0xffffffffull ? 0xffffffffu : (unsigned)bytes), 0x00020000);
+}
+__device__ __forceinline__ uint4 ld16_t(__amdgpu_buffer_rsrc_t r, unsigned voff)
+{
+    const t_u32x4 v = __builtin_amdgcn_raw_buffer_load_b128(r, (int)voff, 0, 0);
+    return make_uint4(v.x, v.y, v.z, v.w);
+}
+constexpr unsigned kOobT = 0xF0000000u;
+
+constexpr int kTailQ = 64;
+constexpr int kTailW = 4 * kTailQ;
+constexpr int kHamU = 2 * 4 * 2 * 2 * 64;
+constexpr int kOutU = 8 * 4 * 64;
+
+template <typename T>
+__device__ __forceinline__ void ham_layer16(const uint4 (&x)[4][2], const uint4 *wl, const float *bl, const int lane, const int g, const long long row,
+                                            const long long rows, T *__restrict__ out, const PostOp &post, uint4 (&y)[4][2])
+{
+    constexpr unsigned tbl = kSignConj;
+#pragma unroll
+    for (int u = 0; u < 2; ++u) {
+        floatx4 acc[4][2], accn[4][2];
+#pragma unroll
+        for (int s = 0; s < 2; ++s) {
+            uint4 W[4][2];
+#pragma unroll
+            for (int p = 0; p < 4; ++p)
+#pragma unroll
+                for (int e = 0; e < 2; ++e) W[p][e] = wl[((((s * 4 + p) * 2 + u) * 2 + e) << 6) + lane];
+#pragma unroll
+            for (int a = 0; a < 4; ++a)
+#pragma unroll
+                for (int b = 0; b < 4; ++b) {
+                    const bool ng = (tbl >> (a * 4 + b)) & 1u;
+                    bool first = s == 0;
+#pragma unroll
+                    for (int a2 = 0; a2 < 4; ++a2)
+                        if (a2 < a && (((tbl >> (a2 * 4 + b)) & 1u) != 0) == ng) first = false;
+                    const floatx4 zero = {0.f, 0.f, 0.f, 0.f};
+#pragma unroll
+                    for (int e = 0; e < 2; ++e) {
+                        if (ng) accn[b][e] = mfma_t(T(), W[a ^ b][e], x[a][s], first ? zero : accn[b][e]);
+                        else acc[b][e] = mfma_t(T(), W[a ^ b][e], x[a][s], first ? zero : acc[b][e]);
+                    }
+                }
+        }
+#pragma unroll
+        for (int b = 0; b < 4; ++b) {
+            constexpr unsigned col_neg = (tbl >> 0 | tbl >> 4 | tbl >> 8 | tbl >> 12) & 0xfu;
+            const int ch = b * kTailQ + 32 * u + 8 * g;
+            const float4 b0 = *reinterpret_cast<const float4 *>(bl + ch), b1 = *reinterpret_cast<const float4 *>(bl + ch + 4);
+            const float bv[2][4] = {{b0.x, b0.y, b0.z, b0.w}, {b1.x, b1.y, b1.z, b1.w}};
+            float v[2][4];
+#pragma unroll
+            for (int e = 0; e < 2; ++e)
+#pragma unroll
+                for (int r = 0; r < 4; ++r) {
+                    v[e][r] = acc[b][e][r] + bv[e][r];
+                    if ((col_neg >> b) & 1u) v[e][r] -= accn[b][e][r];
+                }
+            const uint4 pre = make_uint4(repack2(T(), v[0][0], v[0][1]), repack2(T(), v[0][2], v[0][3]),
+                                         repack2(T(), v[1][0], v[1][1]), repack2(T(), v[1][2], v[1][3]));
+            y[b][u] = post_fwd8<T>(pre, 0.f, (unsigned)(row * kTailW + ch), post);
+            if (row < rows) *reinterpret_cast<uint4 *>(out + row * kTailW + ch) = y[b][u];
+        }
+    }
+}
+
+template <typename T>
+__global__ void __launch_bounds__(512) __attribute__((amdgpu_waves_per_eu(2, 2)))
+k_dense_tail_fwd(const T *__restrict__ h1, const float *__restrict__ w2, const float *__restrict__ b2, const float *__restrict__ w3,
+                 const float *__restrict__ b3, const float *__restrict__ wo, const float *__restrict__ bo, T *__restrict__ y2,
+                 T *__restrict__ y3, T *__restrict__ p, const long long rows, const int U, const PostOp post2)
+{
+    __shared__ __attribute__((aligned(16))) uint4 wham[2 * kHamU];
+    __shared__ __attribute__((aligned(16))) uint4 wout[kOutU];
+    __shared__ __attribute__((aligned(16))) float bham[2 * kTailW];
+    const int tid = threadIdx.x, lane = tid & 63, wave = __builtin_amdgcn_readfirstlane(tid >> 6);
+    const int l16 = lane & 15, g = lane >> 4;
+    const __amdgpu_buffer_rsrc_t rx = rsrc_t(h1, (unsigned long long)rows * kTailW * sizeof(T));
+    const long long n_tiles = (rows + 15) / 16;
+    const long long stride = (long long)gridDim.x * 8;
+    long long tile = (long long)wave * gridDim.x + blockIdx.x;
+    uint4 xf[4][2], xn[4][2];
+    auto fetch = [&](long long tl, uint4 (&dst)[4][2]) {
+        const long long row = tl * 16 + l16;
+        const bool ok = tl < n_tiles && row < rows;
+        const unsigned off = ok ? (unsigned)((row * kTailW + 8 * g) * (long long)sizeof(T)) : kOobT;
+#pragma unroll
+        for (int a = 0; a < 4; ++a)
+#pragma unroll
+            for (int s = 0; s < 2; ++s) dst[a][s] = ld16_t(rx, ok ? off + (unsigned)((a * kTailQ + 32 * s) * sizeof(T)) : kOobT);
+    };
+    fetch(tile, xf);
+    {
+#pragma unroll 2
+        for (int un = tid; un < 2 * kHamU; un += 512) {
+            const int ln = un & 63, e = (un >> 6) & 1, u = (un >> 7) & 1, pp = (un >> 8) & 3, s = (un >> 10) & 1, ly = un >> 11;
+            const int f = 32 * u + 8 * ((ln & 15) >> 2) + 4 * e + (ln & 3);
+            const float *src = (ly ? w3 : w2) + (long long)(32 * s + 8 * (ln >> 4)) * kTailW + pp * kTailQ + f;
+            float v[8];
+#pragma unroll
+            for (int k = 0; k < 8; ++k) v[k] = src[k * kTailW];
+            wham[un] = make_uint4(repack2(T(), v[0], v[1]), repack2(T(), v[2], v[3]), repack2(T(), v[4], v[5]), repack2(T(), v[6], v[7]));
+        }
+#pragma unroll 2
+        for (int un = tid; un < kOutU; un += 512) {
+            const int ln = un & 63, t = (un >> 6) & 3, ks = un >> 8;
+            const int c = 16 * t + (ln & 15);
+            const float *src = wo + (long long)(32 * ks + 8 * (ln >> 4)) * U + c;
+            float v[8];
+#pragma unroll
+            for (int k = 0; k < 8; ++k) v[k] = c < U ? src[(long long)k * U] : 0.f;
+            wout[un] = make_uint4(repack2(T(), v[0], v[1]), repack2(T(), v[2], v[3]), repack2(T(), v[4], v[5]), repack2(T(), v[6], v[7]));
+        }
+        if (tid < kTailW) {
+            bham[tid] = b2 ? b2[tid] : 0.f;
+            bham[kTailW + tid] = b3 ? b3[tid] : 0.f;
+        }
+    }
+    __syncthreads();
+    const PostOp ps2 = resolve_seed(post2);
+    PostOp ps3 = ps2;
+    ps3.drop_thr = 0; ps3.drop_scale = 1.f;
+    float bo0[4][4];
+#pragma unroll
+    for (int t = 0; t < 4; ++t)
+#pragma unroll
+        for (int r = 0; r < 4; ++r) {
+            const int c = 16 * t + 4 * g + r;
+            bo0[t][r] = c < U ? (bo ? bo[c] : 0.f) : -1e30f;
+        }
+    for (; tile < n_tiles; tile += stride) {
+        fetch(tile + stride, xn);
+        const long long row = tile * 16 + l16;
+        int lo = lane;
+        asm volatile("" : "+v"(lo));
+        uint4 f2[4][2], f3[4][2];
+        ham_layer16<T>(xf, wham, bham, lo, g, row, rows, y2, ps2, f2);
+        ham_layer16<T>(f2, wham + kHamU, bham + kTailW, lo, g, row, rows, y3, ps3, f3);
+        floatx4 acc[4];
+#pragma unroll
+        for (int t = 0; t < 4; ++t)
+#pragma unroll
+            for (int r = 0; r < 4; ++r) acc[t][r] = bo0[t][r];
+#pragma unroll
+        for (int ks = 0; ks < 8; ++ks)
+#pragma unroll
+            for (int t = 0; t < 4; ++t) acc[t] = mfma_t(T(), wout[((ks * 4 + t) << 6) + lo], f3[ks >> 1][ks & 1], acc[t]);
+        float m = -1e30f;
+#pragma unroll
+        for (int t = 0; t < 4; ++t)
+#pragma unroll
+            for (int r = 0; r < 4; ++r) m = fmaxf(m, acc[t][r]);
+        m = fmaxf(m, __shfl_xor(m, 16));
+        m = fmaxf(m, __shfl_xor(m, 32));
+        float sum = 0.f;
+#pragma unroll
+        for (int t = 0; t < 4; ++t)
+#pragma unroll
+            for (int r = 0; r < 4; ++r) { acc[t][r] = __expf(acc[t][r] - m); sum += acc[t][r]; }
+        sum += __shfl_xor(sum, 16);
+        sum += __shfl_xor(sum, 32);
+        const float inv = 1.f / sum;
+        if (row < rows) {
+            T *pr = p + row * U;
+#pragma unroll
+            for (int t = 0; t < 4; ++t) {
+                const int c = 16 * t + 4 * g;
+                if (c + 1 < U) *reinterpret_cast<unsigned *>(pr + c) = repack2(T(), acc[t][0] * inv, acc[t][1] * inv);
+                if (c + 3 < U) *reinterpret_cast<unsigned *>(pr + c + 2) = repack2(T(), acc[t][2] * inv, acc[t][3] * inv);
+            }
+        }
+#pragma unroll
+        for (int a = 0; a < 4; ++a)
+#pragma unroll
+            for (int s = 0; s < 2; ++s) xf[a][s] = xn[a][s];
+    }
+}
+
+}
+
+bool dense_tail_supported(int dtype, long long rows, int in_q, int q_units2, int q_units3, int U)
+{
+    return (dtype == QK_BF16 || dtype == QK_F16) && rows >= 0 && in_q == kTailQ && q_units2 == kTailQ && q_units3 == kTailQ && U >= 2 &&
+           U <= 64 && (U % 2) == 0 && rows * (long long)kTailW * 2 < 0xF0000000ll;
+}
+
+int launch_dense_tail_fwd(int dtype, long long rows, int U, const void *h1, const float *w2, const float *b2, const float *w3, const float *b3,
+                          const float *wo, const float *bo, void *y2, void *y3, void *p, const PostOp &post2, hipStream_t stream)
+{
+    const long long n_tiles = (rows + 15) / 16;
+    long long blocks = device_cu_count();
+    if (blocks > (n_tiles + 7) / 8) blocks = (n_tiles + 7) / 8;
+    if (blocks < 1) blocks = 1;
+#define QK_GO(TT) hipLaunchKernelGGL((k_dense_tail_fwd<TT>), dim3((unsigned)blocks), dim3(512), 0, stream, (const TT *)h1, w2, b2, w3, b3, wo, bo, \
+                                     (TT *)y2, (TT *)y3, (TT *)p, rows, U, post2)
+    if (dtype == QK_BF16) QK_GO(bf16); else QK_GO(f16);
+#undef QK_GO
+    return hipGetLastError() == hipSuccess ? 0 : QK_ERR_LAUNCH;
+}
+
+}
diff --git a/quaternion-convolutional-neural-networks-for-end-to-end-automatic-speech-recognition_amd/csrc/qk_out_layer.hip b/quaternion-convolutional-neural-networks-for-end-to-end-automatic-speech-recognition_amd/csrc/qk_out_layer.hip
--- a/quaternion-convolutional-neural-networks-for-end-to-end-automatic-speech-recognition_amd/csrc/qk_out_layer.hip
+++ b/quaternion-convolutional-neural-networks-for-end-to-end-automatic-speech-recognition_amd/csrc/qk_out_layer.hip
@@ -1,4 +1,5 @@
 #include "qk_common.h"
+#include "qk_postop.h"
 
 namespace qk {
 namespace {
@@ -140,7 +141,7 @@
 __global__ void __launch_bounds__(NW * 64)
 k_dense_softmax_bwd(const T *__restrict__ x, const float *__restrict__ w, const T *__restrict__ y, const T *__restrict__ dy,
                     T *__restrict__ dx, float *__restrict__ part, const long long rows, const int U,
-                    const float *__restrict__ dy_scale_dev, const float dy_scale)
+                    const float *__restrict__ dy_scale_dev, const float dy_scale, const int relu_x)
 {
     constexpr int K = NW * 64, NTHR = NW * 64;
     constexpr int XP = K * 2 + 32;
@@ -259,7 +260,8 @@
 #pragma unroll
                     for (int u = 0; u < 2; ++u) {
                         const floatx4 a0 = acc[rt][u][0], a1 = acc[rt][u][1];
-                        const uint4 v = make_uint4(pack2o(T(), a0[0], a0[1]), pack2o(T(), a0[2], a0[3]), pack2o(T(), a1[0], a1[1]), pack2o(T(), a1[2], a1[3]));
+                        uint4 v = make_uint4(pack2o(T(), a0[0], a0[1]), pack2o(T(), a0[2], a0[3]), pack2o(T(), a1[0], a1[1]), pack2o(T(), a1[2], a1[3]));
+                        if (relu_x) v = post_bwd8_relu<T>(v, *reinterpret_cast<const uint4 *>(xs + (16 * rt + l16) * XP + (64 * wave + 32 * u + 8 * g) * 2), 1.f);
                         *reinterpret_cast<uint4 *>(dx + row * K + 64 * wave + 32 * u + 8 * g) = v;
                     }
                 }
@@ -395,12 +397,12 @@
 }
 
 int launch_dense_softmax_bwd(int dtype, long long rows, int K, int U, const void *x, const float *w, const void *y, const void *dy, void *dx,
-                             float *dw, float *dbias, const float *dy_scale_dev, float dy_scale, float *ws, hipStream_t stream)
+                             float *dw, float *dbias, const float *dy_scale_dev, float dy_scale, float *ws, hipStream_t stream, int relu_x)
 {
     if (!dense_softmax_supported(dtype, rows, K, U)) return QK_ERR_UNSUPPORTED;
     const int blocks = dense_softmax_bwd_grid(rows, K);
     float *part = (dw || dbias) ? ws : nullptr;
-#define QK_GO(TT, NW) do { hipLaunchKernelGGL((k_dense_softmax_bwd<TT, NW>), dim3((unsigned)blocks), dim3(NW * 64), 0, stream, (const TT *)x, w, (const TT *)y, (const TT *)dy, (TT *)dx, part, rows, U, dy_scale_dev, dy_scale); \
+#define QK_GO(TT, NW) do { hipLaunchKernelGGL((k_dense_softmax_bwd<TT, NW>), dim3((unsigned)blocks), dim3(NW * 64), 0, stream, (const TT *)x, w, (const TT *)y, (const TT *)dy, (TT *)dx, part, rows, U, dy_scale_dev, dy_scale, relu_x); \
         if (part) hipLaunchKernelGGL((k_dense_softmax_reduce<NW>), dim3(NW * 64 + 1), dim3(1024), 0, stream, part, blocks, dw, dbias, U); } while (0)
     if (dtype == QK_BF16) { if (K == 256) QK_GO(bf16, 4); else if (K == 128) QK_GO(bf16, 2); else QK_GO(bf16, 1); }
     else { if (K == 256) QK_GO(f16, 4); else if (K == 128) QK_GO(f16, 2); else QK_GO(f16, 1); }
diff --git a/quaternion-convolutional-neural-networks-for-end-to-end-automatic-speech-recognition_amd/functional.py b/quaternion-convolutional-neural-networks-for-end-to-end-automatic-speech-recognition_amd/functional.py
--- a/quaternion-convolutional-neural-networks-for-end-to-end-automatic-speech-recognition_amd/functional.py
+++ b/quaternion-convolutional-neural-networks-for-end-to-end-automatic-speech-recognition_amd/functional.py
@@ -267,6 +267,7 @@
         if seed_dev is not None and (seed_dev.dtype != torch.int32 or not seed_dev.is_cuda or seed_dev.numel() != 1):
             raise TypeError('seed_dev must be a one-element int32 device tensor (the training step counter of adam_step)')
         self.seed_dev = seed_dev
+        self.bwd_by_consumer = False
         if not 0.0 <= float(rate) < 1.0:
             raise ValueError('dropout rate must be in [0, 1), got %r' % (rate,))
         self.alpha, self.alpha_axis, self.rate, self.seed = alpha, int(alpha_axis), float(rate), int(seed) & 0xffffffff
@@ -843,7 +844,7 @@
         for i, post in enumerate(posts):
             if post is not None and post.alpha is not None:
                 das[i] = torch.zeros(post.flat.numel(), dtype=torch.float32, device=g.device)
-        if posts[n - 1] is not None:
+        if posts[n - 1] is not None and not posts[n - 1].bwd_by_consumer:
             last = posts[n - 1]
             g = postop_bwd(pres[n - 1] if last.alpha is not None else acts[n], g, last, das[n - 1])
         for i in range(n - 1, -1, -1):
@@ -915,6 +916,8 @@
         ws.append(kernel.contiguous())
         bs.append(bias)
         posts.append(None if po is None else PostOp(po['alpha'], po.get('alpha_axis', -1), po.get('rate', 0.0), po.get('seed', 0), po.get('seed_dev')))
+        if po is not None and po.get('bwd_by_consumer'):
+            posts[-1].bwd_by_consumer = True
         alphas.append(None if po is None else po['alpha'])
         shape = tuple(call.y_shape)
     return _ConvChainFn.apply(xp, tuple(calls), tuple(posts), *ws, *bs, *alphas)
@@ -965,7 +968,38 @@
     return y
 
 
-def dense_softmax_bwd(x, kernel, y, dy, dkernel, dbias, dy_scale_dev=None, dy_scale=1.0):
+def dense_tail_supported(h1, q_units2, q_units3, units):
+    return (h1.is_cuda and h1.dim() == 2 and h1.dtype in (torch.bfloat16, torch.float16) and h1.is_contiguous() and h1.shape[1] % 4 == 0
+            and bool(L.lib().qk_dense_tail_supported(_DTYPES[h1.dtype], h1.shape[0], h1.shape[1] // 4, int(q_units2), int(q_units3), int(units))))
+
+
+def dense_tail_fwd(h1, w2, b2, w3, b3, kernel, bias, post2=None):
+    _require_device(h1, 'dense_tail_fwd')
+    for name, t in (('w2', w2), ('w3', w3), ('kernel', kernel)):
+        if t.dtype != torch.float32 or not t.is_contiguous() or t.dim() != 2 or t.device != h1.device:
+            raise ValueError('dense_tail_fwd: %s must be a contiguous fp32 2-D device tensor' % name)
+    if w2.shape[0] * 4 != h1.shape[1] or w3.shape[0] * 4 != w2.shape[1] or kernel.shape[0] != w3.shape[1]:
+        raise ValueError('dense_tail_fwd: the layer widths do not chain: %s -> %s -> %s -> %s'
+                         % (tuple(h1.shape), tuple(w2.shape), tuple(w3.shape), tuple(kernel.shape)))
+    for name, t, n in (('b2', b2, w2.shape[1]), ('b3', b3, w3.shape[1]), ('bias', bias, kernel.shape[1])):
+        if t is not None and (t.dtype != torch.float32 or t.numel() != n or not t.is_contiguous() or t.device != h1.device):
+            raise ValueError('dense_tail_fwd: %s must be a contiguous fp32 device tensor of %d elements' % (name, n))
+    if post2 is not None and post2.alpha is not None:
+        raise ValueError('dense_tail_fwd: the relu form of the post-op only (alpha=None)')
+    h1 = h1.contiguous()
+    rows = h1.shape[0]
+    y2 = torch.empty((rows, w2.shape[1]), dtype=h1.dtype, device=h1.device)
+    y3 = torch.empty((rows, w3.shape[1]), dtype=h1.dtype, device=h1.device)
+    y = torch.empty((rows, kernel.shape[1]), dtype=h1.dtype, device=h1.device)
+    with _on_device(h1.device):
+        rc = L.lib().qk_dense_tail_fwd(_DTYPES[h1.dtype], rows, h1.shape[1] // 4, w2.shape[1] // 4, w3.shape[1] // 4, kernel.shape[1],
+                                       _ptr(h1), _ptr(w2), _ptr(b2), _ptr(w3), _ptr(b3), _ptr(kernel), _ptr(bias),
+                                       ctypes.byref(post2.struct) if post2 is not None else None, _ptr(y2), _ptr(y3), _ptr(y), _stream(h1))
+    L.check(rc, 'qk_dense_tail_fwd')
+    return y2, y3, y
+
+
+def dense_softmax_bwd(x, kernel, y, dy, dkernel, dbias, dy_scale_dev=None, dy_scale=1.0, relu_x=False):
     if dy_scale_dev is not None and (dy_scale_dev.dtype != torch.float32 or dy_scale_dev.numel() != 1 or dy_scale_dev.device != x.device):
         raise ValueError('dense_softmax_bwd: dy_scale_dev must be a one-element fp32 tensor on the device of x')
     _require_device(x, 'dense_softmax_bwd')
@@ -981,8 +1015,9 @@
         if dkernel is not None or dbias is not None:
             n = int(L.lib().qk_dense_softmax_bwd_workspace_bytes(_DTYPES[x.dtype], x.shape[0], x.shape[1], kernel.shape[1]))
             ws = torch.empty(n, dtype=torch.uint8, device=x.device)
-        rc = L.lib().qk_dense_softmax_bwd(_DTYPES[x.dtype], x.shape[0], x.shape[1], kernel.shape[1], _ptr(x), _ptr(kernel), _ptr(y), _ptr(dy),
-                                          _ptr(dx), _ptr(dkernel), _ptr(dbias), _ptr(dy_scale_dev), float(dy_scale), _ptr(ws), n, _stream(x))
+        rc = L.lib().qk_dense_softmax_bwd_relu(_DTYPES[x.dtype], x.shape[0], x.shape[1], kernel.shape[1], _ptr(x), _ptr(kernel), _ptr(y), _ptr(dy),
+                                               _ptr(dx), _ptr(dkernel), _ptr(dbias), _ptr(dy_scale_dev), float(dy_scale), int(bool(relu_x)),
+                                               _ptr(ws), n, _stream(x))
     L.check(rc, 'qk_dense_softmax_bwd')
     return dx
 
diff --git a/quaternion-convolutional-neural-networks-for-end-to-end-automatic-speech-recognition_amd/layers.py b/quaternion-convolutional-neural-networks-for-end-to-end-automatic-speech-recognition_amd/layers.py
--- a/quaternion-convolutional-neural-networks-for-end-to-end-automatic-speech-recognition_amd/layers.py
+++ b/quaternion-convolutional-neural-networks-for-end-to-end-automatic-speech-recognition_amd/layers.py
@@ -161,6 +161,81 @@
     if not (labels.dim() == 2 and Fq.ctc_shape_supported(t, dense.units, labels.shape[1])):
         return None
     return _DenseSoftmaxCtcMeanFn.apply(x2, dense.kernel, dense.bias, labels, input_length, label_length, b, loss_scale)
+
+
+class _DenseTailCtcMeanFn(torch.autograd.Function):
+
+    @staticmethod
+    def forward(ctx, h1, w2, b2, w3, b3, w, b, labels, input_length, label_length, batch, loss_scale, posts):
+        head_post, post2, post3 = posts
+        y2, y3, y = Fq.dense_tail_fwd(h1, w2.detach(), b2.detach() if b2 is not None else None, w3.detach(),
+                                      b3.detach() if b3 is not None else None, w.detach(), b.detach() if b is not None else None, post2)
+        cost, dpred = Fq.ctc_cost_and_grad(y.view(batch, -1, y.shape[1]), labels, input_length, label_length)
+        ctx.save_for_backward(h1, y2, y3, y, dpred, w2, w3, w)
+        ctx.params, ctx.posts, ctx.batch = (w2, b2, w3, b3, w, b), posts, batch
+        if isinstance(loss_scale, torch.Tensor):
+            ctx.scale, ctx.scale_dev = 1.0 / batch, loss_scale
+        else:
+            ctx.scale, ctx.scale_dev = float(loss_scale) / batch, None
+        return cost.mean()
+
+    @staticmethod
+    def backward(ctx, g):
+        h1, y2, y3, y, dpred, w2k, w3k, wk = ctx.saved_tensors
+        w2, b2, w3, b3, w, b = ctx.params
+        head_post, post2, post3 = ctx.posts
+        need = ctx.needs_input_grad
+        want_w, want_b = need[5], b is not None and need[6]
+        direct = Fq._direct_grad(w, b, want_w, want_b) if want_w and (b is None or want_b) else None
+        if direct is not None:
+            dw, db = direct
+        else:
+            dw = torch.zeros(w.shape, dtype=torch.float32, device=y.device) if want_w else None
+            db = torch.zeros(b.shape, dtype=torch.float32, device=y.device) if want_b else None
+        g = g.detach().reshape(1).float()
+        if ctx.scale_dev is not None:
+            g = g * ctx.scale_dev.reshape(1)
+        gy = Fq.dense_softmax_bwd(y3, wk.detach(), y, dpred.view(y.shape), dw, db, dy_scale_dev=g, dy_scale=ctx.scale, relu_x=True)
+        if direct is not None:
+            Fq._grad_ready(w, b)
+            dw = db = None
+        grads = {}
+        rows, t = h1.shape[0], h1.shape[0] // ctx.batch
+        for name, x, wsaved, pw, pb, post_x, iw in (('3', y2, w3k, w3, b3, post2, 3), ('2', h1, w2k, w2, b2, head_post, 1)):
+            call = Fq.conv_call((ctx.batch, 1, t, x.shape[1]), (1, 1) + tuple(pw.shape), x.dtype, 2, 1, 'valid', 'channels_last', 1, None,
+                                pb is not None, True)
+            d = Fq._direct_grad(pw, pb, need[iw], pb is not None and need[iw + 1])
+            gy, gw, gb = call.bwd_post(x, gy, wsaved, pb is not None, post_x, None, None, direct=d, wparam=pw)
+            gy = gy.reshape(rows, -1)
+            if d is not None:
+                Fq._grad_ready(pw, pb)
+            grads[name] = (None if gw is None else gw.reshape(pw.shape), gb)
+        return ((gy if need[0] else None), grads['2'][0], grads['2'][1], grads['3'][0], grads['3'][1], dw, db,
+                None, None, None, None, None, None)
+
+
+def dense_tail_ctc_mean_supported(batch, frames, in_dim, dtype, device, dense2, dense3, dense, labels):
+    if (device.type != 'cuda' or dtype not in (torch.bfloat16, torch.float16) or batch <= 0 or frames <= 0 or in_dim % 4
+            or L.dbg(L.QK_DBG_NO_DENSE_TAIL | L.QK_DBG_NO_DENSE_IN_CHAIN | L.QK_DBG_NO_FUSED_SOFTMAX | L.QK_DBG_NO_FUSED_CTC)):
+        return False
+    if not (dense2.built and dense3.built and dense.built and activations.serialize(dense.activation) == 'softmax'):
+        return False
+    for t in (dense2.r, dense3.r, dense.kernel, dense2.bias, dense3.bias, dense.bias):
+        if t is not None and (t.dtype != torch.float32 or not t.is_contiguous() or t.device != device):
+            return False
+    if dense2.r.shape[0] * 4 != in_dim or dense3.r.shape[0] * 4 != dense2.r.shape[1] or dense.kernel.shape[0] != dense3.r.shape[1]:
+        return False
+    if not L.lib().qk_dense_tail_supported(Fq._DTYPES[dtype], batch * frames, in_dim // 4, dense2.r.shape[1] // 4, dense3.r.shape[1] // 4,
+                                           dense.units):
+        return False
+    return labels.dim() == 2 and Fq.ctc_shape_supported(frames, dense.units, labels.shape[1])
+
+
+def dense_tail_ctc_mean(h1, posts, dense2, dense3, dense, labels, input_length, label_length, loss_scale=1.0):
+    loss_scale = Fq.loss_scale_arg(loss_scale, h1.device)
+    b, t, k = h1.shape
+    return _DenseTailCtcMeanFn.apply(h1.reshape(b * t, k), dense2.r, dense2.bias, dense3.r, dense3.bias, dense.kernel, dense.bias,
+                                     labels, input_length, label_length, b, loss_scale, tuple(posts))
 
 
 class Dense(Layer):
diff --git a/quaternion-convolutional-neural-networks-for-end-to-end-automatic-speech-recognition_amd/models/interspeech_model.py b/quaternion-convolutional-neural-networks-for-end-to-end-automatic-speech-recognition_amd/models/interspeech_model.py
--- a/quaternion-convolutional-neural-networks-for-end-to-end-automatic-speech-recognition_amd/models/interspeech_model.py
+++ b/quaternion-convolutional-neural-networks-for-end-to-end-automatic-speech-recognition_amd/models/interspeech_model.py
@@ -8,7 +8,7 @@
 from ..complexnn import QuaternionConv2D, QuaternionDense
 from ..keras_like import Layer, activations, regularizers
 from ..layers import (Dense, Dropout, MaxPooling2D, PReLU, TimeDistributed, ctc_batch_cost, ctc_decode, dense_softmax_ctc_mean,
-                      label_error_rate)
+                      dense_tail_ctc_mean, dense_tail_ctc_mean_supported, label_error_rate)
 
 EvalResult = collections.namedtuple('EvalResult', 'loss errors symbols per decoded log_prob')
 
@@ -83,6 +83,9 @@
         return self.pred(self.features(x))
 
     def features(self, x):
+        return self._features(x)
+
+    def _features(self, x, tail_labels=None):
         dev, relu_form = x.device, self.prelu is None
         fusable = self.chain_convs and x.is_cuda and x.dtype in (torch.bfloat16, torch.float16, torch.float32)
         if relu_form:
@@ -134,6 +137,17 @@
             width = d0.r.shape[-1]
             links.append(self._link(d0, kernel, k, (shape[0], shape[3], width), dev, fused, **geometry))
             k, first = k + 1, 1
+            if fused and relu_form and tail_labels is not None and not L.dbg(L.QK_DBG_NO_DENSE_IN_CHAIN):
+                d1, d2, dp = self.dense[1].layer, self.dense[2].layer, self.pred.layer
+                d1.ensure_built((None, width), dev)
+                d2.ensure_built((None, d1.r.shape[-1]), dev)
+                dp.ensure_built((None, d2.r.shape[-1]), dev)
+                if dense_tail_ctc_mean_supported(shape[0], shape[3], width, o.dtype, dev, d1, d2, dp, tail_labels):
+                    links[-1][2]['post']['bwd_by_consumer'] = True
+                    tail_posts = [Fq.PostOp(None, -1, po['rate'], po['seed'], po['seed_dev']) for po in
+                                  (links[-1][2]['post'], self._post(k, None, dev), self._post(k + 1, None, dev, dropout=False))]
+                    y = Fq.quaternion_conv_chain(o.movedim(1, -1), links)
+                    return y.reshape(y.shape[0], y.shape[2], y.shape[3]), tail_posts
             if fused and relu_form and not L.dbg(L.QK_DBG_NO_DENSE_IN_CHAIN):
                 for i in (1, 2):
                     dn = self.dense[i].layer
@@ -180,8 +194,11 @@
     def ctc_mean_loss(self, x, labels, input_length, label_length, loss_scale=1.0):
         if not (x.is_cuda and x.dtype in (torch.bfloat16, torch.float16)):
             return self.ctc_loss(x, labels, input_length, label_length, loss_scale=loss_scale).mean()
-        feats = self.features(x)
         dense = self.pred.layer
+        feats = self._features(x, tail_labels=labels)
+        if isinstance(feats, tuple):
+            return dense_tail_ctc_mean(feats[0], feats[1], self.dense[1].layer, self.dense[2].layer, dense, labels, input_length,
+                                       label_length, loss_scale)
         dense.ensure_built((None, feats.shape[-1]), x.device)
         loss = dense_softmax_ctc_mean(feats, dense, labels, input_length, label_length, loss_scale)
         if loss is None:
```
